# Eurus-Holmes/VAG-NMT

Hardware: AMD Instinct MI355X
Metric: training sentence-pairs/sec (Multi30K en->de, B=64) (higher is better)
Workload: dtype f32; 1 GPU; configs[1]: multimodal en->de train step, B=64/GPU, Ts=Tt=40, E=256, H=512, S=512, I=2048, Vs=8507, V=9391, dropout 0.3/0.5/0.5, tied emb, teacher_force_ratio=1; global_batch=64, parallelism=dp1, hip_graph=True

## Files before the change

include/vag_nmt.h:

```cpp
#ifndef VAG_NMT_H
#define VAG_NMT_H
#include <stddef.h>
#include <stdint.h>

#ifdef __cplusplus
extern "C" {
#endif

typedef void* vag_stream_t;

typedef struct { const float *w_ih, *w_hh, *b_ih, *b_hh; } vag_gru_w;
typedef struct { float *w_ih, *w_hh, *b_ih, *b_hh; } vag_gru_g;

typedef struct {
    const float* emb;
    vag_gru_w gru1;
    const float *attn_h, *attn_v, *c2h;
    vag_gru_w gru2;
} vag_dec_w;
typedef struct {
    float* emb;
    vag_gru_g gru1;
    float *attn_h, *attn_v, *c2h;
    vag_gru_g gru2;
// ... 367 lines not shown
int vag_mrt_pack(const int64_t* cand, int64_t G, int64_t Nc, int64_t L, const int64_t* gold, int64_t Tg, int include_gold, int64_t* tgt,
                 int64_t Tt, float* valid, vag_stream_t stream);

#define VAG_ADAM_SCRATCH_BYTES 2048
#define VAG_ADAM_SCRATCH_SKIPPED_OFFSET 28
#define VAG_ADAM_SCRATCH_GUARD_OFFSET 32
int vag_clip_adam_flat(float* p, float* g, float* m, float* v, int64_t n, int nseg, const int64_t* seg_off,
                       const float* seg_lr, const float* seg_wd, float clip, float grad_scale, float beta1,
                       float beta2, float eps, int zero_grad, int32_t* step, float* norm_out, void* scratch,
                       const float* lr_dev, vag_stream_t stream);

int vag_clip_adam_flat_ema(float* p, float* g, float* m, float* v, int64_t n, int nseg, const int64_t* seg_off,
                           const float* seg_lr, const float* seg_wd, float clip, float grad_scale, float beta1,
                           float beta2, float eps, int zero_grad, int32_t* step, float* norm_out, void* scratch,
                           const float* lr_dev, float* ema, float ema_decay, int ema_warmup, vag_stream_t stream);

int vag_swap_flat(float* a, float* b, int64_t n, vag_stream_t stream);

int vag_clip_adam_shard(float* p, float* g, float* m, float* v, int64_t n, int nseg, const int64_t* seg_off,
                        const float* seg_lr, const float* seg_wd, float clip, float grad_scale, float beta1,
                        float beta2, float eps, int zero_grad, int32_t* step, float* norm_out, void* scratch,
                        const float* lr_dev, int64_t lo, int64_t hi, int phase, double* sumsq, vag_stream_t stream);

typedef struct {
    const float* enc_emb;
    vag_gru_w enc_fw, enc_bw;
    const float *im_w, *im_b, *txt_w, *txt_b, *ctx2ctx, *emb2ctx, *mlp_w;
    const float *ini_w, *ini_b;
    const float* attn_e;
    vag_dec_w dec;
    vag_head_w head;
} vag_model_w;
typedef struct {
    float* enc_emb;
    vag_gru_g enc_fw, enc_bw;
    float *im_w, *im_b, *txt_w, *txt_b, *ctx2ctx, *emb2ctx, *mlp_w;
    float *ini_w, *ini_b;
    float* attn_e;
    vag_dec_g dec;
    vag_head_g head;
} vag_model_g;
typedef struct {
    int64_t B, Ts, Tt, Es, Et, H, S, I, V, ldl;
    int32_t multimodal;
    int32_t attn_method;
    int32_t activation_vse;
    int32_t rank_kind;
    int32_t free_run;
    int32_t storage;
    float margin, loss_w, init_split, p_emb, p_ctx, p_out;
    int32_t loss_ring;
    void* guard;
    float label_smoothing;
    int32_t mrt_n;
    float mrt_alpha, mrt_scale;
    const float *mrt_cost, *mrt_valid;
} vag_step_cfg;
int64_t vag_step_ws_floats(const vag_step_cfg* cfg);
int64_t vag_step_ws_offset(const vag_step_cfg* cfg, int which);
int vag_train_step(const vag_step_cfg* cfg, const vag_model_w* w, const vag_model_g* g, const int64_t* src,
                   const int32_t* lengths, const int64_t* tgt, const float* im, const float* vocab_weight, uint64_t* rng,
                   const float* derived, float* ws, float* losses, int phases, vag_stream_t stream);
typedef struct {
    int32_t k;
    float lambda;
    const int32_t* idx;
    const float* q;
} vag_kd_cfg;
int vag_step_kd_check(const vag_step_cfg* cfg, const vag_kd_cfg* kd);
int vag_train_step_kd(const vag_step_cfg* cfg, const vag_kd_cfg* kd, const vag_model_w* w, const vag_model_g* g, const int64_t* src,
                      const int32_t* lengths, const int64_t* tgt, const float* im, const float* vocab_weight, uint64_t* rng,
                      const float* derived, float* ws, float* losses, int phases, vag_stream_t stream);
typedef struct {
    float alpha;
    float* kl;
} vag_rdrop_cfg;
int vag_step_rdrop_check(const vag_step_cfg* cfg, const vag_rdrop_cfg* rd);
int vag_train_step_rdrop(const vag_step_cfg* cfg, const vag_rdrop_cfg* rd, const vag_model_w* w, const vag_model_g* g,
                         const int64_t* src, const int32_t* lengths, const int64_t* tgt, const float* im, const float* vocab_weight,
                         uint64_t* rng, const float* derived, float* ws, float* losses, int phases, vag_stream_t stream);
int vag_set_operator_context(const float* derived, int storage);
int vag_set_option(const char* name, int64_t value);
int64_t vag_handoff_planes_floats(int64_t B, int64_t Ts, int64_t Tt, int64_t H);
int vag_set_handoff_planes(float* buf, int64_t floats);
int vag_copy4(const void* const* src, void* const* dst, const int64_t* bytes, int n, vag_stream_t stream);
int64_t vag_derived_floats(int64_t H);
int vag_derive_weights(vag_dec_w w, const float* enc_whh_fw, const float* enc_whh_bw, int64_t H, int with_fp16,
                       float* derived, vag_stream_t stream);

int vag_recurrence_supported(int kind, int64_t B, int64_t Ts, int64_t Tt, int64_t H);
int vag_persistent_timeouts(void);
int vag_set_operator_guard(void* guard);
int vag_recurrence_time(int kind, double* ms_total, int* launches);
int vag_gemm_group_plan(int n, const int64_t* M, const int64_t* N, const int64_t* K, const int* accumulate, int* split, int* order);
enum { VAG_GEMM_TILED64 = 0,
       VAG_GEMM_TILED128_F32 = 1,
       VAG_GEMM_SPLIT128 = 2,
       VAG_GEMM_BIG256 = 3 };
int vag_gemm_plan(int64_t M, int64_t N, int64_t K, int a_kc, int b_kc, int vec, float beta, int act, int c_half, int a_bf16,
                  int rowsum, int planes, int* plan);
int64_t vag_recurrence_sync_words(int kind, int64_t B, int64_t T);
int vag_cgru_recurrence_fwd(const float* pe, const float* mask, const float* h0, const float* xp1, vag_dec_w w, const float* wcat,
                            const float* bcat, const float* encwp, int64_t B, int64_t Ts, int64_t Tt, int64_t H, float* h1,
                            float* g1, float* qhp, float* alpha, float* h2_all, float* g2, float* psc, void* sync,
                            vag_stream_t stream);

#define VAG_COMM_ID_BYTES 128
typedef struct vag_comm_s* vag_comm_t;
int vag_comm_unique_id(void* id);
int vag_comm_init(vag_comm_t* comm, int nranks, int rank, const void* id);
int vag_comm_allreduce(vag_comm_t comm, float* buf, int64_t n, vag_stream_t stream);
int vag_comm_size(vag_comm_t comm);
int vag_comm_destroy(vag_comm_t comm);

int vag_dropout_mask(const uint64_t* rng, int which, int64_t n, float p, float* out, vag_stream_t stream);
int vag_rng_advance(uint64_t* rng, vag_stream_t stream);

#ifdef __cplusplus
}
#endif
#endif
```

vag-nmt_amd/csrc/api.hip:

```cpp
#include "../../include/vag_nmt.h"
#include "api_shared.h"
#include <cstring>

static thread_local VagCallCtx g_base_ctx;
static thread_local VagCallCtx* g_active_ctx = nullptr;
VagCallCtx& vag_ctx() { return g_active_ctx ? *g_active_ctx : g_base_ctx; }
VagCallScope::VagCallScope(VagCallCtx& c) : ctx(c), prev(g_active_ctx) { g_active_ctx = &c; }
VagCallScope::~VagCallScope() {
    (void)vag_loss_defer_flush();
    if (ctx.leaf_on) vag_leaf_drop();
    g_active_ctx = prev;
}
static inline const float* as_f(const vag_half* p) { return reinterpret_cast<const float*>(p); }

VagOptions& vag_opt() {
    static VagOptions o;
    return o;
}

extern "C" {

int vag_version(void) { return 330; }

int vag_set_option(const char* name, int64_t value) {
// ... 325 lines not shown
    hipStream_t s = S_(stream);
    VAG_CHECK_ARG(dec_w_ok(w) && prep && H > 0 && H % 4 == 0 && aligned16(prep));
    const int64_t C = 2 * H;
    CgruPrep p = cgru_prep(prep, H);
    VAG_TRY(copy_async(p.wcat, w.attn_h, C * H * sizeof(float), s));
    VAG_TRY(copy_async(p.wcat + C * H, w.gru2.w_hh, 3 * H * H * sizeof(float), s));
    VAG_TRY(zero_async(p.bcat, C * sizeof(float), s));
    VAG_TRY(copy_async(p.bcat + C, w.gru2.b_hh, 3 * H * sizeof(float), s));
    return gemm_nn(3 * H, C, H, w.gru2.w_ih, H, w.c2h, C, 0.f, p.wp, C, s);
}

int vag_derive_weights(vag_dec_w w, const float* enc_whh_fw, const float* enc_whh_bw, int64_t H, int with_fp16,
                       float* derived, vag_stream_t stream) {
    hipStream_t s = S_(stream);
    VAG_CHECK_ARG(dec_w_ok(w) && enc_whh_fw && enc_whh_bw && derived && H > 0 && H % 4 == 0 && aligned16(derived));
    const int64_t C = 2 * H, Q = C + 3 * H;
    DerivedW d = derived_layout(derived, H);
    CgruPrep p = cgru_prep(d.prep, H);
    const VagJob jobs[9] = {
        {w.attn_h, p.wcat, C, H, H, H, 1},
        {w.gru2.w_hh, p.wcat + C * H, 3 * H, H, H, H, 1},
        {nullptr, p.bcat, 1, C, C, C, 0},
        {w.gru2.b_hh, p.bcat + C, 1, 3 * H, 3 * H, 3 * H, 1},
        {w.attn_h, d.wcatT, C, H, H, Q, 2},
        {w.gru2.w_hh, d.wcatT + C, 3 * H, H, H, Q, 2},
        {w.gru1.w_hh, d.whh1T, 3 * H, H, H, 3 * H, 2},
        {enc_whh_fw, d.encT, 3 * H, H, H, 3 * H, 2},
        {enc_whh_bw, d.encT + 3 * H * H, 3 * H, H, H, 3 * H, 2},
    };
    VAG_TRY(vag_jobs_launch(jobs, 9, s));
    if (with_fp16) {
        VAG_CHECK_ARG(H % 8 == 0);
        auto h = [&](vag_half* q) { return reinterpret_cast<float*>(q); };
        const VagJob j16[10] = {
            {w.attn_h, h(d.wcat16), C, H, H, H, 3},
            {w.gru2.w_hh, h(d.wcat16 + C * H), 3 * H, H, H, H, 3},
            {w.attn_h, h(d.wcatT16), C, H, H, Q, 4},
            {w.gru2.w_hh, h(d.wcatT16 + C), 3 * H, H, H, Q, 4},
            {w.gru1.w_hh, h(d.whh1_16), 3 * H, H, H, H, 3},
            {w.gru1.w_hh, h(d.whh1T16), 3 * H, H, H, 3 * H, 4},
            {enc_whh_fw, h(d.enc16), 3 * H, H, H, H, 3},
            {enc_whh_bw, h(d.enc16 + 3 * H * H), 3 * H, H, H, H, 3},
            {enc_whh_fw, h(d.encT16), 3 * H, H, H, 3 * H, 4},
            {enc_whh_bw, h(d.encT16 + 3 * H * H), 3 * H, H, H, 3 * H, 4},
        };
        VAG_TRY(vag_jobs_launch(j16, 10, s));
    }
    return VAG_OK;
}

struct CgruWs {
    float *xp1, *h1, *g1, *g2, *qhp, *scores, *alpha, *tmp, *prep, *encwp;
    float* uk;
    float* psc;
    unsigned* sync;
    unsigned* sync_b;
    float* dal;
    int64_t total;
};
static CgruWs cgru_ws(float* ws, int64_t B, int64_t Ts, int64_t Tt, int64_t E, int64_t H) {
    CgruWs w;
    const int64_t C = 2 * H;
    WsCarver c(ws);
    w.xp1 = c.take(Tt * B * 3 * H);
    w.g1 = c.take(Tt * 4 * B * H);
    w.g2 = c.take(Tt * 4 * B * H);
    w.qhp = c.take(Tt * B * (C + 3 * H));
    w.scores = c.take(B * Ts);
    w.alpha = c.take(Tt * B * Ts);
    w.tmp = c.take(B * E);
    w.prep = c.take(cgru_prep(nullptr, H).total);
    w.encwp = c.take(B * Ts * 3 * H);
    w.uk = c.take(B * Ts * H);
    w.h1 = c.take(Tt * B * H);
    w.psc = c.take(Tt * B * Ts * 4);
    w.sync = c.take_as<unsigned>(vag_dec_persistent_sync_words(B, Tt));
    w.sync_b = c.take_as<unsigned>(vag_dec_persistent_sync_words(B, Tt));
    w.dal = c.take(Tt * B * Ts * 4);
    w.total = c.off;
    return w;
}
}
void vag_step_zero_ranges(float* ws_enc, float* ws_dec, int64_t B, int64_t Ts, int64_t Tt, int64_t Es, int64_t Et, int64_t H,
                          unsigned** p, int64_t* n) {
    BiGruWs e = bigru_ws(ws_enc, B, Ts, Es, H);
    p[0] = e.sync;
    n[0] = (reinterpret_cast<unsigned*>(ws_enc) + e.total) - e.sync;
    CgruWs d = cgru_ws(ws_dec, B, Ts, Tt, Et, H);
    p[2] = reinterpret_cast<unsigned*>(e.dx);
    n[2] = Ts * B * Es;
    p[1] = reinterpret_cast<unsigned*>(d.h1);
    n[1] = (reinterpret_cast<unsigned*>(ws_dec) + d.total) - p[1];
}
extern "C" {
int64_t vag_cgru_ws_floats(int64_t B, int64_t Ts, int64_t Tt, int64_t E, int64_t H) {
    return cgru_ws(nullptr, B, Ts, Tt, E, H).total;
}
int64_t vag_cgru_ws_offset(int64_t B, int64_t Ts, int64_t Tt, int64_t E, int64_t H, int which) {
    static float base[1];
    CgruWs k = cgru_ws(base, B, Ts, Tt, E, H);
    const float* p = which == 0 ? k.alpha : which == 1 ? k.h1 : which == 2 ? k.qhp : nullptr;
    return p ? (int64_t)(p - base) : -1;
}

struct StepBufs {
    const float* xp1;
    const float* hprev;
    float *h1, *g1, *g2, *qhp, *scores, *alpha, *c, *h2;
};

static int cgru_step(const float* enc, const float* pe, const float* mask, int64_t rps, const vag_dec_w& w,
                     const CgruPrep& p, int64_t N, int64_t Ts, int64_t H, const StepBufs& b, hipStream_t s) {
    const int64_t C = 2 * H, Q = C + 3 * H;
    GruStepArgs a = gru_cell_args(b.xp1, b.hprev, w.gru1.w_hh, w.gru1.b_hh, N, H, b.h1, b.g1);
    VAG_TRY(vag_gru_step_launch(a, 1, s));
    VAG_TRY(vag_skinny_launch(N, Q, H, b.h1, H, p.wcat, H, p.bcat, nullptr, 0, b.qhp, Q, 0, s));
    VAG_TRY(vag_attn_scores_launch(0, pe, b.qhp, Q, w.attn_v, mask, N, rps, Ts, C, b.scores, s));
    VAG_TRY(vag_attn_ctx_launch(1, b.scores, enc, N, rps, Ts, C, b.alpha, b.c, s));
    a.lda = C; a.ldw = C; a.ldother = Q; a.K = (int)C; a.comp_hidden = 0;
    a.s[0].A = b.c; a.s[0].W = p.wp; a.s[0].bias = w.gru2.b_ih; a.s[0].other = b.qhp + C;
    a.s[0].hprev = b.h1; a.s[0].hout = b.h2; a.s[0].save = b.g2;
    VAG_TRY(vag_gru_step_launch(a, 1, s));
    return VAG_OK;
}

int vag_cgru_attn_decode_seq_fwd(const float* enc, const float* pe, const float* mask, const float* h0, int64_t* tok,
                                 vag_dec_w w, int64_t B, int64_t Ts, int64_t Tt, int64_t E, int64_t H, int64_t V,
                                 float* h2_all, float* c_all, float* e_all, float* ws, int free_run,
                                 const vag_head_w* head, float p_out, const uint64_t* rng, float* tmid, float* logits,
                                 int64_t ldl, vag_stream_t stream) {
    hipStream_t s = S_(stream);
    VAG_CHECK_ARG(enc && pe && mask && h0 && tok && h2_all && c_all && e_all && ws && dec_w_ok(w));
    VAG_CHECK_ARG(B > 0 && Ts > 0 && Tt > 0 && E % 4 == 0 && H % 4 == 0 && E > 0 && H > 0 && aligned16(ws));
    VAG_CHECK_ARG(!free_run || (head && tmid && logits && ldl >= V && ldl % 4 == 0));
    const int64_t C = 2 * H, Q = C + 3 * H, BH = B * H;
    CgruWs k = cgru_ws(ws, B, Ts, Tt, E, H);
    CgruPrep p = cgru_prep(k.prep, H);
    if (vag_ctx().derived) p = cgru_prep(derived_layout(const_cast<float*>(vag_ctx().derived), H).prep, H);
    else VAG_TRY(vag_cgru_prepare(w, H, k.prep, stream));
    const bool hoist = !free_run;
    const bool s16 = vag_ctx().store16;
    VAG_CHECK_ARG(!s16 || (hoist && vag_ctx().derived && H % 8 == 0 && Ts * B < (1ll << 28)));
    DerivedW dw16 = {};
    if (s16) dw16 = derived_layout(const_cast<float*>(vag_ctx().derived), H);
    {
        VagGemmGroup grp;
        if (!free_run) {
            if (!vag_ctx().step_gathered) VAG_TRY(vag_embed_gather_launch(tok, B, 1, Tt, B, w.emb, E, e_all, nullptr, 0, 0.f, s));
            VAG_TRY(vag_gemm_launch(Tt * B, 3 * H, E, 1.f, e_all, E, 1, w.gru1.w_ih, 1, E, 0.f, k.xp1, 3 * H, w.gru1.b_ih, 0, s));
        }
        VAG_TRY(vag_gemm_launch(B * Ts, H, C, 1.f, enc, C, 1, w.c2h, 1, C, 0.f, k.uk, H, nullptr, 0, s));
        VAG_TRY(grp.end(s));
    }
    {
        VagGemmGroup grp2;
        VAG_TRY(vag_gemm_launch(B * Ts, 3 * H, H, 1.f, k.uk, H, 1, w.gru2.w_ih, 1, H, 0.f, k.encwp, 3 * H, nullptr, 0, s, s16 ? 1 : 0));
        VAG_TRY(grp2.end(s));
    }
    auto hoisted_step = [&](int64_t t) -> int {
        const float* hprev = t == 0 ? h0 : h2_all + (t - 1) * BH;
        float* h1 = k.h1 + t * BH;
        float* qhp = k.qhp + t * B * Q;
        const GruStepArgs a = gru_cell_args(k.xp1 + t * B * 3 * H, hprev, s16 ? as_f(dw16.whh1_16) : w.gru1.w_hh, w.gru1.b_hh, B, H,
                                            h1, k.g1 + t * 4 * BH);
        VAG_TRY(vag_gru_step_launch(a, 1, s, s16));
        if (s16) {
            VAG_TRY(vag_skinny_launch(B, C, H, h1, H, as_f(dw16.wcat16), H, nullptr, nullptr, 0, qhp, Q, 0, s, true));
            VAG_TRY(vag_attn_dot_side_launch(0, pe, qhp, Q, w.attn_v, mask, nullptr, B, Ts, C, k.scores, B, 3 * H, H, h1, H,
                                             as_f(dw16.wcat16 + C * H), H, p.bcat + C, nullptr, qhp + C, Q, s, true));
            VAG_TRY(vag_attn_ctx_gru_launch(k.scores, k.encwp, B, 1, Ts, H, w.gru2.b_ih, qhp + C, Q, h1, k.alpha + t * B * Ts,
                                            h2_all + t * BH, k.g2 + t * 4 * BH, s, true));
            return VAG_OK;
        }
        if (Ts * B < (1ll << 28)) {
// ... 827 lines not shown
int vag_sample_step_p_dev(const float* const* logp, const int64_t* ldl, int64_t M, int64_t* toks, float* token_logp,
                          int32_t* di_state, int64_t max_len, int64_t* tok_out, int64_t B, int64_t n, int64_t V, float temperature,
                          int64_t top_k, const uint64_t* rng, int32_t* n_alive, float top_p, int32_t* set_size,
                          vag_stream_t stream) {
    VAG_CHECK_ARG(di_state != nullptr);
    return vag_sample_step_p_launch(logp, ldl, M, toks, token_logp, 0, di_state, max_len, nullptr, nullptr, nullptr, tok_out, B, n,
                                    V, temperature, top_k, rng, n_alive, top_p, set_size, S_(stream));
}
int vag_sample_noise(const uint64_t* rng, int64_t di, int64_t N, int64_t V, float* out, vag_stream_t stream) {
    return vag_sample_noise_launch(rng, di, N, V, out, S_(stream));
}

int vag_mbr_supported(int64_t Nh, int64_t Lh, int64_t Nr, int64_t Lr) { return vag_mbr_supported_host(Nh, Lh, Nr, Lr); }
int vag_mbr_select(const int64_t* hyps, const int64_t* refs, const float* weights, int64_t B, int64_t Nh, int64_t Lh, int64_t Nr,
                   int64_t Lr, int utility, int32_t* matches, float* util, float* expected, int64_t* best, vag_stream_t stream) {
    return vag_mbr_select_launch(hyps, refs, weights, B, Nh, Lh, Nr, Lr, utility, matches, util, expected, best, S_(stream));
}

int vag_corpus_bleu_supported(int64_t Lh, int64_t R, int64_t Lr) { return vag_corpus_bleu_supported_host(Lh, R, Lr); }
int vag_corpus_bleu_stats(const int64_t* hyps, const int64_t* refs, const int32_t* n_refs, int64_t N, int64_t Lh, int64_t R,
                          int64_t Lr, int32_t* per_sentence, int64_t* totals, vag_stream_t stream) {
    return vag_corpus_bleu_stats_launch(hyps, refs, n_refs, N, Lh, R, Lr, per_sentence, totals, S_(stream));
}

int vag_surface_expand(const int64_t* rows, int64_t R, int64_t L, const int32_t* off, const int32_t* chars, int64_t V, int32_t* out,
                       int64_t C, int32_t* lens, vag_stream_t stream) {
    return vag_surface_expand_launch(rows, R, L, off, chars, V, out, C, lens, S_(stream));
}
int vag_chrf_supported(int64_t Nh, int64_t Ch, int64_t Nr, int64_t Cr) { return vag_chrf_supported_host(Nh, Ch, Nr, Cr); }
int vag_chrf_max_chars(void) { return vag_chrf_max_chars_host(); }
int vag_chrf_select(const int32_t* hchars, const int32_t* hlens, const int32_t* rchars, const int32_t* rlens, const float* weights,
                    int64_t B, int64_t Nh, int64_t Ch, int64_t Nr, int64_t Cr, int32_t* matches, float* util, float* expected,
                    int64_t* best, vag_stream_t stream) {
    return vag_chrf_select_launch(hchars, hlens, rchars, rlens, weights, B, Nh, Ch, Nr, Cr, matches, util, expected, best, S_(stream));
}

int vag_mrt_weights(const float* nll, const float* cost, const float* valid, int64_t B, int64_t Tt, int64_t N, float alpha, float scale,
                    float* inv_cnt, float* q, float* risk, vag_stream_t stream) {
    VAG_CHECK_ARG(risk != nullptr);
    return vag_mrt_weights_launch(nll, cost, valid, B, Tt, N, alpha, scale, inv_cnt, q, risk, nullptr, 0.f, 0, S_(stream));
}
int vag_mrt_pack(const int64_t* cand, int64_t G, int64_t Nc, int64_t L, const int64_t* gold, int64_t Tg, int include_gold, int64_t* tgt,
                 int64_t Tt, float* valid, vag_stream_t stream) {
    return vag_mrt_pack_launch(cand, G, Nc, L, gold, Tg, include_gold, tgt, Tt, valid, S_(stream));
}

int vag_clip_adam_flat(float* p, float* g, float* m, float* v, int64_t n, int nseg, const int64_t* seg_off,
                       const float* seg_lr, const float* seg_wd, float clip, float grad_scale, float beta1, float beta2,
                       float eps, int zero_grad, int32_t* step, float* norm_out, void* scratch, const float* lr_dev,
                       vag_stream_t stream) {
    return vag_clip_adam_launch(p, g, m, v, n, nseg, seg_off, seg_lr, seg_wd, clip, grad_scale, beta1, beta2, eps, zero_grad,
                                step, norm_out, scratch, lr_dev, S_(stream));
}

int vag_clip_adam_flat_ema(float* p, float* g, float* m, float* v, int64_t n, int nseg, const int64_t* seg_off,
                           const float* seg_lr, const float* seg_wd, float clip, float grad_scale, float beta1, float beta2,
                           float eps, int zero_grad, int32_t* step, float* norm_out, void* scratch, const float* lr_dev,
                           float* ema, float ema_decay, int ema_warmup, vag_stream_t stream) {
    return vag_clip_adam_ema_launch(p, g, m, v, n, nseg, seg_off, seg_lr, seg_wd, clip, grad_scale, beta1, beta2, eps, zero_grad,
                                    step, norm_out, scratch, lr_dev, ema, ema_decay, ema_warmup, S_(stream));
}

int vag_swap_flat(float* a, float* b, int64_t n, vag_stream_t stream) { return vag_swap_flat_launch(a, b, n, S_(stream)); }

int vag_clip_adam_shard(float* p, float* g, float* m, float* v, int64_t n, int nseg, const int64_t* seg_off, const float* seg_lr,
                        const float* seg_wd, float clip, float grad_scale, float beta1, float beta2, float eps, int zero_grad,
                        int32_t* step, float* norm_out, void* scratch, const float* lr_dev, int64_t lo, int64_t hi, int phase,
                        double* sumsq, vag_stream_t stream) {
    return vag_clip_adam_shard_launch(p, g, m, v, n, nseg, seg_off, seg_lr, seg_wd, clip, grad_scale, beta1, beta2, eps, zero_grad,
                                      step, norm_out, scratch, lr_dev, lo, hi, phase, sumsq, S_(stream));
}

int vag_copy4(const void* const* src, void* const* dst, const int64_t* bytes, int n, vag_stream_t stream) {
    return vag_copy4_launch(src, dst, bytes, n, S_(stream));
}

int vag_recurrence_supported(int kind, int64_t B, int64_t Ts, int64_t Tt, int64_t H) {
    if (kind == 0) return vag_enc_persistent_ok(B, Ts, H) ? 1 : 0;
    if (kind == 1) return vag_dec_persistent_ok(B, Ts, Tt, H) ? 1 : 0;
    return 0;
}
int vag_persistent_timeouts(void) { return vag_persistent_timeouts_read(); }
int64_t vag_handoff_planes_floats(int64_t B, int64_t Ts, int64_t Tt, int64_t H) {
    const int64_t e = vag_enc_bwd_planes_floats(B, Ts, H), d = vag_dec_bwd_planes_floats(B, Tt, H), f = vag_enc_fwd_planes_floats(B, Ts, H);
    return std::max(std::max(e, d), f);
}
int vag_set_handoff_planes(float* buf, int64_t floats) {
    VAG_CHECK_ARG((buf == nullptr || (floats > 0 && aligned16(buf))));
    g_base_ctx.handoff_planes = buf;
    g_base_ctx.handoff_floats = buf ? floats : 0;
    return VAG_OK;
}
int vag_set_operator_guard(void* guard) {
    VAG_CHECK_ARG((reinterpret_cast<uintptr_t>(guard) & 3) == 0);
    g_base_ctx.guard = reinterpret_cast<unsigned*>(guard);
    return VAG_OK;
}
int vag_gemm_group_plan(int n, const int64_t* M, const int64_t* N, const int64_t* K, const int* accumulate, int* split,
                        int* order) {
    return vag_gemm_group_plan_host(n, M, N, K, accumulate, split, order);
}
int vag_gemm_plan(int64_t M, int64_t N, int64_t K, int a_kc, int b_kc, int vec, float beta, int act, int c_half, int a_bf16,
                  int rowsum, int planes, int* plan) {
    return vag_gemm_plan_host(M, N, K, a_kc, b_kc, vec, beta, act, c_half, a_bf16, rowsum, planes, plan);
}
int vag_recurrence_time(int kind, double* ms_total, int* launches) { return vag_persistent_time_read(kind, ms_total, launches); }
int64_t vag_recurrence_sync_words(int kind, int64_t B, int64_t T) {
    return kind == 0 ? vag_enc_persistent_sync_words(B, T) : vag_dec_persistent_sync_words(B, T);
}
int vag_cgru_recurrence_fwd(const float* pe, const float* mask, const float* h0, const float* xp1, vag_dec_w w, const float* wcat,
                            const float* bcat, const float* encwp, int64_t B, int64_t Ts, int64_t Tt, int64_t H, float* h1,
                            float* g1, float* qhp, float* alpha, float* h2_all, float* g2, float* psc, void* sync,
                            vag_stream_t stream) {
    VAG_CHECK_ARG(dec_w_ok(w) && vag_dec_persistent_ok(B, Ts, Tt, H));
    return vag_dec_fwd_persistent_launch(pe, mask, h0, xp1, w.gru1.w_hh, w.gru1.b_hh, wcat, bcat, w.attn_v, encwp, w.gru2.b_ih, h1,
                                         g1, qhp, alpha, h2_all, g2, psc, reinterpret_cast<unsigned*>(sync), B, Ts, Tt, H,
                                         S_(stream));
}

int vag_dropout_mask(const uint64_t* rng, int which, int64_t n, float p, float* out, vag_stream_t stream) {
    VAG_CHECK_ARG(which >= 1 && which <= 3);
    return vag_dropout_mask_launch(rng, which, n, p, out, S_(stream));
}
int vag_rng_advance(uint64_t* rng, vag_stream_t stream) { return vag_rng_advance_launch(rng, S_(stream)); }

}
```

vag-nmt_amd/csrc/call_ctx.h:

```cpp
#pragma once
#include <hip/hip_runtime.h>
#include <stdint.h>
#include "../../include/vag_nmt.h"

struct LossTask {
    const float* nll = nullptr; const float* inv_cnt = nullptr; float* losses = nullptr;
    int B = 0, Tt = 0, has_vse = 0, ring = 0;
    float w_mt = 0.f, w_vse = 0.f;
};
struct RmwDefer {
    float* out = nullptr;
    const float *a1 = nullptr, *x1 = nullptr, *a2 = nullptr, *x2 = nullptr;
    const float *mask = nullptr, *dx = nullptr; float coef = 0.f;
    int64_t B = 0, Ts = 0, C = 0;
};

struct VagCallCtx {
    const float* derived = nullptr;
    bool store16 = false;
    int gemm_planes = 3;
    unsigned* guard = nullptr;
    float* handoff_planes = nullptr;
    int64_t handoff_floats = 0;

    bool step_zeroed = false;
    bool step_gathered = false;
    bool poison_inject = false;
    bool persist_prezeroed = false;
    struct GemmScratch { float* slab = nullptr; int64_t floats = 0; unsigned* tickets = nullptr; int64_t ntickets = 0; hipStream_t stream = nullptr; } gemm_scratch;
    const float* gemm_prezeroed[4] = {nullptr, nullptr, nullptr, nullptr};
    struct LeafStream { hipStream_t stream = nullptr; hipEvent_t event = nullptr; bool used = false; } leaf_stream;

    struct RowMix { float* xmix = nullptr; float split = 0.f; const float* done = nullptr; } row_mix;
    struct Dh0Tanh { bool req = false; const float* done = nullptr; } dh0_tanh;
    struct LossDefer { bool on = false; LossTask task; hipStream_t stream = nullptr; } loss_defer;
    RmwDefer rmw;
    bool leaf_on = false;
    const float* u_all_ready = nullptr;
};

VagCallCtx& vag_ctx();

struct VagCallScope {
    VagCallCtx& ctx;
    VagCallCtx* prev;
    explicit VagCallScope(VagCallCtx& c);
    ~VagCallScope();
    VagCallScope(const VagCallScope&) = delete;
    VagCallScope& operator=(const VagCallScope&) = delete;
};
```

vag-nmt_amd/csrc/common.h:

```cpp
#pragma once
#include <hip/hip_runtime.h>
#include <stdint.h>
#include <stddef.h>

#define VAG_OK 0
#define VAG_EINVAL (-22)
#define VAG_ENOSYS (-38)

#define VAG_CHECK_ARG(cond)                     \
    do {                                        \
        if (!(cond)) return VAG_EINVAL;         \
    } while (0)

#define VAG_LAUNCH_CHECK()                                  \
    do {                                                    \
        hipError_t e__ = hipGetLastError();                 \
        if (e__ != hipSuccess) return (int)e__;             \
    } while (0)

#define VAG_TRY(expr)                  \
    do {                               \
        int r__ = (expr);              \
        if (r__ != 0) return r__;      \
    } while (0)

typedef float f32x4 __attribute__((ext_vector_type(4)));
typedef float f32x16 __attribute__((ext_vector_type(16)));

static inline int64_t cdiv64(int64_t a, int64_t b) { return (a + b - 1) / b; }
static inline bool aligned16(const void* p) { return (((uintptr_t)p) & 15) == 0; }

template <bool MAX>
__device__ __forceinline__ float wave_allreduce(float v) {
#define VAG_DPP_ROR(N) __builtin_bit_cast(float, __builtin_amdgcn_update_dpp(0, __builtin_bit_cast(int, v), 0x120 + (N), 0xf, 0xf, false))
    { const float o = VAG_DPP_ROR(8); v = MAX ? fmaxf(v, o) : v + o; }
    { const float o = VAG_DPP_ROR(4); v = MAX ? fmaxf(v, o) : v + o; }
    { const float o = VAG_DPP_ROR(2); v = MAX ? fmaxf(v, o) : v + o; }
    { const float o = VAG_DPP_ROR(1); v = MAX ? fmaxf(v, o) : v + o; }
#undef VAG_DPP_ROR
    float a = v, b = v;
    asm volatile("s_nop 1\n\tv_permlane16_swap_b32 %0, %1\n\ts_nop 1" : "+v"(a), "+v"(b));
    v = MAX ? fmaxf(a, b) : a + b;
    a = v; b = v;
    asm volatile("s_nop 1\n\tv_permlane32_swap_b32 %0, %1\n\ts_nop 1" : "+v"(a), "+v"(b));
    return MAX ? fmaxf(a, b) : a + b;
}
__device__ __forceinline__ float quad_sum(float v) {
    v += __builtin_bit_cast(float, __builtin_amdgcn_update_dpp(0, __builtin_bit_cast(int, v), 0xB1, 0xf, 0xf, false));
    v += __builtin_bit_cast(float, __builtin_amdgcn_update_dpp(0, __builtin_bit_cast(int, v), 0x4E, 0xf, 0xf, false));
    return v;
}
__device__ __forceinline__ float wave_sum(float v) { return wave_allreduce<false>(v); }
__device__ __forceinline__ float wave_max(float v) { return wave_allreduce<true>(v); }
__device__ __forceinline__ float vag_tanh(float x) {
    float e = __expf(2.0f * x);
    return 1.0f - 2.0f * __builtin_amdgcn_rcpf(e + 1.0f);
}
__device__ __forceinline__ float vag_sigmoid(float x) { return __builtin_amdgcn_rcpf(1.0f + __expf(-x)); }

__device__ __host__ __forceinline__ uint64_t vag_mix64(uint64_t z) {
    z += 0x9E3779B97F4A7C15ull;
    z = (z ^ (z >> 30)) * 0xBF58476D1CE4E5B9ull;
    z = (z ^ (z >> 27)) * 0x94D049BB133111EBull;
    return z ^ (z >> 31);
}
__device__ __forceinline__ float vag_drop_mul(const uint64_t* rng, uint32_t stream_id, uint64_t idx, float p) {
    if (rng == nullptr || p <= 0.0f) return 1.0f;
    uint64_t key = vag_mix64(rng[0] ^ (rng[1] * 0xD1342543DE82EF95ull) ^ ((uint64_t)stream_id << 56));
    uint64_t r = vag_mix64(key + idx);
    float u = (float)(r >> 40) * (1.0f / 16777216.0f);
    return (u >= p) ? 1.0f / (1.0f - p) : 0.0f;
}

typedef _Float16 vag_half;
__device__ __forceinline__ float h16_lo(unsigned p) { return (float)__builtin_bit_cast(vag_half, (unsigned short)(p & 0xffffu)); }
__device__ __forceinline__ float h16_hi(unsigned p) { return (float)__builtin_bit_cast(vag_half, (unsigned short)(p >> 16)); }
template <bool XH> __device__ __forceinline__ float4 ld4_any(const float* base, int64_t elem) {
    if (XH) {
        const uint2 p = *reinterpret_cast<const uint2*>(reinterpret_cast<const vag_half*>(base) + elem);
        return make_float4(h16_lo(p.x), h16_hi(p.x), h16_lo(p.y), h16_hi(p.y));
    }
    return *reinterpret_cast<const float4*>(base + elem);
}
template <bool XH> __device__ __forceinline__ float ld1_any(const float* base, int64_t elem) {
    if (XH) return (float)reinterpret_cast<const vag_half*>(base)[elem];
    return base[elem];
}

struct VagOptions {
    int gemm_f32mfma = 0;
    int gemm_big = 1;
    int gemm_slabs = 1;
    int gemm_nogroup = 0;
    int gemm_force_tile = 0;
    int gemm_force_splitk = 0;
    int gemm_debug = 0;
    int64_t head_chunk = -1;
    int head_fuse = 1;
    int head_bf16_grads = 1;
    int persistent = 1;
    int persistent_dec_bwd = 1;
    int persistent_enc_bwd = 1;
    int attn_dot_reg = 1;
    int handoff_planes = 7;
    int free_persistent = 1;
    int s16_one_plane = 1;
    int head_bf16_dlogits = 1;
    int leaf_queue = 1;
    int attn_row = 1;
    int loss_ride = 1;
    int dec_xcd_map = 33;
    int step_fork = 0;
    int64_t persist_spin_limit = 0;
    int persist_timing = 0;
    int64_t dec_bwd_stamps = 0;
    int64_t dec_stamps = 0;
};
VagOptions& vag_opt();

enum { VAG_ACT_NONE = 0, VAG_ACT_TANH = 1 };
enum { VAG_DROP_ENC_EMB = 1, VAG_DROP_ENC_CTX = 2, VAG_DROP_DEC_OUT = 3 };

int vag_gemm_launch(int64_t M, int64_t N, int64_t K, float alpha, const float* A, int64_t sam, int64_t sak,
                    const float* B, int64_t sbk, int64_t sbn, float beta, float* C, int64_t ldc,
                    const float* bias, int act, hipStream_t stream, int c_half = 0,
                    float* rowsum = nullptr,
                    int a_bf16 = 0);
int vag_gemm_launch_planes(int planes, int64_t M, int64_t N, int64_t K, float alpha, const float* A, int64_t sam, int64_t sak,
                           const float* B, int64_t sbk, int64_t sbn, float beta, float* C, int64_t ldc, hipStream_t stream,
                           int a_bf16 = 0);
int64_t vag_logits_parts_count(int64_t M, int64_t N, int64_t K, const float* A, int64_t lda, const float* W, int64_t ldw);
int vag_logits_parts_launch(int64_t M, int64_t N, int64_t K, const float* A, int64_t lda, const float* W, int64_t ldw,
                            const float* bias, float* out, int64_t ldo, float* parts, hipStream_t stream);
int vag_skinny_launch(int64_t M, int64_t N, int64_t K, const float* A, int64_t lda, const float* W, int64_t ldw,
                      const float* bias, const float* addend, int64_t ldadd, float* out, int64_t ldo, int act,
                      hipStream_t stream, bool w16 = false);
int vag_attn_dot_side_launch(int mode, const float* x, const float* q, int64_t ldq, const float* v, const float* mask,
                             const float* addend, int64_t N, int64_t Ts, int64_t W, float* out, int64_t M, int64_t Np,
                             int64_t K, const float* A, int64_t lda, const float* Wt, int64_t ldw, const float* pbias,
                             const float* padd, float* P, int64_t ldp, hipStream_t stream, bool s16 = false);
int vag_skinny_gather_launch(int64_t M, int64_t N, int64_t K, const float* table, int64_t ldt, const int64_t* idx, const float* W,
                             int64_t ldw, const float* bias, float* out, int64_t ldo, float* gathered, int64_t ldg,
                             hipStream_t stream);
int vag_skinny3_launch(int64_t M, int64_t N, const float* const* A, const int64_t* lda, const float* const* W, const int64_t* ldw,
                       const int64_t* K, const float* const* bias, float* out, int64_t ldo, int act, const uint64_t* rng, int sid,
                       float p, int64_t drop_idx0, hipStream_t stream, const float* addend = nullptr, int64_t ldadd = 0,
                       const float* addend2 = nullptr, const int64_t* idx2 = nullptr, int64_t ldadd2 = 0);
int vag_skinny_batched_launch(int64_t nb, int64_t M, int64_t N, int64_t K, const float* A, int64_t lda, int64_t bsA,
                              const float* W, int64_t ldw, int64_t bsW, float* out, int64_t ldo, int64_t bsO,
                              hipStream_t stream);
int vag_skinny_nn_launch(int64_t M, int64_t N, int64_t K, const float* A, int64_t lda, const float* B, int64_t ldb,
                         float beta, float* C, int64_t ldc, hipStream_t stream,
                         float* out2 = nullptr, int64_t ldo2 = 0, float scale2 = 0.f, int acc2 = 0);
void vag_gemm_group_begin();
int vag_gemm_group_end(hipStream_t stream);
void vag_gemm_group_abort();
struct VagGemmGroup {
    bool open = true;
    explicit VagGemmGroup(bool enable = true) : open(enable) { if (enable) vag_gemm_group_begin(); }
    int end(hipStream_t s) { if (!open) return VAG_OK; open = false; return vag_gemm_group_end(s); }
    ~VagGemmGroup() { if (open) vag_gemm_group_abort(); }
    VagGemmGroup(const VagGemmGroup&) = delete;
    VagGemmGroup& operator=(const VagGemmGroup&) = delete;
};
int vag_leaf_flush(hipStream_t stream);
void vag_leaf_drop();
int vag_colsum_launch(const float* X, int64_t M, int64_t N, int64_t ld, float* out, hipStream_t stream);
int vag_colsum3_launch(const float* X, int64_t M, int64_t N, int64_t ld, float* out, float* out2, float* out3,
                       hipStream_t stream);
int vag_transpose_launch(const float* in, int64_t M, int64_t N, float* out, hipStream_t stream);

struct GruSide {
    const float* A;
    const float* W;
    const float* bias;
    const float* other;
    const int64_t* other_idx;
    const float* hprev;
    float* hout;
    float* out2;
    float* save;
    int t;
};
struct GruStepArgs {
    GruSide s[2];
    int64_t lda, ldw, ldother, ldh, ld2;
    int M, K, H;
// ... 29 lines not shown
```

vag-nmt_amd/csrc/kernels.h:

```cpp
#pragma once
#include "common.h"
#include "call_ctx.h"
#include "../../include/vag_nmt.h"

static inline int64_t round64(int64_t n) { return (n + 63) & ~63ll; }
struct WsCarver {
    float* base;
    int64_t off = 0;
    explicit WsCarver(float* b) : base(b) {}
    float* take(int64_t n) {
        float* q = base ? base + off : nullptr;
        off += round64(n);
        return q;
    }
    template <class T> T* take_as(int64_t n) {
        return reinterpret_cast<T*>(take((n * (int64_t)sizeof(T) + 3) / 4));
    }
};
struct DecTables {
    float *embp, *embw3, *encw2;
    unsigned long long* cand;
    int64_t total;
};
DecTables vag_dec_tables(float* base, int64_t B, int64_t Ts, int64_t Tt, int64_t E, int64_t H, int64_t V, bool token_only = false);
// ... 107 lines not shown
                          const float* vw, const float* inv_cnt, const float* d_loss, const int32_t* idx, const float* q, int64_t K,
                          float lambda, float* g_bias, hipStream_t s);

int vag_token_conf_launch(const float* const* logits, const int64_t* ldl, const float* const* lse, int64_t M, const int64_t* tgt,
                          int64_t B, int64_t Tt, int64_t V, float* token_logp, float* entropy, int32_t* rank, int32_t* top,
                          float* top_logp, float* sent, hipStream_t s);

inline bool vag_rdrop_ok(float alpha) { return alpha > 0.f && alpha < INFINITY; }
int vag_rdrop_pair_launch(const float* logits, int64_t ldl, int64_t rows, int64_t V, const int64_t* tgt, int64_t B, int64_t Tt,
                          const float* vw, const float* lse, float alpha, float* kl, float* nll, hipStream_t s);
int vag_rdrop_bwd_colsum_launch(float* logits, int64_t ldl, int64_t rows, int64_t V, const int64_t* tgt, int64_t B, int64_t Tt,
                                const float* vw, const float* lse, const float* kl, const float* inv_cnt, const float* d_loss,
                                float alpha, float* g_bias, hipStream_t s, float eps);

int vag_l2norm_fwd_launch(const float* y, int64_t B, int64_t S, float* nrm, float* out, hipStream_t s);
int vag_l2norm_bwd_launch(const float* y, const float* nrm, const float* out, const float* d_out, int64_t B, int64_t S,
                          int act, float* dy, hipStream_t s);
int vag_rank_loss_launch(const float* scores, int64_t B, float margin, int kind, float* G, float* loss, hipStream_t s,
                         const float* g_scale = nullptr, float scale = 1.f);
int vag_retrieval_rank_launch(const float* scores, int64_t N, int* ranks, hipStream_t s);
int vag_scale_by_dev_launch(float* x, int64_t n, const float* scalar, hipStream_t s);

int vag_clip_adam_shard_launch(float* p, float* g, float* m, float* v, int64_t n, int nseg, const int64_t* seg_off,
                               const float* seg_lr, const float* seg_wd, float clip, float grad_scale, float beta1, float beta2,
                               float eps, int zero_grad, int32_t* step, float* norm_out, void* scratch, const float* lr_dev,
                               int64_t lo, int64_t hi, int phase, double* sumsq, hipStream_t s);
int vag_clip_adam_launch(float* p, float* g, float* m, float* v, int64_t n, int nseg, const int64_t* seg_off,
                         const float* seg_lr, const float* seg_wd, float clip, float grad_scale, float beta1,
                         float beta2, float eps, int zero_grad, int32_t* step, float* norm_out, void* scratch, const float* lr_dev,
                         hipStream_t s);
int vag_clip_adam_ema_launch(float* p, float* g, float* m, float* v, int64_t n, int nseg, const int64_t* seg_off,
                             const float* seg_lr, const float* seg_wd, float clip, float grad_scale, float beta1,
                             float beta2, float eps, int zero_grad, int32_t* step, float* norm_out, void* scratch,
                             const float* lr_dev, float* ema, float ema_decay, int ema_warmup, hipStream_t s);
int vag_swap_flat_launch(float* a, float* b, int64_t n, hipStream_t s);

bool vag_enc_persistent_ok(int64_t B, int64_t Ts, int64_t H);
int64_t vag_enc_persistent_sync_words(int64_t B, int64_t Ts);
int vag_enc_fwd_persistent_launch(const float* xp, const float* w_fw, const float* w_bw, const float* b_fw, const float* b_bw,
                                  const int* lengths, float* hst, float* gates, float* enc, float* planes, int64_t planes_floats,
                                  unsigned* sync, const uint64_t* rng, float p_ctx, int64_t B, int64_t Ts, int64_t H, hipStream_t s);
int64_t vag_enc_fwd_planes_floats(int64_t B, int64_t Ts, int64_t H);
int vag_enc_bwd_persistent_launch(const float* whhT, const float* d_enc, const float* gates, const float* hst, const int* lengths,
                                  const uint64_t* rng, float p_ctx, float* d_xp, float* dgh, float* planes, unsigned* sync, int64_t B,
                                  int64_t Ts, int64_t H, hipStream_t s);
int64_t vag_enc_bwd_planes_floats(int64_t B, int64_t Ts, int64_t H);
int64_t vag_dec_bwd_planes_floats(int64_t B, int64_t Tt, int64_t H);
bool vag_enc_wide16_ok(int64_t B, int64_t Ts, int64_t H);
int vag_enc_fwd_wide16_launch(const float* xp, const vag_half* w16_fw, const vag_half* w16_bw, const float* b_fw, const float* b_bw,
                              const int* lengths, float* hst, float* gates, float* enc, vag_half* hx, unsigned* sync, const uint64_t* rng,
                              float p_ctx, int64_t B, int64_t Ts, int64_t H, hipStream_t s);
int vag_enc_bwd_wide16_launch(const vag_half* wt16, const float* d_enc, const float* gates, const float* hst, const int* lengths,
                              const uint64_t* rng, float p_ctx, float* d_xp, float* dgh, vag_half* gx, unsigned* sync, int64_t B,
                              int64_t Ts, int64_t H, hipStream_t s);
int vag_gemm_group_plan_host(int n, const int64_t* M, const int64_t* N, const int64_t* K, const int* accumulate, int* split,
                             int* order);
int vag_gemm_plan_host(int64_t M, int64_t N, int64_t K, int a_kc, int b_kc, int vec, float beta, int act, int c_half, int a_bf16,
                       int rowsum, int planes, int* plan);
int vag_persistent_timeouts_read(void);
unsigned* vag_persist_guard(void);
int vag_persistent_time_read(int kind, double* ms_total, int* launches);
bool vag_dec_bwd_persistent_ok(int64_t B, int64_t Ts, int64_t Tt, int64_t H);
int vag_dec_bwd_persistent_launch(const float* pe, const float* encwp, const float* v, const float* wcatT, const float* whh1T,
                                  const float* h0, const float* h2_all, const float* h1, const float* g1, const float* g2,
                                  const float* qhp, const float* alpha, const float* d_h2_all, const float* dah, float* dgi2,
                                  float* dqgh, float* ds, float* dgi1, float* dgh1, float* d_h0, float* dal, float* planes,
                                  int64_t planes_floats, unsigned* sync, int64_t B, int64_t Ts, int64_t Tt, int64_t H, hipStream_t s);
float* vag_cgru_bwd_scratch_de(float* scratch, int64_t B, int64_t Ts, int64_t Tt, int64_t E, int64_t H);
float* vag_cgru_bwd_scratch_du(float* scratch, int64_t B, int64_t Ts, int64_t Tt, int64_t E, int64_t H);
int vag_attn_dot_row_launch(bool bwd, const float* x, const float* q, int64_t ldq, const float* mask, const float* alpha, int64_t B,
                            int64_t Ts, int64_t C, float* wout, float* sum, hipStream_t s);
int vag_rank_bwd_launch(const float* G, const float* im, const float* sv, const float* d_loss, int64_t B, int64_t S, float* d_im,
                        float* d_s, hipStream_t s);
int vag_attn_wsum_pair_launch(const float* a, const float* y, int64_t Wy, float* out_src, const float* x, int64_t Wx, float* out_time,
                              int64_t B, int64_t Ts, int64_t T, hipStream_t s);
int vag_loss_defer_flush();
bool vag_attn_row_gru_ok(int64_t N, int64_t Ts, int64_t H, int64_t W2);
int vag_attn_row_gru_launch(const float* pe, const float* q, int64_t ldq, const float* v, const float* mask, const float* keys,
                            const float* x2, int64_t N, int64_t rps, int64_t Ts, int64_t H, int64_t W2, const float* b_ih,
                            const float* hp, int64_t ldhp, const float* hprev, float* alpha, float* hout, float* out2, hipStream_t s);
int vag_rmw_defer_flush(hipStream_t s);
bool vag_rmw_defer_meanpool(const float* mask, const float* dx, float coef, int64_t B, int64_t Ts, int64_t C, float* out, int accumulate);
void vag_step_zero_ranges(float* ws_enc, float* ws_dec, int64_t B, int64_t Ts, int64_t Tt, int64_t Es, int64_t Et, int64_t H,
                          unsigned** p, int64_t* n);
bool vag_dec_persistent_ok(int64_t B, int64_t Ts, int64_t Tt, int64_t H);
int64_t vag_dec_persistent_sync_words(int64_t B, int64_t Tt);
int vag_dec_fwd_persistent_launch(const float* pe, const float* mask, const float* h0, const float* xp1, const float* W1,
                                  const float* b1, const float* wcat, const float* bcat, const float* v, const float* encwp,
                                  const float* b_ih2, float* h1, float* g1, float* qhp, float* alpha, float* h2_all, float* g2,
                                  float* psc, unsigned* sync, int64_t B, int64_t Ts, int64_t Tt, int64_t H, hipStream_t s);
bool vag_dec_free_persistent_ok(int64_t B, int64_t Ts, int64_t Tt, int64_t E, int64_t H, int64_t V);
int vag_dec_free_persistent_launch(const float* pe, const float* mask, const float* h0, const float* W1, const float* b1,
                                   const float* wcat, const float* bcat, const float* v, const float* encwp, const float* b_ih2,
                                   float* h1, float* g1, float* qhp, float* alpha, float* h2_all, float* g2, float* psc,
                                   unsigned* sync, const DecTables& tab, const float* hw1, const float* hb1, const float* hb2,
                                   const float* hb3, const float* out_w, const float* out_b, float* tmid, float* logits, int64_t ldl,
                                   int64_t* tok, const uint64_t* rng, float p_out, int64_t B, int64_t Ts, int64_t Tt, int64_t E,
                                   int64_t H, int64_t V, hipStream_t s);

int64_t vag_beam_scratch_bytes_impl(int64_t B, int64_t k, int64_t V);
int vag_beam_step_launch(float* logp, int64_t ldl, float* nll, int64_t* beam, int64_t di, int32_t* di_state,
                         int64_t max_len, const float* h_in, float* h_out, int64_t* tok_out, int64_t B, int64_t k,
                         int64_t V, int64_t H, int32_t* n_alive, void* scratch, hipStream_t s, const float* parts = nullptr,
                         int64_t nparts = 0, int flags = 0);
int vag_beam_finish_launch(const float* nll, const int64_t* beam, int64_t max_len, int64_t steps, int64_t B, int64_t k,
                           int64_t* out, float* best, hipStream_t s);
int vag_beam_ens_step_launch(const float* const* logp, const int64_t* ldl, int64_t M, float* nll, int64_t* beam, int64_t di,
                             int32_t* di_state, int64_t max_len, const float* const* h_in, float* const* h_out, const int64_t* H,
                             int64_t* tok_out, int64_t B, int64_t k, int64_t V, int32_t* n_alive, void* scratch, hipStream_t s,
                             int flags = 0);
int vag_beam_finish_nbest_launch(const float* nll, const int64_t* beam, int64_t max_len, int64_t steps, int64_t B, int64_t k,
                                 int64_t n, int64_t* out, float* scores, hipStream_t s);
int vag_beam_finish_nbest_slots_launch(const float* nll, const int64_t* beam, int64_t max_len, int64_t steps, int64_t B, int64_t k,
                                       int64_t n, int64_t* out, float* scores, int64_t* slots, hipStream_t s);
int64_t vag_beam_div_scratch_bytes_impl(int64_t B, int64_t k, int64_t V);
int vag_beam_div_step_launch(const float* const* logp, const int64_t* ldl, int64_t M, float* nll, int64_t* beam, int64_t di,
                             int32_t* di_state, int64_t max_len, const float* const* h_in, float* const* h_out, const int64_t* H,
                             int64_t* tok_out, int64_t B, int64_t k, int64_t V, int32_t* n_alive, void* scratch, int flags,
                             int64_t groups, float strength, hipStream_t s);
int64_t vag_beam_req_scratch_bytes_impl(int64_t B, int64_t k, int64_t V);
int vag_beam_req_step_launch(const float* const* logp, const int64_t* ldl, int64_t M, float* nll, int64_t* beam, int64_t di,
                             int32_t* di_state, int64_t max_len, const float* const* h_in, float* const* h_out, const int64_t* H,
                             int64_t* tok_out, int64_t B, int64_t k, int64_t V, int32_t* n_alive, void* scratch, int flags,
                             const int64_t* required, int32_t* state, hipStream_t s);
int64_t vag_beam_sbs_scratch_bytes_impl(int64_t B, int64_t k, int64_t V);
int vag_beam_sbs_step_launch(const float* const* logp, const int64_t* ldl, int64_t M, float* nll, int64_t* beam, int64_t di,
                             int32_t* di_state, int64_t max_len, const float* const* h_in, float* const* h_out, const int64_t* H,
                             int64_t* tok_out, int64_t B, int64_t k, int64_t V, int32_t* n_alive, void* scratch, int flags,
                             const uint64_t* rng, float* gum, hipStream_t s);
int64_t vag_beam_pen_scratch_bytes_impl(int64_t B, int64_t k, int64_t V);
int vag_beam_cover_launch(const float* const* alpha, int64_t M, const float* mask, const float* cov, const int64_t* beam, int64_t di,
                          const int32_t* di_state, int64_t max_len, int64_t B, int64_t k, int64_t Tp, float beta, float* cov_row,
                          float* cp_row, hipStream_t s);
int vag_beam_pen_step_launch(const float* const* logp, const int64_t* ldl, int64_t M, float* nll, int64_t* beam, int64_t di,
                             int32_t* di_state, int64_t max_len, const float* const* h_in, float* const* h_out, const int64_t* H,
                             int64_t* tok_out, int64_t B, int64_t k, int64_t V, int32_t* n_alive, void* scratch, int flags,
                             int32_t* lens, const float* cp_row, float* cpen, const float* cov_row, float* cov, int64_t Tp,
                             const float* lp, const float* bonus, int stepwise, hipStream_t s);
int vag_beam_finish_pen_launch(const float* nll, const int64_t* beam, const int32_t* lens, const float* cpen, const float* lp,
                               const float* bonus, int64_t max_len, int64_t steps, int64_t B, int64_t k, int64_t n, int64_t* out,
                               float* scores, int64_t* slots, float* logp, int32_t* length, float* cp, hipStream_t s);
int vag_beam_constrain_launch(float* const* logp, const int64_t* ldl, int64_t M, const int64_t* beam, int64_t di,
                              const int32_t* di_state, bool dev_form, int64_t max_len, int64_t B, int64_t k, int64_t V,
                              const int64_t* prefix, int64_t Lp, const int64_t* phrases, const int32_t* phrase_sent, int64_t P,
                              int64_t ngram, hipStream_t s);
int vag_forced_score_launch(const float* const* logits, const int64_t* ldl, const float* const* lse, int64_t M,
                            const int64_t* tgt, int64_t B, int64_t Tt, int64_t V, float* token_logp, float* logp, float* score,
                            hipStream_t s);
int vag_beam_attn_record_launch(const float* const* alpha, int64_t M, float* attn_hist, int64_t di, const int32_t* di_state,
                                int64_t max_len, int64_t B, int64_t k, int64_t Tp, hipStream_t s);
int vag_beam_finish_align_launch(const float* nll, const int64_t* beam, const float* attn_hist, int64_t max_len, int64_t steps,
                                 int64_t B, int64_t k, int64_t n, int64_t Tp, int64_t Ts, int64_t* out, float* scores,
                                 float* attention, int64_t* src_pos, hipStream_t s);
int vag_forced_align_launch(const float* const* alpha, int64_t M, const int64_t* tgt, int64_t B, int64_t Tt, int64_t Ts,
                            float* attention, int64_t* src_pos, hipStream_t s);
int vag_ens_argmax_launch(const float* const* logp, const int64_t* ldl, int64_t M, int64_t N, int64_t V, int64_t* out,
                          hipStream_t s);

int vag_sample_step_launch(const float* const* logp, const int64_t* ldl, int64_t M, int64_t* toks, float* token_logp, int64_t di,
                           int32_t* di_state, int64_t max_len, const float* const* h_in, float* const* h_out, const int64_t* H,
                           int64_t* tok_out, int64_t B, int64_t n, int64_t V, float temperature, int64_t top_k, const uint64_t* rng,
                           int32_t* n_alive, hipStream_t s);
int vag_sample_step_p_launch(const float* const* logp, const int64_t* ldl, int64_t M, int64_t* toks, float* token_logp, int64_t di,
                             int32_t* di_state, int64_t max_len, const float* const* h_in, float* const* h_out, const int64_t* H,
                             int64_t* tok_out, int64_t B, int64_t n, int64_t V, float temperature, int64_t top_k, const uint64_t* rng,
                             int32_t* n_alive, float top_p, int32_t* set_size, hipStream_t s);
int vag_sample_noise_launch(const uint64_t* rng, int64_t di, int64_t N, int64_t V, float* out, hipStream_t s);
// ... 67 lines not shown
```

vag-nmt_amd/csrc/persist.hip:

```cpp
#include "kernels.h"
#include "gemm_shared.h"
#include <algorithm>
#include <atomic>
#include <mutex>

namespace {

typedef unsigned __attribute__((address_space(1))) gu32;
#define RLX_AGENT __ATOMIC_RELAXED, __HIP_MEMORY_SCOPE_AGENT

constexpr unsigned SPIN_LIMIT = 1u << 19;
__device__ unsigned g_persist_timeouts;
__device__ unsigned g_persist_guard[2];
__device__ __forceinline__ void note_timeout(unsigned* err, unsigned* guard) {
    __hip_atomic_store((gu32*)err, 1u, RLX_AGENT);
    __hip_atomic_store((gu32*)guard, 1u, RLX_AGENT);
    atomicAdd(guard + 1, 1u);
    atomicAdd(&g_persist_timeouts, 1u);
}

struct EncPArgs {
    const float* xp;
    const float* W[2];
    const float* bias[2];
// ... 106 lines not shown
#pragma unroll
    for (int i = 0; i < 3; ++i) {
        const u32x4 t = {q[i][0], q[i][1], q[i][2], q[i][3]};
        p[i] = __builtin_bit_cast(bf16x8, t);
    }
}
__device__ __forceinline__ f32x4 mma6(const bf16x8 (&a)[3], const bf16x8 (&b)[3], f32x4 acc) {
    acc = __builtin_amdgcn_mfma_f32_16x16x32_bf16(a[0], b[2], acc, 0, 0, 0);
    acc = __builtin_amdgcn_mfma_f32_16x16x32_bf16(a[1], b[1], acc, 0, 0, 0);
    acc = __builtin_amdgcn_mfma_f32_16x16x32_bf16(a[2], b[0], acc, 0, 0, 0);
    acc = __builtin_amdgcn_mfma_f32_16x16x32_bf16(a[0], b[1], acc, 0, 0, 0);
    acc = __builtin_amdgcn_mfma_f32_16x16x32_bf16(a[1], b[0], acc, 0, 0, 0);
    acc = __builtin_amdgcn_mfma_f32_16x16x32_bf16(a[0], b[0], acc, 0, 0, 0);
    return acc;
}

constexpr int PL_PLANE_BYTES = 64 * 16, PL_KSTEP_BYTES = 3 * PL_PLANE_BYTES;
__host__ __device__ constexpr int64_t pl_block_bytes(int64_t K) { return (K / 32) * PL_KSTEP_BYTES; }
constexpr int PL_W2_PLANE_BYTES = 32 * 16, PL_W2_KSTEP_BYTES = 3 * PL_W2_PLANE_BYTES;
__host__ __device__ constexpr int64_t pl_w2_bytes(int64_t H) { return (3 * H / 32) * PL_W2_KSTEP_BYTES; }
typedef unsigned u32x2 __attribute__((ext_vector_type(2)));
__device__ __forceinline__ unsigned pl_slot_off(int r, int k0) { return (unsigned)((r + 16 * ((k0 & 31) >> 3)) * 16 + 8 * ((k0 >> 2) & 1)); }
__device__ __forceinline__ void st_planes4(const char* kblk, unsigned voff, float4 v) {
    unsigned q[3][2];
    split3(v.x, v.y, q[0][0], q[1][0], q[2][0]);
    split3(v.z, v.w, q[0][1], q[1][1], q[2][1]);
    const u32x2 x0 = {q[0][0], q[0][1]}, x1 = {q[1][0], q[1][1]}, x2 = {q[2][0], q[2][1]};
    asm volatile("global_store_dwordx2 %0, %1, %4 sc1\n\tglobal_store_dwordx2 %0, %2, %4 offset:1024 sc1\n\t"
                 "global_store_dwordx2 %0, %3, %4 offset:2048 sc1\n\ts_nop 1"
                 :: "v"(voff), "v"(x0), "v"(x1), "v"(x2), "s"(kblk) : "memory");
}
#define VAG_PLD(o, v, a, off) "global_load_dwordx4 %" #o ", %" #v ", %" #a " offset:" #off " sc1\n\t"
template <int N> __device__ __forceinline__ void ld_planes_sc1(const char* p, unsigned voff, u32x4 (&f)[3 * N]);
template <> __device__ __forceinline__ void ld_planes_sc1<1>(const char* p, unsigned voff, u32x4 (&f)[3]) {
    asm volatile(VAG_PLD(0, 3, 4, 0) VAG_PLD(1, 3, 4, 1024) VAG_PLD(2, 3, 4, 2048)
                 "s_waitcnt vmcnt(0)"
                 : "=&v"(f[0]), "=&v"(f[1]), "=&v"(f[2]) : "v"(voff), "s"(p) : "memory");
}
template <> __device__ __forceinline__ void ld_planes_sc1<2>(const char* p, unsigned voff, u32x4 (&f)[6]) {
    const char* p1 = p + 8192;
    asm volatile(VAG_PLD(0, 6, 7, 0) VAG_PLD(1, 6, 7, 1024) VAG_PLD(2, 6, 7, 2048) VAG_PLD(3, 6, 7, 3072) VAG_PLD(4, 6, 8, -4096) VAG_PLD(5, 6, 8, -3072)
                 "s_waitcnt vmcnt(0)"
                 : "=&v"(f[0]), "=&v"(f[1]), "=&v"(f[2]), "=&v"(f[3]), "=&v"(f[4]), "=&v"(f[5]) : "v"(voff), "s"(p), "s"(p1) : "memory");
}
template <> __device__ __forceinline__ void ld_planes_sc1<3>(const char* p, unsigned voff, u32x4 (&f)[9]) {
    const char* p1 = p + 8192;
    asm volatile(VAG_PLD(0, 9, 10, 0) VAG_PLD(1, 9, 10, 1024) VAG_PLD(2, 9, 10, 2048) VAG_PLD(3, 9, 10, 3072) VAG_PLD(4, 9, 11, -4096)
                 VAG_PLD(5, 9, 11, -3072) VAG_PLD(6, 9, 11, -2048) VAG_PLD(7, 9, 11, -1024) VAG_PLD(8, 9, 11, 0)
                 "s_waitcnt vmcnt(0)"
                 : "=&v"(f[0]), "=&v"(f[1]), "=&v"(f[2]), "=&v"(f[3]), "=&v"(f[4]), "=&v"(f[5]), "=&v"(f[6]), "=&v"(f[7]), "=&v"(f[8])
                 : "v"(voff), "s"(p), "s"(p1) : "memory");
}
template <> __device__ __forceinline__ void ld_planes_sc1<4>(const char* p, unsigned voff, u32x4 (&f)[12]) {
    const char* p1 = p + 8192;
    asm volatile(VAG_PLD(0, 12, 13, 0) VAG_PLD(1, 12, 13, 1024) VAG_PLD(2, 12, 13, 2048) VAG_PLD(3, 12, 13, 3072) VAG_PLD(4, 12, 14, -4096)
                 VAG_PLD(5, 12, 14, -3072) VAG_PLD(6, 12, 14, -2048) VAG_PLD(7, 12, 14, -1024) VAG_PLD(8, 12, 14, 0) VAG_PLD(9, 12, 14, 1024)
                 VAG_PLD(10, 12, 14, 2048) VAG_PLD(11, 12, 14, 3072)
                 "s_waitcnt vmcnt(0)"
                 : "=&v"(f[0]), "=&v"(f[1]), "=&v"(f[2]), "=&v"(f[3]), "=&v"(f[4]), "=&v"(f[5]), "=&v"(f[6]), "=&v"(f[7]), "=&v"(f[8]),
                   "=&v"(f[9]), "=&v"(f[10]), "=&v"(f[11])
                 : "v"(voff), "s"(p), "s"(p1) : "memory");
}
template <> __device__ __forceinline__ void ld_planes_sc1<6>(const char* p, unsigned voff, u32x4 (&f)[18]) {
    const char *p1 = p + 8192, *p2 = p + 16384;
    asm volatile(VAG_PLD(0, 18, 19, 0) VAG_PLD(1, 18, 19, 1024) VAG_PLD(2, 18, 19, 2048) VAG_PLD(3, 18, 19, 3072) VAG_PLD(4, 18, 20, -4096)
                 VAG_PLD(5, 18, 20, -3072) VAG_PLD(6, 18, 20, -2048) VAG_PLD(7, 18, 20, -1024) VAG_PLD(8, 18, 20, 0) VAG_PLD(9, 18, 20, 1024)
                 VAG_PLD(10, 18, 20, 2048) VAG_PLD(11, 18, 20, 3072) VAG_PLD(12, 18, 21, -4096) VAG_PLD(13, 18, 21, -3072)
                 VAG_PLD(14, 18, 21, -2048) VAG_PLD(15, 18, 21, -1024) VAG_PLD(16, 18, 21, 0) VAG_PLD(17, 18, 21, 1024)
                 "s_waitcnt vmcnt(0)"
                 : "=&v"(f[0]), "=&v"(f[1]), "=&v"(f[2]), "=&v"(f[3]), "=&v"(f[4]), "=&v"(f[5]), "=&v"(f[6]), "=&v"(f[7]), "=&v"(f[8]),
                   "=&v"(f[9]), "=&v"(f[10]), "=&v"(f[11]), "=&v"(f[12]), "=&v"(f[13]), "=&v"(f[14]), "=&v"(f[15]), "=&v"(f[16]), "=&v"(f[17])
                 : "v"(voff), "s"(p), "s"(p1), "s"(p2) : "memory");
}
#undef VAG_PLD
template <int N>
__device__ __forceinline__ f32x4 mma6_planes(const bf16x8 (&w)[N][3], const u32x4 (&f)[3 * N], f32x4 acc) {
#pragma unroll
    for (int s = 0; s < N; ++s) {
        const bf16x8 hf[3] = {__builtin_bit_cast(bf16x8, f[3 * s]), __builtin_bit_cast(bf16x8, f[3 * s + 1]),
                              __builtin_bit_cast(bf16x8, f[3 * s + 2])};
        acc = mma6(w[s], hf, acc);
    }
    return acc;
}

template <int KS, bool PL>
__global__ __launch_bounds__(512, 1) void enc_fwd_persistent_kernel(EncPArgs a) {
    __shared__ __attribute__((aligned(16))) float lds[21504];
    const int wg = blockIdx.x;
    const int cs = wg % a.CS, rt = a.rt0 + (wg / a.CS) % a.RTP, d = wg / (a.CS * a.RTP);
    const int lane = threadIdx.x & 63, wave = threadIdx.x >> 6;
    const int H = a.H, B = a.B, Ts = a.Ts;
    const int m0 = rt * 16, u0 = cs * 16;
    const int fr = lane & 15, fg = lane >> 4;
    const int kbase = wave * (H >> 3);
    const int64_t BH = (int64_t)B * H;

    bf16x8 wf[KS][3][3];
    {
        const float* W = a.W[d];
#pragma unroll
        for (int s = 0; s < KS; ++s)
#pragma unroll
            for (int j = 0; j < 3; ++j) {
                const float* p = W + (int64_t)(j * H + u0 + fr) * H + kbase + 32 * s + 8 * fg;
                split8(*reinterpret_cast<const float4*>(p), *reinterpret_cast<const float4*>(p + 4), wf[s][j]);
            }
    }
    const int erow = lane >> 2, equad = lane & 3, eslot = erow + 16 * equad;
    const int em = m0 + erow, eu = u0 + 4 * equad;
    const bool eok = wave == 0 && em < B;
    float4 bb[3] = {make_float4(0, 0, 0, 0), make_float4(0, 0, 0, 0), make_float4(0, 0, 0, 0)};
    int len = 0;
    if (eok) {
#pragma unroll
        for (int j = 0; j < 3; ++j) bb[j] = *reinterpret_cast<const float4*>(a.bias[d] + j * H + eu);
        len = a.lengths[em];
    }
    float4 hp = make_float4(0.f, 0.f, 0.f, 0.f);

    float* hs = a.hst + (int64_t)d * (Ts + 1) * BH;
    if (eok) *reinterpret_cast<float4*>(hs + (int64_t)em * H + eu) = hp;
    const __amdgpu_buffer_rsrc_t rs = __builtin_amdgcn_make_buffer_rsrc(hs, 0, (unsigned)((int64_t)(Ts + 1) * BH * 4), 0x00020000);
    gu32* cnt = (gu32*)(a.cnt + ((int64_t)d * a.RT + rt) * Ts);
    const int lrow = min(m0 + ld_row(lane), B - 1);
    const int src4 = ld_src4(lane);
    float4* red = reinterpret_cast<float4*>(lds);
    bool dead = false;
    const char* pld = PL ? a.pl + ((int64_t)d * Ts * a.RT + rt) * pl_block_bytes(H) : nullptr;
    const int64_t pl_step = (int64_t)a.RT * pl_block_bytes(H);
    const int pl_ld = __builtin_amdgcn_readfirstlane(wave) * (KS * PL_KSTEP_BYTES), pl_st = (u0 >> 5) * PL_KSTEP_BYTES;
    const unsigned pl_so = pl_slot_off(erow, eu);

    for (int k = 0; k < Ts; ++k) {
        const int t = d == 0 ? k : Ts - 1 - k;
        float4 xo[3];
        if (eok) {
            const float* xp = a.xp + ((int64_t)t * B + em) * 6 * H + d * 3 * H + eu;
#pragma unroll
            for (int j = 0; j < 3; ++j) xo[j] = *reinterpret_cast<const float4*>(xp + j * H);
        }
        if (k > 0) {
            if (threadIdx.x == 0 && !dead) {
                unsigned spins = 0;
                while (__hip_atomic_load(cnt + (k - 1), RLX_AGENT) < (unsigned)a.CS) {
                    if (++spins > a.spin) { note_timeout(a.err, a.guard); dead = true; break; }
                }
            }
            __syncthreads();
        }
        f32x4 acc[3] = {{0.f, 0.f, 0.f, 0.f}, {0.f, 0.f, 0.f, 0.f}, {0.f, 0.f, 0.f, 0.f}};
        if constexpr (PL) {
            u32x4 gf[3 * KS];
            if (k > 0) {
                ld_planes_sc1<KS>(pld + (k - 1) * pl_step + pl_ld, 16u * lane, gf);
            } else {
#pragma unroll
                for (int s = 0; s < 3 * KS; ++s) gf[s] = u32x4{0u, 0u, 0u, 0u};
            }
#pragma unroll
            for (int s = 0; s < KS; ++s) {
                const bf16x8 hf[3] = {__builtin_bit_cast(bf16x8, gf[3 * s]), __builtin_bit_cast(bf16x8, gf[3 * s + 1]),
                                      __builtin_bit_cast(bf16x8, gf[3 * s + 2])};
#pragma unroll
                for (int j = 0; j < 3; ++j) acc[j] = mma6(wf[s][j], hf, acc[j]);
            }
// ... 506 lines not shown
                        q[0] = (unsigned)__builtin_amdgcn_ds_bpermute(wsrc4, (int)q[0]);
                        q[1] = (unsigned)__builtin_amdgcn_ds_bpermute(wsrc4, (int)q[1]);
                        q[2] = (unsigned)__builtin_amdgcn_ds_bpermute(wsrc4, (int)q[2]);
                        q[3] = (unsigned)__builtin_amdgcn_ds_bpermute(wsrc4, (int)q[3]);
                        acc = __builtin_amdgcn_mfma_f32_16x16x32_f16(wf[hf_ * HK + s], __builtin_bit_cast(h16x8, q), acc, 0, 0, 0);
                    }
                }
                red[(((r * 4 + kq) * 2 + ch)) * 64 + lane] =
                    make_float4(acc[0] * (1.f / GSCALE), acc[1] * (1.f / GSCALE), acc[2] * (1.f / GSCALE), acc[3] * (1.f / GSCALE));
            }
            __syncthreads();
#pragma unroll
            for (int q = 0; q < 4; ++q) {
                const float4 o = red[(((er * 4 + q) * 2 + ech)) * 64 + lane];
                dh.x += o.x; dh.y += o.y; dh.z += o.z; dh.w += o.w;
            }
        }
        if (eok) {
            const bool active = t < len;
            float dhv[4] = {dh.x, dh.y, dh.z, dh.w};
            float gi[3][4], gh[3][4], cy[4];
            if (!active) {
#pragma unroll
                for (int q = 0; q < 4; ++q) { gi[0][q] = gi[1][q] = gi[2][q] = gh[0][q] = gh[1][q] = gh[2][q] = 0.f; cy[q] = dhv[q]; }
            } else {
                const float ev[4] = {e4.x, e4.y, e4.z, e4.w};
                const float r_[4] = {sv[0].x, sv[0].y, sv[0].z, sv[0].w}, z_[4] = {sv[1].x, sv[1].y, sv[1].z, sv[1].w};
                const float n_[4] = {sv[2].x, sv[2].y, sv[2].z, sv[2].w}, hn[4] = {sv[3].x, sv[3].y, sv[3].z, sv[3].w};
                const float hpv[4] = {hp.x, hp.y, hp.z, hp.w};
#pragma unroll
                for (int q = 0; q < 4; ++q) {
                    float e = ev[q];
                    if (a.rng && a.p_ctx > 0.f)
                        e *= vag_drop_mul(a.rng, VAG_DROP_ENC_CTX, (uint64_t)em * ld_add + (uint64_t)t * 2 * H + d * H + eu + q, a.p_ctx);
                    const float x = dhv[q] + e;
                    const float dn_pre = x * (1.f - z_[q]) * (1.f - n_[q] * n_[q]);
                    const float dz_pre = x * (hpv[q] - n_[q]) * z_[q] * (1.f - z_[q]);
                    const float dr_pre = dn_pre * hn[q] * r_[q] * (1.f - r_[q]);
                    gi[0][q] = dr_pre; gi[1][q] = dz_pre; gi[2][q] = dn_pre;
                    gh[0][q] = dr_pre; gh[1][q] = dz_pre; gh[2][q] = dn_pre * r_[q];
                    cy[q] = x * z_[q];
                }
            }
            carry = make_float4(cy[0], cy[1], cy[2], cy[3]);
            const int64_t go = ((int64_t)k * B + em) * K + eu;
#pragma unroll
            for (int g = 0; g < 3; ++g)
                st_sc1_h4(gxd + go + g * H, gh[g][0] * GSCALE, gh[g][1] * GSCALE, gh[g][2] * GSCALE, gh[g][3] * GSCALE);
            asm volatile("s_waitcnt vmcnt(0)" ::: "memory");
            if (lane == 0) __hip_atomic_fetch_add(cnt + k, 1u, RLX_AGENT);
#pragma unroll
            for (int g = 0; g < 3; ++g) *reinterpret_cast<float4*>(dghd + go + g * H) = make_float4(gh[g][0], gh[g][1], gh[g][2], gh[g][3]);
            float* gio = a.d_xp + ((int64_t)t * B + em) * 6 * H + d * 3 * H + eu;
#pragma unroll
            for (int g = 0; g < 3; ++g) *reinterpret_cast<float4*>(gio + g * H) = make_float4(gi[g][0], gi[g][1], gi[g][2], gi[g][3]);
        } else if (lane == 0) {
            __hip_atomic_fetch_add(cnt + k, 1u, RLX_AGENT);
        }
    }
}

struct DecPArgs {
    const float *pe, *mask, *h0, *xp1, *W1, *b1, *wcat, *bcat, *v, *encwp, *b_ih2;
    float *h1, *g1, *qhp, *alpha, *h2_all, *g2, *psc;
    unsigned* cnt;
    unsigned* err;
    unsigned* guard;
    unsigned spin;
    unsigned long long* dbg;
    int B, Ts, Tt, H, RT;
    int rt0;
    const float *embp;
    const float *embw3;
    const float *encw2;
    const float *hw1, *hb1, *hb2, *hb3, *out_w, *out_b;
    float *tmid;
    float *logits;
    unsigned long long* cand;
    int64_t* tok;
    const uint64_t* rng;
    float p_out;
    int V, ldl;
    int xcd_map;
};

constexpr int SHARDS = 4, SHARD_STRIDE = 16, CNT_WORDS = SHARDS * SHARD_STRIDE;
__device__ __forceinline__ void arrive(gu32* c, int i) { __hip_atomic_fetch_add(c + (i & (SHARDS - 1)) * SHARD_STRIDE, 1u, RLX_AGENT); }
__device__ __forceinline__ void wait_count(gu32* c, unsigned want_per_shard, unsigned* err, unsigned* guard, unsigned spin, bool& dead) {
    if (threadIdx.x < 64 && !dead) {
        const int lane = threadIdx.x;
        unsigned spins = 0;
        for (;;) {
            const bool ok = lane >= SHARDS || __hip_atomic_load(c + lane * SHARD_STRIDE, RLX_AGENT) >= want_per_shard;
            if (__all(ok)) break;
            if (++spins > spin) { if (lane == 0) note_timeout(err, guard); dead = true; break; }
        }
    }
    __syncthreads();
}

__device__ __forceinline__ void ld_acc_shards(const float* p0, const float* p1, int64_t stride, float& v0, float& v1) {
    float a0, a1, a2, a3, b0, b1, b2, b3;
    const float *p02 = p0 + 2 * stride, *p12 = p1 + 2 * stride;
    const float *p01 = p0 + stride, *p03 = p02 + stride, *p11 = p1 + stride, *p13 = p12 + stride;
    asm volatile("global_load_dword %0, %8, off sc1\n\tglobal_load_dword %1, %9, off sc1\n\t"
                 "global_load_dword %2, %10, off sc1\n\tglobal_load_dword %3, %11, off sc1\n\t"
                 "global_load_dword %4, %12, off sc1\n\tglobal_load_dword %5, %13, off sc1\n\t"
                 "global_load_dword %6, %14, off sc1\n\tglobal_load_dword %7, %15, off sc1\n\ts_waitcnt vmcnt(0)"
                 : "=&v"(a0), "=&v"(a1), "=&v"(a2), "=&v"(a3), "=&v"(b0), "=&v"(b1), "=&v"(b2), "=&v"(b3)
                 : "v"(p0), "v"(p01), "v"(p02), "v"(p03), "v"(p1), "v"(p11), "v"(p12), "v"(p13) : "memory");
    v0 = (a0 + a1) + (a2 + a3);
    v1 = (b0 + b1) + (b2 + b3);
}

__device__ __forceinline__ void ld_acc_shards_and_rows6(const float* p0, const float* p1, int64_t stride, float& v0, float& v1,
                                                        const float* rows, float4 (&a)[6], float4 (&b)[6]) {
    float a0, a1, a2, a3, b0, b1, b2, b3;
    const float *p02 = p0 + 2 * stride, *p12 = p1 + 2 * stride;
    const float *p01 = p0 + stride, *p03 = p02 + stride, *p11 = p1 + stride, *p13 = p12 + stride;
    asm volatile("global_load_dword %0, %20, off sc1\n\tglobal_load_dword %1, %21, off sc1\n\t"
                 "global_load_dword %2, %22, off sc1\n\tglobal_load_dword %3, %23, off sc1\n\t"
                 "global_load_dword %4, %24, off sc1\n\tglobal_load_dword %5, %25, off sc1\n\t"
                 "global_load_dword %6, %26, off sc1\n\tglobal_load_dword %7, %27, off sc1\n\t"
                 "global_load_dwordx4 %8, %28, off sc1\n\tglobal_load_dwordx4 %9, %28, off offset:16 sc1\n\t"
                 "global_load_dwordx4 %10, %28, off offset:128 sc1\n\tglobal_load_dwordx4 %11, %28, off offset:144 sc1\n\t"
                 "global_load_dwordx4 %12, %28, off offset:256 sc1\n\tglobal_load_dwordx4 %13, %28, off offset:272 sc1\n\t"
                 "global_load_dwordx4 %14, %28, off offset:384 sc1\n\tglobal_load_dwordx4 %15, %28, off offset:400 sc1\n\t"
                 "global_load_dwordx4 %16, %28, off offset:512 sc1\n\tglobal_load_dwordx4 %17, %28, off offset:528 sc1\n\t"
                 "global_load_dwordx4 %18, %28, off offset:640 sc1\n\tglobal_load_dwordx4 %19, %28, off offset:656 sc1\n\t"
                 "s_waitcnt vmcnt(0)"
                 : "=&v"(a0), "=&v"(a1), "=&v"(a2), "=&v"(a3), "=&v"(b0), "=&v"(b1), "=&v"(b2), "=&v"(b3),
                   "=&v"(a[0]), "=&v"(b[0]), "=&v"(a[1]), "=&v"(b[1]), "=&v"(a[2]), "=&v"(b[2]), "=&v"(a[3]), "=&v"(b[3]),
                   "=&v"(a[4]), "=&v"(b[4]), "=&v"(a[5]), "=&v"(b[5])
                 : "v"(p0), "v"(p01), "v"(p02), "v"(p03), "v"(p1), "v"(p11), "v"(p12), "v"(p13), "v"(rows) : "memory");
    v0 = (a0 + a1) + (a2 + a3);
    v1 = (b0 + b1) + (b2 + b3);
}

__device__ __forceinline__ void ld_acc_shards_and_rows3(const float* p0, const float* p1, int64_t stride, float& v0, float& v1,
                                                        const float* rows, float4 (&a)[3], float4 (&b)[3]) {
    float a0, a1, a2, a3, b0, b1, b2, b3;
    const float *p02 = p0 + 2 * stride, *p12 = p1 + 2 * stride;
    const float *p01 = p0 + stride, *p03 = p02 + stride, *p11 = p1 + stride, *p13 = p12 + stride;
    asm volatile("global_load_dword %0, %14, off sc1\n\tglobal_load_dword %1, %15, off sc1\n\t"
                 "global_load_dword %2, %16, off sc1\n\tglobal_load_dword %3, %17, off sc1\n\t"
                 "global_load_dword %4, %18, off sc1\n\tglobal_load_dword %5, %19, off sc1\n\t"
                 "global_load_dword %6, %20, off sc1\n\tglobal_load_dword %7, %21, off sc1\n\t"
                 "global_load_dwordx4 %8, %22, off sc1\n\tglobal_load_dwordx4 %9, %22, off offset:16 sc1\n\t"
                 "global_load_dwordx4 %10, %22, off offset:128 sc1\n\tglobal_load_dwordx4 %11, %22, off offset:144 sc1\n\t"
                 "global_load_dwordx4 %12, %22, off offset:256 sc1\n\tglobal_load_dwordx4 %13, %22, off offset:272 sc1\n\t"
                 "s_waitcnt vmcnt(0)"
                 : "=&v"(a0), "=&v"(a1), "=&v"(a2), "=&v"(a3), "=&v"(b0), "=&v"(b1), "=&v"(b2), "=&v"(b3),
                   "=&v"(a[0]), "=&v"(b[0]), "=&v"(a[1]), "=&v"(b[1]), "=&v"(a[2]), "=&v"(b[2])
                 : "v"(p0), "v"(p01), "v"(p02), "v"(p03), "v"(p1), "v"(p11), "v"(p12), "v"(p13), "v"(rows) : "memory");
    v0 = (a0 + a1) + (a2 + a3);
    v1 = (b0 + b1) + (b2 + b3);
}
__device__ __forceinline__ void ld_acc_shards_and_rows(const float* p0, const float* p1, int64_t stride, float& v0, float& v1,
                                                       const float* rows, float4 (&a)[6], float4 (&b)[6]) {
    ld_acc_shards_and_rows6(p0, p1, stride, v0, v1, rows, a, b);
}
__device__ __forceinline__ void ld_acc_shards_and_rows(const float* p0, const float* p1, int64_t stride, float& v0, float& v1,
                                                       const float* rows, float4 (&a)[3], float4 (&b)[3]) {
    ld_acc_shards_and_rows3(p0, p1, stride, v0, v1, rows, a, b);
}

constexpr int DEC_WGS = 64;
template <int WGS>
__device__ __forceinline__ void dec_slice_map(int mode, int rt0, int& i, int& rt) {
    const int bx = blockIdx.x % WGS;
    rt = rt0 + blockIdx.x / WGS;
    int g = mode == 1 ? 8 : (mode == 2 ? 2 : (mode == 3 ? 4 : 1));
    if (g > WGS / 8) g = WGS / 8;
    i = (bx & 7) * g + ((bx >> 3) % g) + 8 * g * (bx / (8 * g));
}
constexpr int ACC_SHARDS = 4;
constexpr int DEC_U = 8;

constexpr int DEC_E = 4 * DEC_WGS;
__device__ __forceinline__ unsigned long long cand_key(float v, int idx) {
    const unsigned u = __builtin_bit_cast(unsigned, v);
    return ((unsigned long long)(u ^ ((u >> 31) ? 0xffffffffu : 0x80000000u)) << 32) | (unsigned long long)(0xffffffffu - (unsigned)idx);
}

template <bool FREE, int WGS = DEC_WGS>
__global__ __launch_bounds__(512, 1) void dec_fwd_persistent_kernel(DecPArgs a) {
    extern __shared__ __attribute__((aligned(16))) float dlds[];
    static_assert(WGS == 64 || (WGS == 32 && !FREE), "H = 512 (both forms) or H = 256 (teacher-forced form)");
    constexpr int H = WGS * DEC_U, C = 2 * H, Q = C + 3 * H, KS = H / 256;
    constexpr int E = DEC_E;
    int i, rt;
    dec_slice_map<WGS>(a.xcd_map, a.rt0, i, rt);
    const int lane = threadIdx.x & 63, wave = threadIdx.x >> 6;
    const int B = a.B, Ts = a.Ts, Tt = a.Tt;
    const int m0 = rt * 16, u0 = i * DEC_U;
    const int fr = lane & 15, fg = lane >> 4;
    const int kbase = wave * (H >> 3);
    const int64_t BH = (int64_t)B * H;
    float4* red = reinterpret_cast<float4*>(dlds);
    float* pe_s = dlds + 6144;
    float* ew_s = pe_s + 16 * Ts * 16;
    float* sc_s = ew_s + 16 * Ts * 24;
    float* gi_s = sc_s + 16 * Ts;
    float* hp_s = gi_s + 16 * 24;
    float* bs_s = hp_s + 16 * 24;
    float* hs_s = bs_s + 80;
    float* v_s = hs_s + 256;
    float* mk_s = v_s + C;
    float* q_s = mk_s + 16 * Ts;
    float* cw_s = q_s + 256;
    float* hb_s = cw_s + 64;
    int* tok_s = reinterpret_cast<int*>(hb_s + 16);
    float* ew2_s = reinterpret_cast<float*>(tok_s + 16);
    unsigned long long* cb_s = reinterpret_cast<unsigned long long*>(q_s);
    bf16x8* tm_s = reinterpret_cast<bf16x8*>(red);

#ifdef VAG_LAB
#define VAG_PSTAMP(k) do { if (!FREE && a.dbg && blockIdx.x == 0 && threadIdx.x == 0) a.dbg[Tt * 8 + (k)] = __builtin_amdgcn_s_memrealtime(); } while (0)
#else
#define VAG_PSTAMP(k) do { } while (0)
#endif
    VAG_PSTAMP(0);
#ifdef VAG_LAB
    if (!FREE && a.dbg && threadIdx.x == 0 && rt < 8) {
        if (i == 0) a.dbg[(Tt + 1) * 8 + rt] = __builtin_amdgcn_s_memrealtime();
        if (i == WGS - 1) a.dbg[(Tt + 3) * 8 + rt] = __builtin_amdgcn_s_memrealtime();
    }
#endif
    bf16x8 w1[KS][2][3], w2[KS][3][3];
    {
        const int ur = fr & 7, g01 = fr >> 3;
#pragma unroll
        for (int s = 0; s < KS; ++s) {
            const int ko = kbase + 32 * s + 8 * fg;
            const float* p0 = a.W1 + (int64_t)(g01 * H + u0 + ur) * H + ko;
            const float* p1 = a.W1 + (int64_t)(2 * H + u0 + ur) * H + ko;
            if (FREE && fr >= 8 && fr < 12) p1 = a.hw1 + (int64_t)(4 * i + fr - 8) * H + ko;
            split8(*reinterpret_cast<const float4*>(p0), *reinterpret_cast<const float4*>(p0 + 4), w1[s][0]);
            split8(*reinterpret_cast<const float4*>(p1), *reinterpret_cast<const float4*>(p1 + 4), w1[s][1]);
            const float* q0 = a.wcat + (int64_t)(16 * i + fr) * H + ko;
            const float* q1 = a.wcat + (int64_t)(C + g01 * H + u0 + ur) * H + ko;
            const float* q2 = a.wcat + (int64_t)(C + 2 * H + u0 + ur) * H + ko;
            split8(*reinterpret_cast<const float4*>(q0), *reinterpret_cast<const float4*>(q0 + 4), w2[s][0]);
            split8(*reinterpret_cast<const float4*>(q1), *reinterpret_cast<const float4*>(q1 + 4), w2[s][1]);
            split8(*reinterpret_cast<const float4*>(q2), *reinterpret_cast<const float4*>(q2 + 4), w2[s][2]);
        }
    }
    VAG_PSTAMP(1);
    for (int x = threadIdx.x; x < 16 * Ts * 4; x += 512) {
        const int P = x >> 2, c4 = x & 3;
        const int r = P / Ts, sp = P - r * Ts, b = min(m0 + r, B - 1);
        reinterpret_cast<float4*>(pe_s)[x] = *reinterpret_cast<const float4*>(a.pe + ((int64_t)b * Ts + sp) * C + 16 * i + 4 * c4);
    }
    for (int x = threadIdx.x; x < 16 * Ts * 6; x += 512) {
        const int hf = x & 1, g = (x >> 1) % 3, rs_ = x / 6;
        const int r = rs_ / Ts, sp = rs_ - r * Ts, b = min(m0 + r, B - 1);
        reinterpret_cast<float4*>(ew_s)[rs_ * 6 + g * 2 + hf] =
            *reinterpret_cast<const float4*>(a.encwp + ((int64_t)b * Ts + sp) * 3 * H + g * H + u0 + 4 * hf);
    }
    const int hq = (threadIdx.x >> 4) & 1;
    const int em = m0 + fr, eu = u0 + 4 * hq;
    const bool ep = threadIdx.x < 32, eok = ep && em < B;
    if (threadIdx.x < 72) {
        const int kind = threadIdx.x / 24, g = (threadIdx.x / 8) % 3, u = threadIdx.x & 7;
        const float* src = kind == 0 ? a.b1 : (kind == 1 ? a.bcat + C : a.b_ih2);
        bs_s[threadIdx.x] = src[g * H + u0 + u];
    }
    for (int x = threadIdx.x; x < C / 4; x += 512) reinterpret_cast<float4*>(v_s)[x] = reinterpret_cast<const float4*>(a.v)[x];
    for (int x = threadIdx.x; x < 16 * Ts; x += 512) {
        const int r = x / Ts, sp = x - r * Ts;
        mk_s[x] = a.mask[(int64_t)min(m0 + r, B - 1) * Ts + sp];
    }
    if (ep) *reinterpret_cast<float4*>(hs_s + 128 + fr * 8 + 4 * hq) = eok ? *reinterpret_cast<const float4*>(a.h0 + (int64_t)em * H + eu)
                                                                             : make_float4(0.f, 0.f, 0.f, 0.f);
    float4 e3 = make_float4(0.f, 0.f, 0.f, 0.f);
    if (FREE) {
        for (int x = threadIdx.x; x < 16 * Ts; x += 512) {
            const int r = x / Ts, sp = x - r * Ts, b = min(m0 + r, B - 1);
            reinterpret_cast<float4*>(ew2_s)[x] = *reinterpret_cast<const float4*>(a.encw2 + ((int64_t)b * Ts + sp) * E + 4 * i);
        }
        if (threadIdx.x < 4) hb_s[threadIdx.x] = a.hb1[4 * i + threadIdx.x] + a.hb2[4 * i + threadIdx.x] + a.hb3[4 * i + threadIdx.x];
        if (threadIdx.x < 16) {
            const int tk = min(max((int)a.tok[min(m0 + (int)threadIdx.x, B - 1)], 0), a.V - 1);
            tok_s[threadIdx.x] = tk;
            e3 = *reinterpret_cast<const float4*>(a.embw3 + (int64_t)tk * E + 4 * i);
        }
    }
    gu32* c1 = (gu32*)(a.cnt + ((int64_t)0 * a.RT + rt) * Tt * CNT_WORDS);
    gu32* c2 = (gu32*)(a.cnt + ((int64_t)1 * a.RT + rt) * Tt * CNT_WORDS);
    gu32* c4 = (gu32*)(a.cnt + ((int64_t)3 * a.RT + rt) * Tt * CNT_WORDS);
    gu32* c5 = (gu32*)(a.cnt + ((int64_t)2 * a.RT + rt) * Tt * CNT_WORDS);
    gu32* c6 = (gu32*)(a.cnt + ((int64_t)4 * a.RT + rt) * Tt * CNT_WORDS);
    constexpr unsigned PER_SHARD = WGS / SHARDS;
    bool dead = false;
    __syncthreads();
    VAG_PSTAMP(2);
#ifdef VAG_LAB
    const bool stamp = a.dbg != nullptr && blockIdx.x == 0 && threadIdx.x == 0;
#define VAG_STAMP(k) do { if (stamp) a.dbg[t * (FREE ? 16 : 8) + (k)] = __builtin_amdgcn_s_memrealtime(); } while (0)
#else
#define VAG_STAMP(k) do { } while (0)
#endif

    for (int t = 0; t < Tt + (FREE ? 1 : 0); ++t) {
        int tx = threadIdx.x;
        if (FREE) asm volatile("" : "+v"(tx));
        const int lane = tx & 63, wave = FREE ? __builtin_amdgcn_readfirstlane(tx >> 6) : tx >> 6, fr = lane & 15, fg = lane >> 4;
        const int kbase = wave * (H >> 3), hq = (tx >> 4) & 1, em = m0 + fr, eu = u0 + 4 * hq;
        const bool ep = tx < 32, eok = ep && em < B;
        const int arow = min(m0 + fr, B - 1);
        const int lrow = min(m0 + ld_row(lane), B - 1);
        const int src4 = ld_src4(lane);
        VAG_STAMP(0);
        float4 ha[KS], hb[KS];
        if (t == 0) {
            const float* hp = a.h0 + (int64_t)arow * H + kbase + 8 * fg;
#pragma unroll
            for (int s = 0; s < KS; ++s) { ha[s] = *reinterpret_cast<const float4*>(hp + 32 * s); hb[s] = *reinterpret_cast<const float4*>(hp + 32 * s + 4); }
        } else {
            wait_count(c1 + (t - 1) * CNT_WORDS, PER_SHARD, a.err, a.guard, a.spin, dead);
            VAG_STAMP(1);
            ld_rows_tagged<KS>(a.h2_all + ((int64_t)(t - 1) * B + lrow) * H + kbase + 8 * (lane & 3), ha, hb, a.spin, dead, a.err, a.guard);
#pragma unroll
            for (int s = 0; s < KS; ++s) { ha[s] = perm4(ha[s], src4); hb[s] = perm4(hb[s], src4); }
        }
        {
            f32x4 acc[2] = {{0.f, 0.f, 0.f, 0.f}, {0.f, 0.f, 0.f, 0.f}};
#pragma unroll
            for (int s = 0; s < KS; ++s) {
                bf16x8 hf[3];
                split8(ha[s], hb[s], hf);
                acc[0] = mma6(w1[s][0], hf, acc[0]);
                acc[1] = mma6(w1[s][1], hf, acc[1]);
            }
            red[(wave * 3 + 0) * 64 + lane] = make_float4(acc[0][0], acc[0][1], acc[0][2], acc[0][3]);
            red[(wave * 3 + 1) * 64 + lane] = make_float4(acc[1][0], acc[1][1], acc[1][2], acc[1][3]);
        }
        float4 xo[3];
        if (!FREE && eok) {
            const float* xp = a.xp1 + ((int64_t)t * B + em) * 3 * H + eu;
#pragma unroll
            for (int g = 0; g < 3; ++g) xo[g] = *reinterpret_cast<const float4*>(xp + g * H);
        }
        __syncthreads();
        float4 cr = make_float4(0, 0, 0, 0), cz = cr, cn = cr, hw = cr;
        if (ep) {
#pragma unroll
            for (int w = 0; w < 8; ++w) {
                const float4 x0 = red[(w * 3 + 0) * 64 + hq * 16 + fr], x1 = red[(w * 3 + 0) * 64 + (2 + hq) * 16 + fr];
                const float4 x2 = red[(w * 3 + 1) * 64 + hq * 16 + fr];
                cr.x += x0.x; cr.y += x0.y; cr.z += x0.z; cr.w += x0.w;
                cz.x += x1.x; cz.y += x1.y; cz.z += x1.z; cz.w += x1.w;
                cn.x += x2.x; cn.y += x2.y; cn.z += x2.z; cn.w += x2.w;
                if (FREE) {
                    const float4 x3 = red[(w * 3 + 1) * 64 + 2 * 16 + fr];
                    hw.x += x3.x; hw.y += x3.y; hw.z += x3.z; hw.w += x3.w;
                }
            }
        }
        if (FREE) {
            VAG_STAMP(8);
            if (t >= 1) {
                const int ts = t - 1;
                const int V = a.V, NVT = (V + 15) >> 4, NJ = i < NVT ? (NVT - i + 63) >> 6 : 0;
                const int nfull = NJ >> 3, rext = NJ & 7;
                const bool splitx = rext >= 1 && rext <= 3;
                const int xj = splitx ? (wave < 2 * rext ? 8 * nfull + (wave >> 1) : -1) : (wave < rext ? 8 * nfull + wave : -1);
                const int npass = 2 * nfull + (xj < 0 ? 0 : (splitx ? 1 : 2));
                auto pass_ptr = [&](int g, int u) -> const float* {
                    const int j = g < 2 * nfull ? wave + 8 * (g >> 1) : xj;
                    const int k0 = g < 2 * nfull ? 4 * (g & 1) : (splitx ? 4 * (wave & 1) : 4 * (g - 2 * nfull));
                    return a.out_w + (int64_t)min(16 * (i + 64 * j) + fr, V - 1) * E + 32 * (k0 + u) + 8 * fg;
                };
                float4 wr[4][2];
                if (npass > 0) {
#pragma unroll
                    for (int u = 0; u < 4; ++u) { const float* wp = pass_ptr(0, u); wr[u][0] = *reinterpret_cast<const float4*>(wp); wr[u][1] = *reinterpret_cast<const float4*>(wp + 4); }
                }
                if (tx < 16) {
                    const float4 cw = *reinterpret_cast<const float4*>(cw_s + 4 * fr);
                    const float4 bb = *reinterpret_cast<const float4*>(hb_s);
                    const uint64_t di = ((uint64_t)ts * B + (uint64_t)min(m0 + fr, B - 1)) * E + 4 * i;
                    float4 tv;
                    tv.x = vag_tanh(hw.x + cw.x + e3.x + bb.x) * vag_drop_mul(a.rng, VAG_DROP_DEC_OUT, di + 0, a.p_out);
                    tv.y = vag_tanh(hw.y + cw.y + e3.y + bb.y) * vag_drop_mul(a.rng, VAG_DROP_DEC_OUT, di + 1, a.p_out);
                    tv.z = vag_tanh(hw.z + cw.z + e3.z + bb.z) * vag_drop_mul(a.rng, VAG_DROP_DEC_OUT, di + 2, a.p_out);
                    tv.w = vag_tanh(hw.w + cw.w + e3.w + bb.w) * vag_drop_mul(a.rng, VAG_DROP_DEC_OUT, di + 3, a.p_out);
                    if (m0 + fr < B) st_sc1_f4(a.tmid + ((int64_t)ts * B + m0 + fr) * E + 4 * i, tv);
                    asm volatile("s_waitcnt vmcnt(0)" ::: "memory");
                }
                if (tx == 0) arrive(c5 + ts * CNT_WORDS, i);
                wait_count(c5 + ts * CNT_WORDS, PER_SHARD, a.err, a.guard, a.spin, dead);
                VAG_STAMP(9);
                {
                    float4 ta[1], tb[1];
                    bf16x8 tf[3];
                    ld_rows_sc1<1>(a.tmid + ((int64_t)ts * B + lrow) * E + 32 * wave + 8 * (lane & 3), ta, tb);
                    split8(perm4(ta[0], src4), perm4(tb[0], src4), tf);
#pragma unroll
                    for (int pl = 0; pl < 3; ++pl) tm_s[(pl * 8 + wave) * 64 + lane] = tf[pl];
                }
                __syncthreads();
                unsigned long long best = 0ull;
                f32x4 acc = {0.f, 0.f, 0.f, 0.f};
                float* part_s = gi_s;
                auto finish_tile = [&](int j, const f32x4& t4) {
                    const int v0 = 16 * (i + 64 * j) + 4 * fg;
                    float lv[4] = {t4[0], t4[1], t4[2], t4[3]};
#pragma unroll
                    for (int q = 0; q < 4; ++q)
                        if (v0 + q < V) {
                            lv[q] += a.out_b[v0 + q];
                            const unsigned long long key = cand_key(lv[q], v0 + q);
                            best = key > best ? key : best;
                        }
                    if (a.logits && m0 + fr < B) {
                        float* lp = a.logits + ((int64_t)ts * B + m0 + fr) * a.ldl + v0;
                        if (v0 + 3 < V) *reinterpret_cast<float4*>(lp) = make_float4(lv[0], lv[1], lv[2], lv[3]);
                        else
                            for (int q = 0; q < 4; ++q) if (v0 + q < V) lp[q] = lv[q];
                    }
                };
                for (int g = 0; g < npass; ++g) {
                    const int k0 = g < 2 * nfull ? 4 * (g & 1) : (splitx ? 4 * (wave & 1) : 4 * (g - 2 * nfull));
#pragma unroll
                    for (int u = 0; u < 4; ++u) {
                        const float4 ca = wr[u][0], cb = wr[u][1];
                        if (g + 1 < npass) {
                            const float* wp = pass_ptr(g + 1, u);
                            wr[u][0] = *reinterpret_cast<const float4*>(wp); wr[u][1] = *reinterpret_cast<const float4*>(wp + 4);
                        }
                        bf16x8 aw[3], bw[3];
                        split8(ca, cb, aw);
#pragma unroll
                        for (int pl = 0; pl < 3; ++pl) bw[pl] = tm_s[(pl * 8 + k0 + u) * 64 + lane];
                        acc = mma6(aw, bw, acc);
                    }
                    if (g < 2 * nfull ? (g & 1) : (!splitx && g == npass - 1)) {
                        finish_tile(g < 2 * nfull ? wave + 8 * (g >> 1) : xj, acc);
                        acc = f32x4{0.f, 0.f, 0.f, 0.f};
                    }
                }
                if (splitx) {
                    if (xj >= 0 && (wave & 1)) *reinterpret_cast<f32x4*>(part_s + ((wave >> 1) * 64 + lane) * 4) = acc;
                    __syncthreads();
                    if (xj >= 0 && !(wave & 1)) finish_tile(xj, acc + *reinterpret_cast<const f32x4*>(part_s + ((wave >> 1) * 64 + lane) * 4));
                }
                VAG_STAMP(10);
                {
                    unsigned lo = (unsigned)best, hi = (unsigned)(best >> 32);
#pragma unroll
                    for (int o = 16; o <= 32; o <<= 1) {
                        const unsigned olo = __shfl_xor(lo, o, 64), ohi = __shfl_xor(hi, o, 64);
                        const unsigned long long ob = ((unsigned long long)ohi << 32) | olo;
                        if (ob > best) { best = ob; lo = olo; hi = ohi; }
                    }
                    if (lane < 16) cb_s[wave * 16 + lane] = best;
                }
                __syncthreads();
                if (tx < 16) {
                    unsigned long long b = 0ull;
#pragma unroll
                    for (int x = 0; x < 8; ++x) { const unsigned long long c = cb_s[16 * x + fr]; b = c > b ? c : b; }
                    if (m0 + fr < B)
                        __hip_atomic_store(a.cand + ((int64_t)ts * B + m0 + fr) * DEC_WGS + i, b, RLX_AGENT);
                    asm volatile("s_waitcnt vmcnt(0)" ::: "memory");
                }
                if (tx == 0) arrive(c6 + ts * CNT_WORDS, i);
                wait_count(c6 + ts * CNT_WORDS, PER_SHARD, a.err, a.guard, a.spin, dead);
                VAG_STAMP(11);
                if (tx < 128) {
                    const int r = tx >> 3, c0 = tx & 7;
                    const unsigned long long* cp = a.cand + ((int64_t)ts * B + min(m0 + r, B - 1)) * DEC_WGS + c0;
                    unsigned long long k[8];
#pragma unroll
                    for (int x = 0; x < 8; ++x) k[x] = __hip_atomic_load(cp + 8 * x, RLX_AGENT);
                    unsigned long long b = k[0];
#pragma unroll
                    for (int x = 1; x < 8; ++x) b = k[x] > b ? k[x] : b;
                    cb_s[tx] = b;
                }
                __syncthreads();
                if (tx < 16) {
                    unsigned long long b = 0ull;
#pragma unroll
                    for (int x = 0; x < 8; ++x) { const unsigned long long c = cb_s[fr * 8 + x]; b = c > b ? c : b; }
                    const int tk = min(max((int)(0xffffffffu - (unsigned)(b & 0xffffffffull)), 0), V - 1);
                    tok_s[fr] = tk;
                    if (i == 0 && m0 + fr < B) a.tok[(int64_t)t * B + m0 + fr] = tk;
                    e3 = *reinterpret_cast<const float4*>(a.embw3 + (int64_t)tk * E + 4 * i);
                }
                __syncthreads();
            }
            VAG_STAMP(12);
            if (t == Tt) break;

            if (eok) {
                const float* xp = a.embp + (int64_t)tok_s[fr] * 3 * H + eu;
#pragma unroll
                for (int g = 0; g < 3; ++g) xo[g] = *reinterpret_cast<const float4*>(xp + g * H);
            }
        }
        if (ep) {
            if (eok) {
                const float4 b0 = *reinterpret_cast<const float4*>(bs_s + 0 * 8 + 4 * hq), b1_ = *reinterpret_cast<const float4*>(bs_s + 1 * 8 + 4 * hq);
                const float4 b2_ = *reinterpret_cast<const float4*>(bs_s + 2 * 8 + 4 * hq);
                const float r_[4] = {cr.x + b0.x + xo[0].x, cr.y + b0.y + xo[0].y, cr.z + b0.z + xo[0].z, cr.w + b0.w + xo[0].w};
                const float z_[4] = {cz.x + b1_.x + xo[1].x, cz.y + b1_.y + xo[1].y, cz.z + b1_.z + xo[1].z, cz.w + b1_.w + xo[1].w};
                const float gh[4] = {cn.x + b2_.x, cn.y + b2_.y, cn.z + b2_.z, cn.w + b2_.w};
                const float xn[4] = {xo[2].x, xo[2].y, xo[2].z, xo[2].w};
                const float4 hprev = *reinterpret_cast<const float4*>(hs_s + 128 + fr * 8 + 4 * hq);
                const float hpv[4] = {hprev.x, hprev.y, hprev.z, hprev.w};
                float rr[4], zz[4], nn[4], ho[4];
#pragma unroll
                for (int q = 0; q < 4; ++q) {
                    rr[q] = vag_sigmoid(r_[q]);
                    zz[q] = vag_sigmoid(z_[q]);
                    nn[q] = vag_tanh(xn[q] + rr[q] * gh[q]);
                    ho[q] = (1.f - zz[q]) * nn[q] + zz[q] * hpv[q];
                }
                const float4 h1v = tag4(make_float4(ho[0], ho[1], ho[2], ho[3]));
                *reinterpret_cast<float4*>(hs_s + fr * 8 + 4 * hq) = h1v;
                const int64_t o = (int64_t)em * H + eu;
                st_sc1_f4(a.h1 + (int64_t)t * BH + o, h1v);
                if (!VAG_TAGGED) asm volatile("s_waitcnt vmcnt(0)" ::: "memory");
                if (VAG_TAGGED && tx == 0) arrive(c2 + t * CNT_WORDS, i);
                float* sv = a.g1 + (int64_t)t * 4 * BH + o;
                *reinterpret_cast<float4*>(sv) = make_float4(rr[0], rr[1], rr[2], rr[3]);
                *reinterpret_cast<float4*>(sv + BH) = make_float4(zz[0], zz[1], zz[2], zz[3]);
                *reinterpret_cast<float4*>(sv + 2 * BH) = make_float4(nn[0], nn[1], nn[2], nn[3]);
                *reinterpret_cast<float4*>(sv + 3 * BH) = make_float4(gh[0], gh[1], gh[2], gh[3]);
            }
            if (tx == 0 && (!VAG_TAGGED || !eok)) arrive(c2 + t * CNT_WORDS, i);
        }
        VAG_STAMP(2);
        wait_count(c2 + t * CNT_WORDS, PER_SHARD, a.err, a.guard, a.spin, dead);
        VAG_STAMP(3);
        ld_rows_tagged<KS>(a.h1 + ((int64_t)t * B + lrow) * H + kbase + 8 * (lane & 3), ha, hb, a.spin, dead, a.err, a.guard);
#pragma unroll
        for (int s = 0; s < KS; ++s) { ha[s] = perm4(ha[s], src4); hb[s] = perm4(hb[s], src4); }
        bf16x8 hf2[KS][3];
        {
            f32x4 acc = {0.f, 0.f, 0.f, 0.f};
#pragma unroll
            for (int s = 0; s < KS; ++s) {
                split8(ha[s], hb[s], hf2[s]);
                acc = mma6(w2[s][0], hf2[s], acc);
            }
            red[(wave * 3 + 0) * 64 + lane] = make_float4(acc[0], acc[1], acc[2], acc[3]);
        }
        __syncthreads();
        if (wave == 0) {
            float4 qv = make_float4(0, 0, 0, 0);
#pragma unroll
            for (int w = 0; w < 8; ++w) {
                const float4 x0 = red[(w * 3 + 0) * 64 + lane];
                qv.x += x0.x; qv.y += x0.y; qv.z += x0.z; qv.w += x0.w;
            }
            if (m0 + fr < B) *reinterpret_cast<float4*>(a.qhp + ((int64_t)t * B + m0 + fr) * Q + 16 * i + 4 * fg) = qv;
            *reinterpret_cast<float4*>(q_s + fr * 16 + 4 * fg) = qv;
        }
        __syncthreads();
        {
            const int cq = tx & 3;
            const float4 vq = *reinterpret_cast<const float4*>(v_s + 16 * i + 4 * cq);
            for (int P = tx >> 2; P < 16 * Ts; P += 128) {
                const int r = P / Ts;
                const float4 pv = reinterpret_cast<const float4*>(pe_s)[P * 4 + cq];
                const float4 qq = *reinterpret_cast<const float4*>(q_s + r * 16 + 4 * cq);
                float acc = vq.x * vag_tanh(pv.x + qq.x) + vq.y * vag_tanh(pv.y + qq.y) + vq.z * vag_tanh(pv.z + qq.z) +
                            vq.w * vag_tanh(pv.w + qq.w);
                acc = quad_sum(acc);
                if (cq == 0 && m0 + r < B)
                    atomicAdd(a.psc + (((int64_t)t * ACC_SHARDS + (i & (ACC_SHARDS - 1))) * B + m0 + r) * Ts + (P - r * Ts), acc);
            }
        }
        {
            f32x4 acc[2] = {{0.f, 0.f, 0.f, 0.f}, {0.f, 0.f, 0.f, 0.f}};
#pragma unroll
            for (int s = 0; s < KS; ++s) {
                acc[0] = mma6(w2[s][1], hf2[s], acc[0]);
                acc[1] = mma6(w2[s][2], hf2[s], acc[1]);
            }
            red[(wave * 3 + 1) * 64 + lane] = make_float4(acc[0][0], acc[0][1], acc[0][2], acc[0][3]);
            red[(wave * 3 + 2) * 64 + lane] = make_float4(acc[1][0], acc[1][1], acc[1][2], acc[1][3]);
        }
        VAG_STAMP(4);
        asm volatile("s_waitcnt vmcnt(0)" ::: "memory");
        __syncthreads();
        if (tx == 0) arrive(c4 + t * CNT_WORDS, i);
        VAG_STAMP(5);
        if (ep) {
            float4 hp2[3] = {make_float4(0, 0, 0, 0), make_float4(0, 0, 0, 0), make_float4(0, 0, 0, 0)};
#pragma unroll
            for (int w = 0; w < 8; ++w) {
                const float4 x0 = red[(w * 3 + 1) * 64 + hq * 16 + fr], x1 = red[(w * 3 + 1) * 64 + (2 + hq) * 16 + fr];
                const float4 x2 = red[(w * 3 + 2) * 64 + hq * 16 + fr];
                hp2[0].x += x0.x; hp2[0].y += x0.y; hp2[0].z += x0.z; hp2[0].w += x0.w;
                hp2[1].x += x1.x; hp2[1].y += x1.y; hp2[1].z += x1.z; hp2[1].w += x1.w;
                hp2[2].x += x2.x; hp2[2].y += x2.y; hp2[2].z += x2.z; hp2[2].w += x2.w;
            }
#pragma unroll
            for (int g = 0; g < 3; ++g) {
                const float4 bb = *reinterpret_cast<const float4*>(bs_s + 24 + g * 8 + 4 * hq);
                hp2[g].x += bb.x; hp2[g].y += bb.y; hp2[g].z += bb.z; hp2[g].w += bb.w;
                *reinterpret_cast<float4*>(hp_s + fr * 24 + g * 8 + 4 * hq) = hp2[g];
                if (eok) *reinterpret_cast<float4*>(a.qhp + ((int64_t)t * B + em) * Q + C + g * H + eu) = hp2[g];
            }
        }
        VAG_STAMP(6);
        wait_count(c4 + t * CNT_WORDS, PER_SHARD, a.err, a.guard, a.spin, dead);
        VAG_STAMP(7);
        for (int x0 = tx; x0 < 16 * Ts; x0 += 1024) {
            const int x1 = x0 + 512;
            const int r0 = x0 / Ts, r1 = min(x1, 16 * Ts - 1) / Ts;
            const float* p0 = a.psc + ((int64_t)t * ACC_SHARDS * B + min(m0 + r0, B - 1)) * Ts + (x0 - r0 * Ts);
            const float* p1 = a.psc + ((int64_t)t * ACC_SHARDS * B + min(m0 + r1, B - 1)) * Ts + (min(x1, 16 * Ts - 1) - r1 * Ts);
            float v0, v1;
            ld_acc_shards(p0, p1, (int64_t)B * Ts, v0, v1);
            sc_s[x0] = mk_s[x0] == 0.f ? -INFINITY : v0;
            if (x1 < 16 * Ts) sc_s[x1] = mk_s[x1] == 0.f ? -INFINITY : v1;
        }
        __syncthreads();
        for (int r = wave; r < 16; r += 8) {
            float mx = -INFINITY;
            for (int sp = lane; sp < Ts; sp += 64) mx = fmaxf(mx, sc_s[r * Ts + sp]);
            mx = wave_max(mx);
            float sum = 0.f;
            for (int sp = lane; sp < Ts; sp += 64) sum += __expf(sc_s[r * Ts + sp] - mx);
            sum = wave_sum(sum);
            const float inv = 1.f / sum;
            for (int sp = lane; sp < Ts; sp += 64) {
                const float al = __expf(sc_s[r * Ts + sp] - mx) * inv;
                sc_s[r * Ts + sp] = al;
                if (((r * Ts + sp) & (WGS - 1)) == i && m0 + r < B) a.alpha[((int64_t)t * B + m0 + r) * Ts + sp] = al;
            }
        }
        __syncthreads();
        if (tx < 16 * 24) {
            const int r = tx / 24, col = tx - r * 24;
            const float* al = sc_s + r * Ts;
            const float* ew = ew_s + (int64_t)r * Ts * 24 + col;
            float s0 = 0.f, s1 = 0.f;
            int sp = 0;
            for (; sp + 1 < Ts; sp += 2) { s0 += al[sp] * ew[sp * 24]; s1 += al[sp + 1] * ew[(sp + 1) * 24]; }
            if (sp < Ts) s0 += al[sp] * ew[sp * 24];
            gi_s[tx] = s0 + s1;
        } else if (FREE && tx < 16 * 24 + 64) {
            const int x = tx - 16 * 24, r = x >> 2, col = x & 3;
            const float* al = sc_s + r * Ts;
            const float* ew = ew2_s + (int64_t)r * Ts * 4 + col;
            float s0 = 0.f, s1 = 0.f;
            int sp = 0;
            for (; sp + 1 < Ts; sp += 2) { s0 += al[sp] * ew[sp * 4]; s1 += al[sp + 1] * ew[(sp + 1) * 4]; }
            if (sp < Ts) s0 += al[sp] * ew[sp * 4];
            cw_s[x] = s0 + s1;
        }
        __syncthreads();
        if (eok) {
            float gi[3][4];
#pragma unroll
            for (int g = 0; g < 3; ++g) {
                const float4 x = *reinterpret_cast<const float4*>(gi_s + fr * 24 + g * 8 + 4 * hq);
                gi[g][0] = x.x; gi[g][1] = x.y; gi[g][2] = x.z; gi[g][3] = x.w;
            }
            float bi[3][4], hh[3][4];
#pragma unroll
            for (int g = 0; g < 3; ++g) {
                const float4 x = *reinterpret_cast<const float4*>(bs_s + 48 + g * 8 + 4 * hq);
                const float4 y = *reinterpret_cast<const float4*>(hp_s + fr * 24 + g * 8 + 4 * hq);
                bi[g][0] = x.x; bi[g][1] = x.y; bi[g][2] = x.z; bi[g][3] = x.w;
                hh[g][0] = y.x; hh[g][1] = y.y; hh[g][2] = y.z; hh[g][3] = y.w;
            }
            const float* hr = hh[0];
            const float* hz = hh[1];
            const float* hn = hh[2];
            const float4 h1v = *reinterpret_cast<const float4*>(hs_s + fr * 8 + 4 * hq);
            const float h1a[4] = {h1v.x, h1v.y, h1v.z, h1v.w};
            float rr[4], zz[4], nn[4], ho[4];
#pragma unroll
            for (int q = 0; q < 4; ++q) {
                rr[q] = vag_sigmoid(gi[0][q] + bi[0][q] + hr[q]);
                zz[q] = vag_sigmoid(gi[1][q] + bi[1][q] + hz[q]);
                nn[q] = vag_tanh(gi[2][q] + bi[2][q] + rr[q] * hn[q]);
                ho[q] = (1.f - zz[q]) * nn[q] + zz[q] * h1a[q];
            }
            const float4 h2v = tag4(make_float4(ho[0], ho[1], ho[2], ho[3]));
            *reinterpret_cast<float4*>(hs_s + 128 + fr * 8 + 4 * hq) = h2v;
            const int64_t o = (int64_t)em * H + eu;
            st_sc1_f4(a.h2_all + (int64_t)t * BH + o, h2v);
            if (!VAG_TAGGED) asm volatile("s_waitcnt vmcnt(0)" ::: "memory");
            if (VAG_TAGGED && tx == 0) arrive(c1 + t * CNT_WORDS, i);
            float* sv = a.g2 + (int64_t)t * 4 * BH + o;
            *reinterpret_cast<float4*>(sv) = make_float4(rr[0], rr[1], rr[2], rr[3]);
            *reinterpret_cast<float4*>(sv + BH) = make_float4(zz[0], zz[1], zz[2], zz[3]);
            *reinterpret_cast<float4*>(sv + 2 * BH) = make_float4(nn[0], nn[1], nn[2], nn[3]);
            *reinterpret_cast<float4*>(sv + 3 * BH) = make_float4(hn[0], hn[1], hn[2], hn[3]);
        }
        if (tx == 0 && (!VAG_TAGGED || !eok)) arrive(c1 + t * CNT_WORDS, i);
    }
#ifdef VAG_LAB
    if (!FREE && a.dbg && threadIdx.x == 0 && i == 0 && rt < 8) a.dbg[(Tt + 2) * 8 + rt] = __builtin_amdgcn_s_memrealtime();
#endif
#undef VAG_STAMP
}

struct DecBArgs {
    const float *pe, *encwp, *v, *wcatT, *whh1T;
    const float *h0, *h2_all, *h1, *g1, *g2, *qhp, *alpha;
    const float *d_h2_all, *dah;
    float *dgi2, *dqgh, *ds, *dgi1, *dgh1, *d_h0;
    float* dal;
    unsigned* cnt;
    unsigned* err;
    unsigned* guard;
    unsigned spin;
    unsigned long long* dbg;
    int B, Ts, Tt, H, RT;
    int rt0;
    int xcd_map;
    int h0_tanh;
    char *pl_dq, *pl_dgh1;
    char *pl_dgh2, *pl_w2;
};

__device__ __forceinline__ void cell_bwd4(const float (&dh)[4], const float4 (&sv)[4], const float4 hp, float (&gi)[3][4],
                                          float (&gh)[3][4], float (&direct)[4]) {
    const float r_[4] = {sv[0].x, sv[0].y, sv[0].z, sv[0].w}, z_[4] = {sv[1].x, sv[1].y, sv[1].z, sv[1].w};
    const float n_[4] = {sv[2].x, sv[2].y, sv[2].z, sv[2].w}, hn[4] = {sv[3].x, sv[3].y, sv[3].z, sv[3].w};
    const float hpv[4] = {hp.x, hp.y, hp.z, hp.w};
#pragma unroll
    for (int q = 0; q < 4; ++q) {
        const float dn_pre = dh[q] * (1.f - z_[q]) * (1.f - n_[q] * n_[q]);
        const float dz_pre = dh[q] * (hpv[q] - n_[q]) * z_[q] * (1.f - z_[q]);
        const float dr_pre = dn_pre * hn[q] * r_[q] * (1.f - r_[q]);
        gi[0][q] = dr_pre; gi[1][q] = dz_pre; gi[2][q] = dn_pre;
        gh[0][q] = dr_pre; gh[1][q] = dz_pre; gh[2][q] = dn_pre * r_[q];
        direct[q] = dh[q] * z_[q];
    }
}

template <int WGS, int PLM>
__global__ __launch_bounds__(512, 1) void dec_bwd_persistent_kernel(DecBArgs a) {
    extern __shared__ __attribute__((aligned(16))) float dlds[];
    constexpr bool PL = (PLM & 1) != 0, PL2 = (PLM & 2) != 0;
    static_assert(PL || !PL2, "the hidden side's planes come with the hand-off planes");
    constexpr int H = WGS * DEC_U, C = 2 * H, Q = C + 3 * H;
    constexpr unsigned PER_SHARD = WGS / SHARDS;
    int i, rt;
    dec_slice_map<WGS>(a.xcd_map, a.rt0, i, rt);
    const int lane = threadIdx.x & 63, wave = threadIdx.x >> 6;
    const int B = a.B, Ts = a.Ts, Tt = a.Tt;
#ifdef VAG_LAB
#define VAG_BPSTAMP(k) do { if (a.dbg && blockIdx.x == 0 && threadIdx.x == 0) a.dbg[Tt * 8 + (k)] = __builtin_amdgcn_s_memrealtime(); } while (0)
#else
#define VAG_BPSTAMP(k) do { } while (0)
#endif
    VAG_BPSTAMP(0);
    const int m0 = rt * 16, u0 = i * DEC_U;
    const int fr = lane & 15, fg = lane >> 4;
    const int64_t BH = (int64_t)B * H;
    const int NP = 16 * Ts;
    float4* red = reinterpret_cast<float4*>(dlds);
    float* pe_s = dlds + 2048;
    float* ew_t = pe_s + NP * 16;
    float* da_s = ew_t + 24 * NP;
    float* al_s = da_s + NP;
    float* gi_s = al_s + NP;
    float* d1_s = gi_s + 384;
    float* pb_s = d1_s + 128;
    float* c1_s = pb_s + 128;
    float* dq_s = c1_s + 128;
    float* wb_s = dq_s + 256;
    constexpr int WBLD = C + 4;

    constexpr int KB = C / 8 / 32, KC = 3 * H / 8 / 32;
    bf16x8 wc[KC][3];
    {
        const float* pc = a.whh1T + (int64_t)(u0 + (fr & 7)) * (3 * H) + wave * (3 * H >> 3) + 8 * fg;
#pragma unroll
        for (int s = 0; s < KC; ++s) split8(*reinterpret_cast<const float4*>(pc + 32 * s), *reinterpret_cast<const float4*>(pc + 32 * s + 4), wc[s]);
    }
// ... 482 lines not shown
    for (int rt0 = 0; rt0 < RT; rt0 += tpp) launch(rt0, std::min(tpp, RT - rt0));
}
static int enc_tiles_per_pass(int64_t H) {
    const int cus = persist_cu_count();
    return (H == 256 || H == 512 || H == 1024) ? (int)(cus / (2 * (H / 16))) : 0;
}
static bool passes_ok(int64_t rt, int tpp, int max_passes) {
    if (tpp <= 0 || rt > (int64_t)tpp * max_passes) return false;
    return rt <= tpp || 4 * (rt - tpp * ((rt - 1) / tpp)) >= 3 * tpp;
}
bool vag_enc_persistent_ok(int64_t B, int64_t Ts, int64_t H) {
    if (!(H == 256 || H == 512 || H == 1024) || B <= 0 || Ts <= 0) return false;
    return passes_ok(cdiv64(B, 16), enc_tiles_per_pass(H), 2) && persist_lds_ok(84 * 1024) && (int64_t)(Ts + 1) * B * H * 4 < (1ll << 31);
}
int64_t vag_enc_persistent_sync_words(int64_t B, int64_t Ts) { return 2 * cdiv64(B, 16) * Ts + 64; }

int vag_enc_fwd_persistent_launch(const float* xp, const float* w_fw, const float* w_bw, const float* b_fw, const float* b_bw,
                                  const int* lengths, float* hst, float* gates, float* enc, float* planes, int64_t planes_floats,
                                  unsigned* sync, const uint64_t* rng, float p_ctx, int64_t B, int64_t Ts, int64_t H, hipStream_t s) {
    VAG_CHECK_ARG(xp && w_fw && w_bw && b_fw && b_bw && lengths && hst && gates && enc && sync && vag_enc_persistent_ok(B, Ts, H));
    VAG_CHECK_ARG(aligned16(xp) && aligned16(w_fw) && aligned16(w_bw) && aligned16(b_fw) && aligned16(b_bw) && aligned16(hst) &&
                  aligned16(gates) && aligned16(enc) && aligned16(planes));
    const int64_t pl_need = vag_enc_fwd_planes_floats(B, Ts, H);
    const bool pl = planes && (vag_opt().handoff_planes & 4) && pl_need > 0 && planes_floats >= pl_need;
    EncPArgs a;
    a.pl = pl ? reinterpret_cast<char*>(planes) : nullptr;
    a.xp = xp; a.W[0] = w_fw; a.W[1] = w_bw; a.bias[0] = b_fw; a.bias[1] = b_bw; a.lengths = lengths;
    a.hst = hst; a.gates = gates; a.enc = enc; a.rng = rng; a.p_ctx = p_ctx;
    a.B = (int)B; a.Ts = (int)Ts; a.H = (int)H; a.RT = (int)cdiv64(B, 16); a.CS = (int)(H / 16);
    VAG_TRY(sync_begin(a, sync, vag_enc_persistent_sync_words(B, Ts), s));
    {
        PTimerScope timed(0, s);
        row_tile_passes(a.RT, enc_tiles_per_pass(H), [&](int rt0, int tiles) {
            a.rt0 = rt0; a.RTP = tiles;
            const dim3 grid((unsigned)(2 * a.RTP * a.CS));
            if (H == 256 && pl) hipLaunchKernelGGL((enc_fwd_persistent_kernel<1, true>), grid, dim3(512), 0, s, a);
            else if (H == 256) hipLaunchKernelGGL((enc_fwd_persistent_kernel<1, false>), grid, dim3(512), 0, s, a);
            else if (H == 512 && pl) hipLaunchKernelGGL((enc_fwd_persistent_kernel<2, true>), grid, dim3(512), 0, s, a);
            else if (H == 512) hipLaunchKernelGGL((enc_fwd_persistent_kernel<2, false>), grid, dim3(512), 0, s, a);
            else if (pl) hipLaunchKernelGGL((enc_fwd_persistent_kernel<4, true>), grid, dim3(512), 0, s, a);
            else hipLaunchKernelGGL((enc_fwd_persistent_kernel<4, false>), grid, dim3(512), 0, s, a);
        });
    }
    VAG_LAUNCH_CHECK();
    return VAG_OK;
}

constexpr int DEC_MAX_PASSES = 2;
static int64_t dec_persistent_lds_bytes(int64_t Ts, bool free_run = false) {
    return 4 * (6144 + 16 * Ts * 16 + 16 * Ts * 24 + 16 * Ts + 16 * 24 + 16 * 24 + 80 + 256 + 1024 + 16 * Ts + 256 +
                (free_run ? 64 + 16 + 16 + 16 * Ts * 4 : 0));
}
static int dec_wgs(int64_t H) { return (int)(H / DEC_U); }
static int dec_tiles_per_pass(int64_t H) {
    const int cus = persist_cu_count();
    return (H == 256 || H == 512) ? cus / dec_wgs(H) : 0;
}
bool vag_dec_persistent_ok(int64_t B, int64_t Ts, int64_t Tt, int64_t H) {
    if ((H != 512 && H != 256) || B <= 0 || Ts <= 0 || Tt <= 0 || Ts > 512) return false;
    const int tpp = dec_tiles_per_pass(H);
    if (!passes_ok(cdiv64(B, 16), tpp, DEC_MAX_PASSES)) return false;
    return dec_persistent_lds_bytes(Ts) <= 160 * 1024 && persist_lds_ok(160 * 1024);
}
int64_t vag_dec_persistent_sync_words(int64_t B, int64_t Tt) { return 5 * cdiv64(B, 16) * Tt * CNT_WORDS + 64; }

static DecPArgs dec_fwd_args(const float* pe, const float* mask, const float* h0, const float* xp1, const float* W1, const float* b1,
                             const float* wcat, const float* bcat, const float* v, const float* encwp, const float* b_ih2, float* h1,
                             float* g1, float* qhp, float* alpha, float* h2_all, float* g2, float* psc, int64_t B, int64_t Ts,
                             int64_t Tt, int64_t H) {
    DecPArgs a = {};
    a.pe = pe; a.mask = mask; a.h0 = h0; a.xp1 = xp1; a.W1 = W1; a.b1 = b1; a.wcat = wcat; a.bcat = bcat; a.v = v; a.encwp = encwp;
    a.b_ih2 = b_ih2; a.h1 = h1; a.g1 = g1; a.qhp = qhp; a.alpha = alpha; a.h2_all = h2_all; a.g2 = g2; a.psc = psc;
    a.B = (int)B; a.Ts = (int)Ts; a.Tt = (int)Tt; a.H = (int)H; a.RT = (int)cdiv64(B, 16);
    a.xcd_map = vag_opt().dec_xcd_map & 15;
#ifdef VAG_LAB
    a.dbg = reinterpret_cast<unsigned long long*>(vag_opt().dec_stamps);
#else
    a.dbg = nullptr;
#endif
    return a;
}
static int dec_fwd_zero(DecPArgs& a, unsigned* sync, hipStream_t s) {
    VAG_TRY(sync_begin(a, sync, vag_dec_persistent_sync_words(a.B, a.Tt), s, a.psc, a.Tt * a.B * a.Ts * ACC_SHARDS));
    if (VAG_TAGGED && !vag_ctx().persist_prezeroed) {
        const int nh = a.Tt * a.B * a.H;
        hipLaunchKernelGGL(zero2_u32_kernel, dim3((unsigned)cdiv64(2 * (int64_t)nh, 256)), dim3(256), 0, s,
                           reinterpret_cast<unsigned*>(a.h1), nh, reinterpret_cast<unsigned*>(a.h2_all), nh);
        VAG_LAUNCH_CHECK();
    }
    return VAG_OK;
}

int vag_dec_fwd_persistent_launch(const float* pe, const float* mask, const float* h0, const float* xp1, const float* W1,
                                  const float* b1, const float* wcat, const float* bcat, const float* v, const float* encwp,
                                  const float* b_ih2, float* h1, float* g1, float* qhp, float* alpha, float* h2_all, float* g2,
                                  float* psc, unsigned* sync, int64_t B, int64_t Ts, int64_t Tt, int64_t H, hipStream_t s) {
    VAG_CHECK_ARG(pe && mask && h0 && xp1 && W1 && b1 && wcat && bcat && v && encwp && b_ih2 && h1 && g1 && qhp && alpha && h2_all &&
                  g2 && psc && sync && vag_dec_persistent_ok(B, Ts, Tt, H));
    VAG_CHECK_ARG(aligned16(pe) && aligned16(h0) && aligned16(xp1) && aligned16(W1) && aligned16(b1) && aligned16(wcat) &&
                  aligned16(bcat) && aligned16(v) && aligned16(encwp) && aligned16(b_ih2) && aligned16(h1) && aligned16(g1) &&
                  aligned16(qhp) && aligned16(h2_all) && aligned16(g2));
    DecPArgs a = dec_fwd_args(pe, mask, h0, xp1, W1, b1, wcat, bcat, v, encwp, b_ih2, h1, g1, qhp, alpha, h2_all, g2, psc, B, Ts, Tt, H);
    VAG_TRY(dec_fwd_zero(a, sync, s));
    int64_t lds = dec_persistent_lds_bytes(Ts);
    if (lds < 84 * 1024) lds = 84 * 1024;
    if (!max_lds_once<dec_fwd_persistent_kernel<false, 64>>()) return VAG_EINVAL;
    if (H == 256 && !max_lds_once<dec_fwd_persistent_kernel<false, 32>>()) return VAG_EINVAL;
    {
        PTimerScope timed(1, s);
        row_tile_passes(a.RT, dec_tiles_per_pass(H), [&](int rt0, int tiles) {
            a.rt0 = rt0;
            if (H == 512) hipLaunchKernelGGL((dec_fwd_persistent_kernel<false, 64>), dim3(tiles * 64u), dim3(512), (size_t)lds, s, a);
            else hipLaunchKernelGGL((dec_fwd_persistent_kernel<false, 32>), dim3(tiles * 32u), dim3(512), (size_t)lds, s, a);
        });
    }
    VAG_LAUNCH_CHECK();
    return VAG_OK;
}

bool vag_dec_free_persistent_ok(int64_t B, int64_t Ts, int64_t Tt, int64_t E, int64_t H, int64_t V) {
    if (H != 512 || E != DEC_E || B <= 0 || B > 64 || Ts <= 0 || Tt <= 0 || Ts > 512 || V < 16 || V >= (1ll << 30)) return false;
    const int cus = persist_cu_count();
    return cdiv64(B, 16) * DEC_WGS <= cus && dec_persistent_lds_bytes(Ts, true) <= 160 * 1024 && persist_lds_ok(160 * 1024);
}
DecTables vag_dec_tables(float* base, int64_t B, int64_t Ts, int64_t Tt, int64_t E, int64_t H, int64_t V, bool token_only) {
    WsCarver c(base);
    DecTables t = {};
    t.embp = c.take(V * 3 * H); t.embw3 = c.take(V * E);
    if (!token_only) { t.encw2 = c.take(B * Ts * E); t.cand = c.take_as<unsigned long long>(Tt * B * DEC_WGS); }
    t.total = c.off;
    return t;
}
int vag_dec_free_persistent_launch(const float* pe, const float* mask, const float* h0, const float* W1, const float* b1,
                                   const float* wcat, const float* bcat, const float* v, const float* encwp, const float* b_ih2,
                                   float* h1, float* g1, float* qhp, float* alpha, float* h2_all, float* g2, float* psc,
                                   unsigned* sync, const DecTables& tab, const float* hw1, const float* hb1, const float* hb2,
                                   const float* hb3, const float* out_w, const float* out_b, float* tmid, float* logits, int64_t ldl,
                                   int64_t* tok, const uint64_t* rng, float p_out, int64_t B, int64_t Ts, int64_t Tt, int64_t E,
                                   int64_t H, int64_t V, hipStream_t s) {
    const float* tables = tab.embp;
    VAG_CHECK_ARG(pe && mask && h0 && W1 && b1 && wcat && bcat && v && encwp && b_ih2 && h1 && g1 && qhp && alpha && h2_all && g2 &&
                  psc && sync && tables && hw1 && hb1 && hb2 && hb3 && out_w && out_b && tmid && tok &&
                  vag_dec_free_persistent_ok(B, Ts, Tt, E, H, V));
    VAG_CHECK_ARG(aligned16(pe) && aligned16(h0) && aligned16(W1) && aligned16(b1) && aligned16(wcat) && aligned16(bcat) &&
                  aligned16(v) && aligned16(encwp) && aligned16(b_ih2) && aligned16(h1) && aligned16(g1) && aligned16(qhp) &&
                  aligned16(h2_all) && aligned16(g2) && aligned16(tables) && aligned16(hw1) && aligned16(out_w) && aligned16(tmid));
    VAG_CHECK_ARG(!logits || (aligned16(logits) && ldl >= V && ldl % 4 == 0));
    DecPArgs a = dec_fwd_args(pe, mask, h0, nullptr, W1, b1, wcat, bcat, v, encwp, b_ih2, h1, g1, qhp, alpha, h2_all, g2, psc, B, Ts, Tt, H);
    a.embp = tab.embp; a.embw3 = tab.embw3; a.encw2 = tab.encw2; a.cand = tab.cand;
    a.hw1 = hw1; a.hb1 = hb1; a.hb2 = hb2; a.hb3 = hb3; a.out_w = out_w; a.out_b = out_b; a.tmid = tmid; a.logits = logits;
    a.tok = tok; a.rng = rng; a.p_out = p_out; a.V = (int)V; a.ldl = (int)ldl;
    VAG_TRY(dec_fwd_zero(a, sync, s));
    int64_t lds = dec_persistent_lds_bytes(Ts, true);
    if (lds < 84 * 1024) lds = 84 * 1024;
    if (!max_lds_once<dec_fwd_persistent_kernel<true>>()) return VAG_EINVAL;
    {
        PTimerScope timed(1, s);
        hipLaunchKernelGGL(dec_fwd_persistent_kernel<true>, dim3((unsigned)(a.RT * DEC_WGS)), dim3(512), (size_t)lds, s, a);
    }
    VAG_LAUNCH_CHECK();
    return VAG_OK;
}

bool vag_enc_wide16_ok(int64_t B, int64_t Ts, int64_t H) {
    if (!(H == 512 || H == 1024) || B < 1 || Ts < 1) return false;
    const int64_t wgs = 2 * cdiv64(B, 64) * (H / 32);
    if (wgs > persist_cu_count() || !persist_lds_ok(160 * 1024)) return false;
    return 2 * cdiv64(B, 64) * Ts + 64 <= vag_enc_persistent_sync_words(B, Ts);
}
int vag_enc_fwd_wide16_launch(const float* xp, const vag_half* w16_fw, const vag_half* w16_bw, const float* b_fw, const float* b_bw,
                              const int* lengths, float* hst, float* gates, float* enc, vag_half* hx, unsigned* sync, const uint64_t* rng,
                              float p_ctx, int64_t B, int64_t Ts, int64_t H, hipStream_t s) {
    VAG_CHECK_ARG(xp && w16_fw && w16_bw && b_fw && b_bw && lengths && hst && gates && enc && hx && sync &&
                  vag_enc_wide16_ok(B, Ts, H));
    VAG_CHECK_ARG(aligned16(xp) && aligned16(w16_fw) && aligned16(w16_bw) && aligned16(b_fw) && aligned16(b_bw) && aligned16(hst) &&
                  aligned16(gates) && aligned16(enc) && aligned16(hx));
    EncWArgs a;
    a.xp = xp; a.W16[0] = w16_fw; a.W16[1] = w16_bw; a.bias[0] = b_fw; a.bias[1] = b_bw; a.lengths = lengths;
    a.hst = hst; a.gates = gates; a.enc = enc; a.hx = hx; a.rng = rng; a.p_ctx = p_ctx;
    a.B = (int)B; a.Ts = (int)Ts; a.H = (int)H; a.RG = (int)cdiv64(B, 64); a.CS = (int)(H / 32);
    VAG_TRY(sync_begin(a, sync, vag_enc_persistent_sync_words(B, Ts), s));
    const size_t lds = 96 * 1024;
    if (!max_lds_once<enc_fwd_wide16_kernel<4>>() || !max_lds_once<enc_fwd_wide16_kernel<8>>()) return VAG_EINVAL;
    const dim3 grid((unsigned)(2 * a.RG * a.CS));
    {
        PTimerScope timed(0, s);
        if (H == 512) hipLaunchKernelGGL(enc_fwd_wide16_kernel<4>, grid, dim3(512), lds, s, a);
        else hipLaunchKernelGGL(enc_fwd_wide16_kernel<8>, grid, dim3(512), lds, s, a);
    }
    VAG_LAUNCH_CHECK();
    return VAG_OK;
}

int vag_enc_bwd_wide16_launch(const vag_half* wt16, const float* d_enc, const float* gates, const float* hst, const int* lengths,
                              const uint64_t* rng, float p_ctx, float* d_xp, float* dgh, vag_half* gx, unsigned* sync, int64_t B,
                              int64_t Ts, int64_t H, hipStream_t s) {
    VAG_CHECK_ARG(wt16 && d_enc && gates && hst && lengths && d_xp && dgh && gx && sync && vag_enc_wide16_ok(B, Ts, H));
    VAG_CHECK_ARG(aligned16(wt16) && aligned16(d_enc) && aligned16(gates) && aligned16(hst) && aligned16(d_xp) && aligned16(dgh) &&
                  aligned16(gx));
    EncWBArgs a;
    a.WT16[0] = wt16; a.WT16[1] = wt16 + 3 * H * H; a.d_enc = d_enc; a.gates = gates; a.hst = hst; a.lengths = lengths;
    a.rng = rng; a.p_ctx = p_ctx; a.d_xp = d_xp; a.dgh = dgh; a.gx = gx;
    a.B = (int)B; a.Ts = (int)Ts; a.H = (int)H; a.RG = (int)cdiv64(B, 64); a.CS = (int)(H / 32);
    VAG_TRY(sync_begin(a, sync, vag_enc_persistent_sync_words(B, Ts), s));
    const size_t lds = 84 * 1024;
    if (!max_lds_once<enc_bwd_wide16_kernel<6>>() || !max_lds_once<enc_bwd_wide16_kernel<12>>()) return VAG_EINVAL;
    const dim3 grid((unsigned)(2 * a.RG * a.CS));
    {
        PTimerScope timed(2, s);
        if (H == 512) hipLaunchKernelGGL(enc_bwd_wide16_kernel<6>, grid, dim3(512), lds, s, a);
        else hipLaunchKernelGGL(enc_bwd_wide16_kernel<12>, grid, dim3(512), lds, s, a);
    }
    VAG_LAUNCH_CHECK();
    return VAG_OK;
}

int vag_enc_bwd_persistent_launch(const float* whhT, const float* d_enc, const float* gates, const float* hst, const int* lengths,
                                  const uint64_t* rng, float p_ctx, float* d_xp, float* dgh, float* planes, unsigned* sync, int64_t B,
                                  int64_t Ts, int64_t H, hipStream_t s) {
    VAG_CHECK_ARG(whhT && d_enc && gates && hst && lengths && d_xp && dgh && sync && (H == 512 || H == 256) && vag_enc_persistent_ok(B, Ts, H));
    VAG_CHECK_ARG(aligned16(whhT) && aligned16(d_enc) && aligned16(gates) && aligned16(hst) && aligned16(d_xp) && aligned16(dgh) && aligned16(planes));
    const bool pl = planes && (vag_opt().handoff_planes & 1) && vag_enc_bwd_planes_floats(B, Ts, H) > 0;
    EncBArgs a;
    a.WT[0] = whhT; a.WT[1] = whhT + 3 * H * H; a.d_enc = d_enc; a.gates = gates; a.hst = hst; a.lengths = lengths;
    a.rng = rng; a.p_ctx = p_ctx; a.d_xp = d_xp; a.dgh = dgh; a.pl = reinterpret_cast<char*>(planes);
    a.B = (int)B; a.Ts = (int)Ts; a.H = (int)H; a.RT = (int)cdiv64(B, 16); a.CS = (int)(H / 16);
    VAG_TRY(sync_begin(a, sync, vag_enc_persistent_sync_words(B, Ts), s));
    {
        PTimerScope timed(2, s);
        row_tile_passes(a.RT, enc_tiles_per_pass(H), [&](int rt0, int tiles) {
            a.rt0 = rt0; a.RTP = tiles;
            const dim3 grid((unsigned)(2 * a.RTP * a.CS));
            if (H == 512 && pl) hipLaunchKernelGGL((enc_bwd_persistent_kernel<6, true>), grid, dim3(512), 0, s, a);
            else if (H == 512) hipLaunchKernelGGL((enc_bwd_persistent_kernel<6, false>), grid, dim3(512), 0, s, a);
            else if (pl) hipLaunchKernelGGL((enc_bwd_persistent_kernel<3, true>), grid, dim3(512), 0, s, a);
            else hipLaunchKernelGGL((enc_bwd_persistent_kernel<3, false>), grid, dim3(512), 0, s, a);
        });
    }
    VAG_LAUNCH_CHECK();
    return VAG_OK;
}

unsigned* vag_persist_guard(void) {
    if (vag_ctx().guard) return vag_ctx().guard;
    void* p = nullptr;
    if (hipGetSymbolAddress(&p, HIP_SYMBOL(g_persist_guard)) != hipSuccess) { (void)hipGetLastError(); return nullptr; }
    return reinterpret_cast<unsigned*>(p);
}
int vag_persistent_timeouts_read(void) {
    unsigned v = 0, z = 0;
    const unsigned zz[2] = {0u, 0u};
    if (hipMemcpyFromSymbol(&v, HIP_SYMBOL(g_persist_timeouts), sizeof(v)) != hipSuccess) return -1;
    if (v != 0 && (hipMemcpyToSymbol(HIP_SYMBOL(g_persist_timeouts), &z, sizeof(z)) != hipSuccess ||
                   hipMemcpyToSymbol(HIP_SYMBOL(g_persist_guard), zz, sizeof(zz)) != hipSuccess)) return -1;
    return (int)v;
}

static int64_t dec_bwd_persistent_lds_bytes(int64_t Ts, int64_t H = 512) {
    const int64_t NP = 16 * Ts;
    return 4 * (2048 + NP * 16 + 24 * NP + 2 * NP + 384 + 3 * 128 + 256 + 8 * (2 * H + 4) + 64);
}
static bool pl_any_device_takes(int64_t rt, int tpp_max) {
    for (int tpp = 1; tpp <= tpp_max; ++tpp)
        if (passes_ok(rt, tpp, DEC_MAX_PASSES)) return true;
    return false;
}
constexpr int PL_MAX_CUS = 256;
int64_t vag_enc_bwd_planes_floats(int64_t B, int64_t Ts, int64_t H) {
    if ((H != 512 && H != 256) || B <= 0 || Ts <= 0 || !pl_any_device_takes(cdiv64(B, 16), (int)(PL_MAX_CUS / (2 * (H / 16))))) return 0;
    return 2 * Ts * cdiv64(B, 16) * pl_block_bytes(3 * H) / 4;
}
int64_t vag_enc_fwd_planes_floats(int64_t B, int64_t Ts, int64_t H) {
    if ((H != 1024 && H != 512 && H != 256) || B <= 0 || Ts <= 0 || !pl_any_device_takes(cdiv64(B, 16), (int)(PL_MAX_CUS / (2 * (H / 16))))) return 0;
    return 2 * Ts * cdiv64(B, 16) * pl_block_bytes(H) / 4;
}
static int64_t dec_bwd_handoff_floats(int64_t B, int64_t Tt, int64_t H) {
    if ((H != 512 && H != 256) || B <= 0 || Tt <= 0 || !pl_any_device_takes(cdiv64(B, 16), PL_MAX_CUS / dec_wgs(H))) return 0;
    return Tt * cdiv64(B, 16) * (pl_block_bytes(2 * H) + pl_block_bytes(3 * H)) / 4;
}
static int64_t dec_bwd_hidden_floats(int64_t B, int64_t Tt, int64_t H, int64_t tiles_per_pass) {
    const int64_t RT = cdiv64(B, 16);
    return (Tt * RT * pl_block_bytes(3 * H) + std::min(RT, tiles_per_pass) * dec_wgs(H) * pl_w2_bytes(H)) / 4;
}
int64_t vag_dec_bwd_planes_floats(int64_t B, int64_t Tt, int64_t H) {
    const int64_t base = dec_bwd_handoff_floats(B, Tt, H);
    return base > 0 ? base + dec_bwd_hidden_floats(B, Tt, H, PL_MAX_CUS / dec_wgs(H)) : 0;
}
bool vag_dec_bwd_persistent_ok(int64_t B, int64_t Ts, int64_t Tt, int64_t H) {
    return vag_dec_persistent_ok(B, Ts, Tt, H) && dec_bwd_persistent_lds_bytes(Ts, H) <= 160 * 1024;
}
int vag_dec_bwd_persistent_launch(const float* pe, const float* encwp, const float* v, const float* wcatT, const float* whh1T,
                                  const float* h0, const float* h2_all, const float* h1, const float* g1, const float* g2,
                                  const float* qhp, const float* alpha, const float* d_h2_all, const float* dah, float* dgi2,
                                  float* dqgh, float* ds, float* dgi1, float* dgh1, float* d_h0, float* dal, float* planes,
                                  int64_t planes_floats, unsigned* sync, int64_t B, int64_t Ts, int64_t Tt, int64_t H, hipStream_t s) {
    VAG_CHECK_ARG(pe && encwp && v && wcatT && whh1T && h0 && h2_all && h1 && g1 && g2 && qhp && alpha && d_h2_all && dah && dgi2 &&
                  dqgh && ds && dgi1 && dgh1 && d_h0 && dal && sync && vag_dec_bwd_persistent_ok(B, Ts, Tt, H));
    VAG_CHECK_ARG(aligned16(pe) && aligned16(encwp) && aligned16(wcatT) && aligned16(whh1T) && aligned16(h0) && aligned16(h2_all) &&
                  aligned16(h1) && aligned16(g1) && aligned16(g2) && aligned16(qhp) && aligned16(d_h2_all) && aligned16(dgi2) &&
                  aligned16(dqgh) && aligned16(dgi1) && aligned16(dgh1) && aligned16(d_h0) && aligned16(planes));
    const int64_t pl_base = dec_bwd_handoff_floats(B, Tt, H);
    const int64_t pl_hid = dec_bwd_hidden_floats(B, Tt, H, dec_tiles_per_pass(H));
    const int plopt = vag_opt().handoff_planes;
    const bool pl = planes && (plopt & 1) && pl_base > 0 && planes_floats >= pl_base;
    const bool pl2 = pl && (plopt & 2) && planes_floats >= vag_dec_bwd_planes_floats(B, Tt, H) && planes_floats >= pl_base + pl_hid;
    DecBArgs a;
    a.pe = pe; a.encwp = encwp; a.v = v; a.wcatT = wcatT; a.whh1T = whh1T; a.h0 = h0; a.h2_all = h2_all; a.h1 = h1; a.g1 = g1;
    a.g2 = g2; a.qhp = qhp; a.alpha = alpha; a.d_h2_all = d_h2_all; a.dah = dah; a.dgi2 = dgi2; a.dqgh = dqgh; a.ds = ds;
    a.dgi1 = dgi1; a.dgh1 = dgh1; a.d_h0 = d_h0; a.dal = dal;
    VagCallCtx::Dh0Tanh& dh0 = vag_ctx().dh0_tanh;
    a.h0_tanh = dh0.req ? 1 : 0;
    if (dh0.req) dh0.done = d_h0;
    dh0.req = false;
#ifdef VAG_LAB
    a.dbg = reinterpret_cast<unsigned long long*>(vag_opt().dec_bwd_stamps);
#else
    a.dbg = nullptr;
#endif
    a.B = (int)B; a.Ts = (int)Ts; a.Tt = (int)Tt; a.H = (int)H; a.RT = (int)cdiv64(B, 16);
    a.pl_dq = reinterpret_cast<char*>(planes);
    a.pl_dgh1 = a.pl_dq ? a.pl_dq + Tt * a.RT * pl_block_bytes(2 * H) : nullptr;
    a.pl_dgh2 = pl2 ? a.pl_dq + pl_base * 4 : nullptr;
    a.pl_w2 = pl2 ? a.pl_dgh2 + Tt * a.RT * pl_block_bytes(3 * H) : nullptr;
    a.xcd_map = vag_opt().dec_xcd_map >> 4;
    VAG_TRY(sync_begin(a, sync, vag_dec_persistent_sync_words(B, Tt), s, dal, (int)(Tt * B * Ts) * ACC_SHARDS));
    int64_t lds = dec_bwd_persistent_lds_bytes(Ts, H);
    if (lds < 84 * 1024) lds = 84 * 1024;
    const int form = pl2 ? 3 : pl ? 1 : 0;
    bool lds_ok = false;
    void (*kern)(DecBArgs) = nullptr;
#define VAG_DEC_BWD_FORM(W, F) do { lds_ok = max_lds_once<dec_bwd_persistent_kernel<W, F>>(); kern = dec_bwd_persistent_kernel<W, F>; } while (0)
    if (H == 512) { if (form == 3) VAG_DEC_BWD_FORM(64, 3); else if (form == 1) VAG_DEC_BWD_FORM(64, 1); else VAG_DEC_BWD_FORM(64, 0); }
    else { if (form == 3) VAG_DEC_BWD_FORM(32, 3); else if (form == 1) VAG_DEC_BWD_FORM(32, 1); else VAG_DEC_BWD_FORM(32, 0); }
#undef VAG_DEC_BWD_FORM
    if (!lds_ok) return VAG_EINVAL;
    {
        PTimerScope timed(3, s);
        row_tile_passes(a.RT, dec_tiles_per_pass(H), [&](int rt0, int tiles) {
            a.rt0 = rt0;
            hipLaunchKernelGGL(kern, dim3(tiles * (unsigned)dec_wgs(H)), dim3(512), (size_t)lds, s, a);
        });
    }
    VAG_LAUNCH_CHECK();
    return VAG_OK;
}
```

vag-nmt_amd/csrc/step.hip:

```cpp
#include "../../include/vag_nmt.h"
#include <vector>
#include "kernels.h"

#define S_(x) reinterpret_cast<hipStream_t>(x)

namespace {

struct StepWs {
    float *enc, *mask, *ws_enc, *pe;
    float *y_im, *nrm_im, *im_emb, *ws_img, *alpha_v, *ctx, *y_txt, *nrm_txt, *txt_emb, *rscores, *G;
    float *xmix, *hseq, *c_all, *e_all, *ws_dec, *tmid, *logits, *lse, *nll, *inv_cnt, *consts;
    int64_t* tok;
    float *d_enc, *d_pe, *d_h2, *d_c, *d_e, *d_h0, *d_ctx, *d_im, *d_txt, *scr_dec, *scr_head, *scr_ini;
    float* free_tab;
    float* gemm_slab;
    unsigned* gemm_ticket;
    int64_t gemm_slab_floats, gemm_tickets;
    int64_t total;
};

StepWs step_ws(float* p, const vag_step_cfg& c) {
    StepWs w;
    const int64_t B = c.B, Ts = c.Ts, Tt = c.Tt, H = c.H, C = 2 * c.H, S = c.S, R = c.Tt * c.B;
    WsCarver cv(p);
// ... 145 lines not shown
        f = fork_state();
        if (!f) return main;
        if (hipEventRecord(f->ev[slot], main) != hipSuccess || hipStreamWaitEvent(f->side, f->ev[slot], 0) != hipSuccess) {
            (void)hipGetLastError();
            return main;
        }
        open = true;
        return f->side;
    }
    int join(hipStream_t main, int slot) {
        if (!open) return VAG_OK;
        open = false;
        if (hipEventRecord(f->ev[slot], f->side) != hipSuccess || hipStreamWaitEvent(main, f->ev[slot], 0) != hipSuccess)
            return (int)hipGetLastError();
        return VAG_OK;
    }
};
}

static int train_step(const vag_step_cfg* cfg, const vag_kd_cfg* kd, const vag_rdrop_cfg* rd, const vag_model_w* wp,
                      const vag_model_g* gp, const int64_t* src, const int32_t* lengths, const int64_t* tgt, const float* im, const float* vocab_weight, uint64_t* rng,
                      const float* derived, float* ws, float* losses, int phases, vag_stream_t stream) {
    hipStream_t s = S_(stream);
    VAG_CHECK_ARG(cfg_ok(cfg) && wp && gp && src && lengths && tgt && vocab_weight && ws && losses && aligned16(ws));
    const vag_step_cfg& c = *cfg;
    const vag_model_w& w = *wp;
    const vag_model_g& g = *gp;
    const bool mm = c.multimodal != 0;
    VAG_CHECK_ARG(!mm || (im && w.im_w && w.im_b && w.txt_w && w.txt_b && w.ctx2ctx && w.emb2ctx &&
                          (c.attn_method == 0 || w.mlp_w)));
    VAG_CHECK_ARG(w.enc_emb && w.ini_w && w.ini_b && w.attn_e && (phases & 55) != 0 && (phases & ~55) == 0);
    const int64_t B = c.B, Ts = c.Ts, Tt = c.Tt, H = c.H, C = 2 * H, S = c.S, V = c.V, Et = c.Et;
    StepWs k = step_ws(ws, c);
    VAG_CHECK_ARG(c.storage == 0 || (c.storage == 1 && derived && !c.free_run && H % 8 == 0));
    int64_t chunk = 0;
    if (!c.free_run && (double)c.Tt * (double)c.B * (double)c.ldl * 4.0 > 1073741824.0) {
        chunk = (int64_t)(671088640.0 / ((double)c.ldl * 4.0)) / c.B * c.B;
        if (chunk < c.B) chunk = c.B;
    }
    if (vag_opt().head_chunk >= 0)
        chunk = c.free_run ? 0 : vag_opt().head_chunk;
    VagCallCtx ctx = vag_ctx();
    ctx.derived = derived;
    ctx.store16 = c.storage == 1;
    ctx.gemm_planes = ctx.store16 ? 2 : 3;
    const bool mrt = c.mrt_n > 0;
    if (c.guard) ctx.guard = reinterpret_cast<unsigned*>(c.guard);
    ctx.persist_prezeroed = true;
    ctx.step_zeroed = true;
    VagCallScope scope(ctx);
    const VagCallCtx::GemmScratch slabs = {k.gemm_slab, k.gemm_slab_floats, k.gemm_ticket, k.gemm_tickets, s};
    if (!(phases & 1)) ctx.gemm_scratch = slabs;
    const bool head_finish_in_fwd = chunk > 0 && (phases & 1) && (phases & (2 | 16)) && vag_opt().head_fuse != 0 && !mrt;
    const bool has_vse = mm && c.rank_kind >= 0;
    const float w_mt = mm ? c.loss_w : 1.f, w_vse = mm ? 1.f - c.loss_w : 0.f;
    float* h0 = k.hseq;
    float* h2_all = k.hseq + B * H;
    const uint64_t* crng = rng;
    float* d_e = vag_cgru_bwd_scratch_de(k.scr_dec, B, Ts, Tt, Et, H);
    HeadSeq head;
    head.B = B; head.Tt = Tt; head.E = Et; head.H = H; head.V = V; head.ldl = c.ldl;
    head.p_out = c.p_out; head.rng = crng; head.eps = c.label_smoothing;
    head.h2 = h2_all; head.c = k.c_all; head.e = k.e_all; head.w = w.head;
    head.tgt = tgt; head.vocab_weight = vocab_weight; head.logits_ready = c.free_run ? 1 : 0;
    head.tmid = k.tmid; head.logits = k.logits; head.lse = k.lse; head.nll = k.nll; head.inv_cnt = k.inv_cnt;
    head.losses = losses; head.w_mt = w_mt; head.w_vse = w_vse; head.has_vse = has_vse ? 1 : 0; head.ring = c.loss_ring;
    head.d_loss = k.consts + 0; head.d_h2 = k.d_h2; head.d_c = k.d_c; head.d_e = d_e; head.g = g.head; head.dt = k.scr_head;
    head.inv_cnt_ready = true; head.chunk = chunk; head.finish_in_fwd = head_finish_in_fwd;
    if (mrt) head.mrt = {c.mrt_n, c.mrt_alpha, c.mrt_scale, c.mrt_cost, c.mrt_valid};
    if (kd) head.kd = {kd->k, kd->lambda, kd->idx, kd->q};
    if (rd) head.rd = {rd->alpha, rd->kl};
    head.s = s;
    const bool one_plane = c.storage == 1 && !c.free_run && vag_opt().s16_one_plane != 0;
    StepBranch br_im, br_leaf, br_dw;
    if (phases & 1) {
        if (one_plane) ctx.gemm_planes = 11;
        if (mm) {
            hipStream_t si = br_im.fork(s, 0, 1);
            VAG_TRY(vag_img_proj_l2_fwd(im, w.im_w, w.im_b, B, c.I, S, c.activation_vse, k.y_im, k.nrm_im, k.im_emb, si));
        }
        {
            unsigned* zp[3];
            int64_t zn[3];
            vag_step_zero_ranges(k.ws_enc, k.ws_dec, B, Ts, Tt, c.Es, Et, H, zp, zn);
            int64_t nb = cdiv64((Tt + 1) * B, 256);
            if (nb < cdiv64(zn[1], 1024)) nb = cdiv64(zn[1], 1024);
            if (nb > 1024) nb = 1024;
            ZeroRanges zr;
            zr.p[0] = reinterpret_cast<uint4*>(h2_all); zr.n[0] = Tt * B * H / 4;
            zr.p[1] = reinterpret_cast<uint4*>(k.tmid); zr.n[1] = Tt * B * Et / 4;
            zr.p[2] = reinterpret_cast<uint4*>(zp[2]); zr.n[2] = zn[2] / 4;
            zr.p[3] = reinterpret_cast<uint4*>(k.scr_head); zr.n[3] = chunk > 0 ? 0 : Tt * B * Et / 4;
            zr.p[4] = reinterpret_cast<uint4*>(vag_cgru_bwd_scratch_du(k.scr_dec, B, Ts, Tt, Et, H)); zr.n[4] = Tt * B * H / 4;
            zr.p[5] = reinterpret_cast<uint4*>(k.gemm_ticket); zr.n[5] = k.gemm_tickets / 4;
            GatherTask ga = {nullptr, nullptr, 0};
            if (!c.free_run) { ga.emb = w.dec.emb; ga.out = k.e_all; ga.E4 = (int)(Et / 4); }
            hipLaunchKernelGGL(step_prologue_kernel, dim3((unsigned)nb), dim3(256), 0, s, rng, tgt, (int)B, (int)Tt, k.tok,
                               k.consts, k.inv_cnt, w_mt, w_vse, zp[0], zn[0], zp[1], zn[1], zr, ga);
            VAG_LAUNCH_CHECK();
            if (ga.out) ctx.step_gathered = true;
        }
        ctx.gemm_scratch = slabs;
        VAG_TRY(vag_bigru_seq_fwd(src, lengths, w.enc_emb, w.enc_fw, w.enc_bw, c.p_emb, c.p_ctx, crng, B, Ts, c.Es, H, k.enc,
                                  k.mask, k.ws_enc, stream));
        if (mm) {
            VAG_TRY(br_im.join(s, 1));
            ctx.row_mix = {k.xmix, c.init_split, nullptr};
            const int rc_att = vag_imagine_attn_ctx_fwd(k.im_emb, k.enc, k.mask, w.ctx2ctx, w.emb2ctx, w.mlp_w, c.attn_method, B, Ts, C, S,
                                                        k.alpha_v, k.ctx, k.ws_img, stream);
            ctx.row_mix.xmix = nullptr;
            VAG_TRY(rc_att);
            VAG_TRY(vag_img_proj_l2_fwd(k.ctx, w.txt_w, w.txt_b, B, C, S, c.activation_vse, k.y_txt, k.nrm_txt, k.txt_emb,
                                        stream));
            if (has_vse)
                VAG_TRY(vag_rank_loss_fwd_impl(k.im_emb, k.txt_emb, B, S, c.margin, c.rank_kind | (rd ? 2 : 0), k.rscores, k.G,
                                               losses + 2, k.consts + 1, s, rd ? 0.25f : 1.f));
        }
        VAG_TRY(vag_dec_init_fwd(k.enc, k.mask, mm ? k.ctx : nullptr, mm ? c.init_split : 0.f, w.ini_w, w.ini_b, B, Ts, C, H,
                                 k.xmix, h0, stream));
        {
            VagGemmGroup outer(derived != nullptr);
            VAG_TRY(vag_attn_keys_proj(k.enc, w.attn_e, B * Ts, C, k.pe, stream));
            if (c.free_run && vag_cgru_free_supported(B, Ts, Tt, Et, H, V))
                VAG_TRY(vag_cgru_attn_decode_free_fwd(k.enc, k.pe, k.mask, h0, k.tok, w.dec, B, Ts, Tt, Et, H, V, h2_all, k.c_all,
                                                      k.e_all, k.ws_dec, &w.head, c.p_out, crng, k.tmid, k.logits, c.ldl,
                                                      k.free_tab, stream));
            else
            VAG_TRY(vag_cgru_attn_decode_seq_fwd(k.enc, k.pe, k.mask, h0, k.tok, w.dec, B, Ts, Tt, Et, H, V, h2_all, k.c_all,
                                                 k.e_all, k.ws_dec, c.free_run, &w.head, c.p_out, crng, k.tmid, k.logits,
                                                 c.ldl, stream));
            VAG_TRY(outer.end(s));
        }
        if ((phases & (2 | 16)) && chunk == 0 && vag_opt().loss_ride != 0 && !mrt && !rd) ctx.loss_defer.on = true;
        VAG_TRY(vag_head_seq_fwd(head));
    }
    if (one_plane && (phases & 54)) ctx.gemm_planes = 1;
    if (phases & (2 | 16)) {
        if (chunk == 0) ctx.gemm_prezeroed[0] = k.scr_head;
        ctx.gemm_prezeroed[1] = vag_cgru_bwd_scratch_du(k.scr_dec, B, Ts, Tt, Et, H);
        VAG_TRY(vag_head_seq_bwd(head));
        VAG_TRY(vag_loss_defer_flush());
        {
            VagGemmGroup outer(true);
            ForkState* dw_side = (phases & 4) && (phases & (2 | 32)) && (vag_opt().step_fork & 4) ? fork_state() : nullptr;
            if (dw_side) ctx.leaf_stream = {dw_side->side, dw_side->ev[4], false};
            ctx.dh0_tanh.req = (phases & 2) != 0;
            VAG_TRY(vag_cgru_attn_decode_seq_bwd_loop(k.enc, k.pe, k.mask, h0, k.tok, w.dec, B, Ts, Tt, Et, H, V, h2_all, k.c_all,
                                                      k.e_all, k.d_h2, k.d_c, d_e, k.ws_dec, k.d_enc, 0, k.d_pe, k.d_h0,
                                                      k.scr_dec, stream));
            VAG_TRY(vag_attn_keys_proj_bwd(k.enc, w.attn_e, k.d_pe, B * Ts, C, k.d_enc, 1, g.attn_e, stream));
            VAG_TRY(vag_cgru_attn_decode_seq_bwd_weights(h0, k.tok, w.dec, B, Ts, Tt, Et, H, h2_all, k.c_all, k.e_all, d_e,
                                                         k.ws_dec, g.dec, k.scr_dec, stream));
            VAG_TRY(outer.end(s));
            if (dw_side && ctx.leaf_stream.used) { br_dw.f = dw_side; br_dw.open = true; }
            ctx.leaf_stream.stream = nullptr; ctx.leaf_stream.event = nullptr;
            ctx.dh0_tanh.req = false;
        }
    }
    if (phases & (2 | 32)) {
        ctx.leaf_on = vag_opt().leaf_queue != 0;
        ctx.rmw = RmwDefer();
        ctx.rmw.out = k.d_enc;
        if (mm) {
            if (has_vse) {
                VAG_TRY(vag_rank_loss_bwd_impl(k.im_emb, k.txt_emb, k.G, nullptr, B, S, k.d_im, k.d_txt, s));
            } else {
                VAG_TRY(vag_axpy_launch(0.f, k.d_im, k.d_im, B * S, 2, s));
                VAG_TRY(vag_axpy_launch(0.f, k.d_txt, k.d_txt, B * S, 2, s));
            }
            VAG_TRY(vag_img_proj_l2_bwd(k.ctx, w.txt_w, k.y_txt, k.nrm_txt, k.txt_emb, k.d_txt, B, C, S, c.activation_vse,
                                        k.d_ctx, g.txt_w, g.txt_b, stream));
        }
// ... 54 lines not shown
```

vag-nmt_amd/vagnmt_hip/_lib.py:

```python
import ctypes as C
import os
import subprocess

import torch

_HERE = os.path.dirname(os.path.abspath(__file__))
PKG_ROOT = os.path.dirname(_HERE)
CSRC = os.path.join(PKG_ROOT, "csrc")
LIB_PATH = os.environ.get("VAG_LIB") or os.path.join(PKG_ROOT, "lib", "libvagnmt.so")

P = C.c_void_p
I64 = C.c_int64
I32 = C.c_int
F = C.c_float


class GruW(C.Structure):
    _fields_ = [("w_ih", P), ("w_hh", P), ("b_ih", P), ("b_hh", P)]


class DecW(C.Structure):
    _fields_ = [("emb", P), ("gru1", GruW), ("attn_h", P), ("attn_v", P), ("c2h", P), ("gru2", GruW)]


# ... 113 lines not shown
    "vag_imagine_attn_ctx_bwd": (I32, [P, P, P, P, P, P, I32, I64, I64, I64, I64, P, P, P, P, I32, P, P, P, P, P]),
    "vag_rank_loss_fwd": (I32, [P, P, I64, I64, F, I32, P, P, P, P]),
    "vag_rank_loss_bwd": (I32, [P, P, P, P, I64, I64, P, P, P]),
    "vag_gather_rows_i64": (I32, [P, I64, P, I64, I64, P, P]),
    "vag_retrieval_ranks": (I32, [P, P, I64, I64, P, P, P]),
    "vag_dec_init_fwd": (I32, [P, P, P, F, P, P, I64, I64, I64, I64, P, P, P]),
    "vag_dec_init_bwd": (I32, [P, P, P, F, P, P, I64, I64, I64, I64, P, I32, P, P, P, P, P]),
    "vag_beam_scratch_bytes": (I64, [I64, I64, I64, I64]),
    "vag_beam_step": (I32, [P, I64, P, P, I64, I64, P, P, I64, I64, I64, I64, P, P, P]),
    "vag_beam_step_dev": (I32, [P, I64, P, P, P, I64, P, P, P, I64, I64, I64, I64, P, P, P]),
    "vag_head_logits_parts_count": (I64, [HeadW, I64, I64, I64]),
    "vag_head_logits_step": (I32, [P, P, P, HeadW, I64, I64, I64, I64, P, I64, P, P, P]),
    "vag_beam_step_logits_dev": (I32, [P, I64, P, I64, P, P, P, I64, P, P, P, I64, I64, I64, I64, P, P, P]),
    "vag_beam_finish": (I32, [P, P, I64, I64, I64, I64, P, P, P]),
    "vag_ens_max_models": (I32, []),
    "vag_beam_ens_step": (I32, [P, P, I64, P, P, I64, I64, P, P, P, I64, I64, I64, P, P, P]),
    "vag_beam_ens_step_dev": (I32, [P, P, I64, P, P, P, I64, P, P, P, P, I64, I64, I64, P, P, P]),
    "vag_ens_argmax": (I32, [P, P, I64, I64, I64, P, P]),
    "vag_beam_step_opt": (I32, [P, I64, P, P, I64, I64, P, P, I64, I64, I64, I64, P, P, I32, P]),
    "vag_beam_step_dev_opt": (I32, [P, I64, P, P, P, I64, P, P, P, I64, I64, I64, I64, P, P, I32, P]),
    "vag_beam_step_logits_dev_opt": (I32, [P, I64, P, I64, P, P, P, I64, P, P, P, I64, I64, I64, I64, P, P, I32, P]),
    "vag_beam_ens_step_opt": (I32, [P, P, I64, P, P, I64, I64, P, P, P, I64, I64, I64, P, P, I32, P]),
    "vag_beam_ens_step_dev_opt": (I32, [P, P, I64, P, P, P, I64, P, P, P, P, I64, I64, I64, P, P, I32, P]),
    "vag_beam_finish_nbest": (I32, [P, P, I64, I64, I64, I64, I64, P, P, P]),
    "vag_beam_finish_nbest_slots": (I32, [P, P, I64, I64, I64, I64, I64, P, P, P, P]),
    "vag_beam_div_scratch_bytes": (I64, [I64, I64, I64, I64]),
    "vag_beam_div_step": (I32, [P, P, I64, P, P, I64, I64, P, P, P, I64, I64, I64, P, P, I32, I64, F, P]),
    "vag_beam_div_step_dev": (I32, [P, P, I64, P, P, P, I64, P, P, P, P, I64, I64, I64, P, P, I32, I64, F, P]),
    "vag_beam_req_scratch_bytes": (I64, [I64, I64, I64, I64]),
    "vag_beam_req_step": (I32, [P, P, I64, P, P, I64, I64, P, P, P, I64, I64, I64, P, P, I32, P, P, P]),
    "vag_beam_req_step_dev": (I32, [P, P, I64, P, P, P, I64, P, P, P, P, I64, I64, I64, P, P, I32, P, P, P]),
    "vag_beam_sbs_scratch_bytes": (I64, [I64, I64, I64, I64]),
    "vag_beam_sbs_step": (I32, [P, P, I64, P, P, I64, I64, P, P, P, I64, I64, I64, P, P, I32, P, P, P]),
    "vag_beam_sbs_step_dev": (I32, [P, P, I64, P, P, P, I64, P, P, P, P, I64, I64, I64, P, P, I32, P, P, P]),
    "vag_beam_pen_scratch_bytes": (I64, [I64, I64, I64, I64]),
    "vag_beam_cover": (I32, [P, I64, P, P, P, I64, I64, I64, I64, I64, F, P, P, P]),
    "vag_beam_cover_dev": (I32, [P, I64, P, P, P, P, I64, I64, I64, I64, F, P, P, P]),
    "vag_beam_pen_step": (I32, [P, P, I64, P, P, I64, I64, P, P, P, I64, I64, I64, P, P, I32, P, P, P, P, P, I64, P, P, I32, P]),
    "vag_beam_pen_step_dev": (I32, [P, P, I64, P, P, P, I64, P, P, P, P, I64, I64, I64, P, P, I32, P, P, P, P, P, I64, P, P, I32,
                                    P]),
    "vag_beam_finish_pen": (I32, [P, P, P, P, P, P, I64, I64, I64, I64, I64, P, P, P, P, P, P, P]),
    "vag_beam_constrain": (I32, [P, P, I64, P, I64, I64, I64, I64, I64, P, I64, P, P, I64, I64, P]),
    "vag_beam_constrain_dev": (I32, [P, P, I64, P, P, I64, I64, I64, I64, P, I64, P, P, I64, I64, P]),
    "vag_forced_score": (I32, [P, P, P, I64, P, I64, I64, I64, P, P, P, P]),
    "vag_token_conf": (I32, [P, P, P, I64, P, I64, I64, I64, P, P, P, P, P, P, P]),
    "vag_beam_attn_record": (I32, [P, I64, P, I64, I64, I64, I64, I64, P]),
    "vag_beam_attn_record_dev": (I32, [P, I64, P, P, I64, I64, I64, I64, P]),
    "vag_beam_finish_align": (I32, [P, P, P, I64, I64, I64, I64, I64, I64, I64, P, P, P, P, P]),
    "vag_forced_align": (I32, [P, I64, P, I64, I64, I64, P, P, P]),
    "vag_sample_step": (I32, [P, P, I64, P, P, I64, I64, P, P, P, P, I64, I64, I64, F, I64, P, P, P]),
    "vag_sample_step_dev": (I32, [P, P, I64, P, P, P, I64, P, I64, I64, I64, F, I64, P, P, P]),
    "vag_sample_step_p": (I32, [P, P, I64, P, P, I64, I64, P, P, P, P, I64, I64, I64, F, I64, P, P, F, P, P]),
    "vag_sample_step_p_dev": (I32, [P, P, I64, P, P, P, I64, P, I64, I64, I64, F, I64, P, P, F, P, P]),
    "vag_sample_noise": (I32, [P, I64, I64, I64, P, P]),
    "vag_mbr_supported": (I32, [I64, I64, I64, I64]),
    "vag_mbr_select": (I32, [P, P, P, I64, I64, I64, I64, I64, I32, P, P, P, P, P]),
    "vag_corpus_bleu_supported": (I32, [I64, I64, I64]),
    "vag_corpus_bleu_stats": (I32, [P, P, P, I64, I64, I64, I64, P, P, P]),
    "vag_surface_expand": (I32, [P, I64, I64, P, P, I64, P, I64, P, P]),
    "vag_chrf_supported": (I32, [I64, I64, I64, I64]),
    "vag_chrf_max_chars": (I32, []),
    "vag_chrf_select": (I32, [P, P, P, P, P, I64, I64, I64, I64, I64, P, P, P, P, P]),
    "vag_mrt_weights": (I32, [P, P, P, I64, I64, I64, F, F, P, P, P, P]),
    "vag_mrt_pack": (I32, [P, I64, I64, I64, P, I64, I32, P, I64, P, P]),
    "vag_clip_adam_flat": (I32, [P, P, P, P, I64, I32, C.POINTER(I64), C.POINTER(F), C.POINTER(F), F, F, F, F, F, I32, P,
                                 P, P, P, P]),
    "vag_clip_adam_flat_ema": (I32, [P, P, P, P, I64, I32, C.POINTER(I64), C.POINTER(F), C.POINTER(F), F, F, F, F, F, I32, P,
                                     P, P, P, P, F, I32, P]),
    "vag_swap_flat": (I32, [P, P, I64, P]),
    "vag_clip_adam_shard": (I32, [P, P, P, P, I64, I32, C.POINTER(I64), C.POINTER(F), C.POINTER(F), F, F, F, F, F, I32, P,
                                  P, P, P, I64, I64, I32, P, P]),
    "vag_step_ws_floats": (I64, [StepCfgArg]),
    "vag_step_ws_offset": (I64, [StepCfgArg, I32]),
    "vag_train_step": (I32, [StepCfgArg, C.POINTER(ModelW), C.POINTER(ModelW), P, P, P, P, P, P, P, P, P, I32, P]),
    "vag_step_kd_check": (I32, [StepCfgArg, C.POINTER(KdCfg)]),
    "vag_train_step_kd": (I32, [StepCfgArg, C.POINTER(KdCfg), C.POINTER(ModelW), C.POINTER(ModelW), P, P, P, P, P, P, P, P, P, I32, P]),
    "vag_step_rdrop_check": (I32, [StepCfgArg, C.POINTER(RdropCfg)]),
    "vag_train_step_rdrop": (I32, [StepCfgArg, C.POINTER(RdropCfg), C.POINTER(ModelW), C.POINTER(ModelW), P, P, P, P, P, P, P, P, P, I32,
                                   P]),
    "vag_copy4": (I32, [C.POINTER(P), C.POINTER(P), C.POINTER(I64), I32, P]),
    "vag_set_operator_context": (I32, [P, I32]),
    "vag_set_option": (I32, [C.c_char_p, I64]),
    "vag_handoff_planes_floats": (I64, [I64, I64, I64, I64]),
    "vag_set_handoff_planes": (I32, [P, I64]),
    "vag_recurrence_supported": (I32, [I32, I64, I64, I64, I64]),
    "vag_persistent_timeouts": (I32, []),
    "vag_set_operator_guard": (I32, [P]),
    "vag_recurrence_time": (I32, [I32, P, P]),
    "vag_gemm_group_plan": (I32, [I32, P, P, P, P, P, P]),
    "vag_gemm_plan": (I32, [I64, I64, I64, I32, I32, I32, F, I32, I32, I32, I32, I32, P]),
    "vag_comm_unique_id": (I32, [P]),
    "vag_comm_init": (I32, [P, I32, I32, P]),
    "vag_comm_allreduce": (I32, [P, P, I64, P]),
    "vag_comm_size": (I32, [P]),
    "vag_comm_destroy": (I32, [P]),
    "vag_recurrence_sync_words": (I64, [I32, I64, I64]),
    "vag_cgru_recurrence_fwd": (I32, [P, P, P, P, DecW, P, P, P, I64, I64, I64, I64, P, P, P, P, P, P, P, P, P]),
    "vag_derived_floats": (I64, [I64]),
    "vag_derive_weights": (I32, [DecW, P, P, I64, I32, P, P]),
    "vag_cgru_ws_offset": (I64, [I64, I64, I64, I64, I64, I32]),
    "vag_dropout_mask": (I32, [P, I32, I64, F, P, P]),
    "vag_rng_advance": (I32, [P, P]),
}

_lib = None


def use_lab_build():
    global LIB_PATH
    assert _lib is None, "use_lab_build() must come before the library is loaded"
    r = subprocess.run(["make", "-C", CSRC, "-j8", "LAB=1"], capture_output=True, text=True)
    if r.returncode != 0:
        raise RuntimeError("building libvagnmt_lab.so failed:\n" + r.stderr[-2000:])
    LIB_PATH = os.path.join(os.path.dirname(LIB_PATH), "libvagnmt_lab.so")
    return LIB_PATH


def build(verbose=False):
    r = subprocess.run(["make", "-C", CSRC, "-j8"], capture_output=True, text=True)
    if verbose or r.returncode != 0:
        print(r.stdout[-4000:])
        print(r.stderr[-4000:])
    if r.returncode != 0:
        raise RuntimeError("building libvagnmt.so failed")
    return LIB_PATH


def lib():
    global _lib
    if _lib is None:
        if not os.path.exists(LIB_PATH):
            raise RuntimeError(
                "libvagnmt.so not found at %s: build it with `make -C %s` (or __graft_entry__.build()). "
                "There is no CPU fallback for the VAG-NMT hot path." % (LIB_PATH, CSRC))
        L = C.CDLL(LIB_PATH)
        for name, (res, args) in PROTOS.items():
            fn = getattr(L, name)
            fn.restype = res
            fn.argtypes = args
        _lib = L
    return _lib


class VagError(RuntimeError):
    pass


def check(rc, what=""):
    if rc != 0:
        kind = "argument/shape error" if rc < 0 else "hipError_t"
        raise VagError("libvagnmt %s failed: %s %d" % (what, kind, rc))


def stream():
    return C.c_void_p(torch.cuda.current_stream().cuda_stream)


class capture:
    _streams = {}

    def __init__(self, graph, pool=None):
        self._graph = graph
        self._pool = pool
        self._gc = False
        self._ctx = None

# ... 65 lines not shown
```

Measured before the change: 23290 sentence-pairs/s.

## Hand off decoder forward hidden states via pre-split bf16 planes

Adds a plane-based hand-off form of the persistent teacher-forced decoder forward kernel. Each step's h1/h2 is written once as pre-split bf16x3 planes with nonzero markers, and consumers read these directly instead of loading tagged fp32 rows, permuting them and re-splitting before the MMAs. The goal is less per-step work on the serial recurrence critical path. In exchange the epilogue runs as float2 on half as many threads, the handoff buffer grows to hold both encoder and decoder planes, and zero-initialisation moves to the plane region. The option default is raised to 15 so this path is on by default.

```diff
diff --git a/include/vag_nmt.h b/include/vag_nmt.h
--- a/include/vag_nmt.h
+++ b/include/vag_nmt.h
@@ -473,6 +473,7 @@
 int vag_set_operator_context(const float* derived, int storage);
 int vag_set_option(const char* name, int64_t value);
 int64_t vag_handoff_planes_floats(int64_t B, int64_t Ts, int64_t Tt, int64_t H);
+int64_t vag_dec_fwd_planes_floats(int64_t B, int64_t Tt, int64_t H);
 int vag_set_handoff_planes(float* buf, int64_t floats);
 int vag_copy4(const void* const* src, void* const* dst, const int64_t* bytes, int n, vag_stream_t stream);
 int64_t vag_derived_floats(int64_t H);
diff --git a/vag-nmt_amd/csrc/api.hip b/vag-nmt_amd/csrc/api.hip
--- a/vag-nmt_amd/csrc/api.hip
+++ b/vag-nmt_amd/csrc/api.hip
@@ -431,14 +431,14 @@
 }
 }
 void vag_step_zero_ranges(float* ws_enc, float* ws_dec, int64_t B, int64_t Ts, int64_t Tt, int64_t Es, int64_t Et, int64_t H,
-                          unsigned** p, int64_t* n) {
+                          bool dec_fwd_planes, unsigned** p, int64_t* n) {
     BiGruWs e = bigru_ws(ws_enc, B, Ts, Es, H);
     p[0] = e.sync;
     n[0] = (reinterpret_cast<unsigned*>(ws_enc) + e.total) - e.sync;
     CgruWs d = cgru_ws(ws_dec, B, Ts, Tt, Et, H);
     p[2] = reinterpret_cast<unsigned*>(e.dx);
     n[2] = Ts * B * Es;
-    p[1] = reinterpret_cast<unsigned*>(d.h1);
+    p[1] = reinterpret_cast<unsigned*>(dec_fwd_planes ? d.psc : d.h1);
     n[1] = (reinterpret_cast<unsigned*>(ws_dec) + d.total) - p[1];
 }
 extern "C" {
@@ -1432,7 +1432,8 @@
 }
 int vag_persistent_timeouts(void) { return vag_persistent_timeouts_read(); }
 int64_t vag_handoff_planes_floats(int64_t B, int64_t Ts, int64_t Tt, int64_t H) {
-    const int64_t e = vag_enc_bwd_planes_floats(B, Ts, H), d = vag_dec_bwd_planes_floats(B, Tt, H), f = vag_enc_fwd_planes_floats(B, Ts, H);
+    const int64_t e = vag_enc_bwd_planes_floats(B, Ts, H), d = vag_dec_bwd_planes_floats(B, Tt, H);
+    const int64_t f = vag_enc_fwd_planes_floats(B, Ts, H) + vag_dec_fwd_planes_floats(B, Tt, H);
     return std::max(std::max(e, d), f);
 }
 int vag_set_handoff_planes(float* buf, int64_t floats) {
diff --git a/vag-nmt_amd/csrc/call_ctx.h b/vag-nmt_amd/csrc/call_ctx.h
--- a/vag-nmt_amd/csrc/call_ctx.h
+++ b/vag-nmt_amd/csrc/call_ctx.h
@@ -27,6 +27,7 @@
     bool step_gathered = false;
     bool poison_inject = false;
     bool persist_prezeroed = false;
+    float* dec_fwd_planes_zeroed = nullptr;
     struct GemmScratch { float* slab = nullptr; int64_t floats = 0; unsigned* tickets = nullptr; int64_t ntickets = 0; hipStream_t stream = nullptr; } gemm_scratch;
     const float* gemm_prezeroed[4] = {nullptr, nullptr, nullptr, nullptr};
     struct LeafStream { hipStream_t stream = nullptr; hipEvent_t event = nullptr; bool used = false; } leaf_stream;
diff --git a/vag-nmt_amd/csrc/common.h b/vag-nmt_amd/csrc/common.h
--- a/vag-nmt_amd/csrc/common.h
+++ b/vag-nmt_amd/csrc/common.h
@@ -102,7 +102,7 @@
     int persistent_dec_bwd = 1;
     int persistent_enc_bwd = 1;
     int attn_dot_reg = 1;
-    int handoff_planes = 7;
+    int handoff_planes = 15;
     int free_persistent = 1;
     int s16_one_plane = 1;
     int head_bf16_dlogits = 1;
diff --git a/vag-nmt_amd/csrc/kernels.h b/vag-nmt_amd/csrc/kernels.h
--- a/vag-nmt_amd/csrc/kernels.h
+++ b/vag-nmt_amd/csrc/kernels.h
@@ -213,7 +213,8 @@
 int vag_rmw_defer_flush(hipStream_t s);
 bool vag_rmw_defer_meanpool(const float* mask, const float* dx, float coef, int64_t B, int64_t Ts, int64_t C, float* out, int accumulate);
 void vag_step_zero_ranges(float* ws_enc, float* ws_dec, int64_t B, int64_t Ts, int64_t Tt, int64_t Es, int64_t Et, int64_t H,
-                          unsigned** p, int64_t* n);
+                          bool dec_fwd_planes, unsigned** p, int64_t* n);
+float* vag_dec_fwd_planes_region(int64_t B, int64_t Ts, int64_t Tt, int64_t H);
 bool vag_dec_persistent_ok(int64_t B, int64_t Ts, int64_t Tt, int64_t H);
 int64_t vag_dec_persistent_sync_words(int64_t B, int64_t Tt);
 int vag_dec_fwd_persistent_launch(const float* pe, const float* mask, const float* h0, const float* xp1, const float* W1,
diff --git a/vag-nmt_amd/csrc/persist.hip b/vag-nmt_amd/csrc/persist.hip
--- a/vag-nmt_amd/csrc/persist.hip
+++ b/vag-nmt_amd/csrc/persist.hip
@@ -212,6 +212,27 @@
         acc = mma6(w[s], hf, acc);
     }
     return acc;
+}
+
+__device__ __forceinline__ unsigned pl_mark(unsigned w) { return w ? w : 0x80008000u; }
+__device__ __forceinline__ void st_planes2_marked(const char* kblk, unsigned voff, float x, float y) {
+    unsigned q0, q1, q2;
+    split3(x, y, q0, q1, q2);
+    asm volatile("global_store_dword %0, %1, %4 sc1\n\tglobal_store_dword %0, %2, %4 offset:1024 sc1\n\t"
+                 "global_store_dword %0, %3, %4 offset:2048 sc1\n\ts_nop 1"
+                 :: "v"(voff), "v"(pl_mark(q0)), "v"(pl_mark(q1)), "v"(pl_mark(q2)), "s"(kblk) : "memory");
+}
+template <int N>
+__device__ __forceinline__ void ld_planes_marked(const char* p, unsigned voff, u32x4 (&f)[3 * N], unsigned spin, bool& dead,
+                                                 unsigned* err, unsigned* guard) {
+    for (unsigned tries = 0;; ++tries) {
+        ld_planes_sc1<N>(p, voff, f);
+        unsigned m = 0xffffffffu;
+#pragma unroll
+        for (int s = 0; s < 3 * N; ++s) m = min(min(m, min(f[s][0], f[s][1])), min(f[s][2], f[s][3]));
+        if (__all(m != 0u) || dead) return;
+        if (tries > spin) { if ((threadIdx.x & 63) == 0) note_timeout(err, guard); dead = true; return; }
+    }
 }
 
 template <int KS, bool PL>
@@ -884,6 +905,7 @@
     float p_out;
     int V, ldl;
     int xcd_map;
+    char* pl;
 };
 
 constexpr int SHARDS = 4, SHARD_STRIDE = 16, CNT_WORDS = SHARDS * SHARD_STRIDE;
@@ -985,10 +1007,11 @@
     return ((unsigned long long)(u ^ ((u >> 31) ? 0xffffffffu : 0x80000000u)) << 32) | (unsigned long long)(0xffffffffu - (unsigned)idx);
 }
 
-template <bool FREE, int WGS = DEC_WGS>
+template <bool FREE, int WGS = DEC_WGS, bool PL = false>
 __global__ __launch_bounds__(512, 1) void dec_fwd_persistent_kernel(DecPArgs a) {
     extern __shared__ __attribute__((aligned(16))) float dlds[];
     static_assert(WGS == 64 || (WGS == 32 && !FREE), "H = 512 (both forms) or H = 256 (teacher-forced form)");
+    static_assert(!(PL && FREE), "the free-running form keeps the fp32 hand-off");
     constexpr int H = WGS * DEC_U, C = 2 * H, Q = C + 3 * H, KS = H / 256;
     constexpr int E = DEC_E;
     int i, rt;
@@ -1095,6 +1118,10 @@
     gu32* c6 = (gu32*)(a.cnt + ((int64_t)4 * a.RT + rt) * Tt * CNT_WORDS);
     constexpr unsigned PER_SHARD = WGS / SHARDS;
     bool dead = false;
+    const char* plb = PL ? a.pl + (int64_t)rt * pl_block_bytes(H) : nullptr;
+    const int64_t pl_step = (int64_t)a.RT * pl_block_bytes(H);
+    const int pl_ld = __builtin_amdgcn_readfirstlane(wave) * (KS * PL_KSTEP_BYTES), pl_st = (u0 >> 5) * PL_KSTEP_BYTES;
+    const unsigned pl_so = pl_slot_off(fr, eu);
     __syncthreads();
     VAG_PSTAMP(2);
 #ifdef VAG_LAB
@@ -1115,38 +1142,117 @@
         const int src4 = ld_src4(lane);
         VAG_STAMP(0);
         float4 ha[KS], hb[KS];
-        if (t == 0) {
-            const float* hp = a.h0 + (int64_t)arow * H + kbase + 8 * fg;
-#pragma unroll
-            for (int s = 0; s < KS; ++s) { ha[s] = *reinterpret_cast<const float4*>(hp + 32 * s); hb[s] = *reinterpret_cast<const float4*>(hp + 32 * s + 4); }
-        } else {
-            wait_count(c1 + (t - 1) * CNT_WORDS, PER_SHARD, a.err, a.guard, a.spin, dead);
-            VAG_STAMP(1);
-            ld_rows_tagged<KS>(a.h2_all + ((int64_t)(t - 1) * B + lrow) * H + kbase + 8 * (lane & 3), ha, hb, a.spin, dead, a.err, a.guard);
-#pragma unroll
-            for (int s = 0; s < KS; ++s) { ha[s] = perm4(ha[s], src4); hb[s] = perm4(hb[s], src4); }
-        }
-        {
+        if constexpr (PL) {
+            bf16x8 hf[KS][3];
+            if (t == 0) {
+                const float* hp = a.h0 + (int64_t)arow * H + kbase + 8 * fg;
+#pragma unroll
+                for (int s = 0; s < KS; ++s)
+                    split8(*reinterpret_cast<const float4*>(hp + 32 * s), *reinterpret_cast<const float4*>(hp + 32 * s + 4), hf[s]);
+            } else {
+                wait_count(c1 + (t - 1) * CNT_WORDS, PER_SHARD, a.err, a.guard, a.spin, dead);
+                VAG_STAMP(1);
+                u32x4 gf[3 * KS];
+                ld_planes_marked<KS>(plb + (int64_t)(Tt + t - 1) * pl_step + pl_ld, 16u * lane, gf, a.spin, dead, a.err, a.guard);
+#pragma unroll
+                for (int s = 0; s < 3 * KS; ++s) hf[s / 3][s % 3] = __builtin_bit_cast(bf16x8, gf[s]);
+            }
             f32x4 acc[2] = {{0.f, 0.f, 0.f, 0.f}, {0.f, 0.f, 0.f, 0.f}};
 #pragma unroll
             for (int s = 0; s < KS; ++s) {
-                bf16x8 hf[3];
-                split8(ha[s], hb[s], hf);
-                acc[0] = mma6(w1[s][0], hf, acc[0]);
-                acc[1] = mma6(w1[s][1], hf, acc[1]);
+                acc[0] = mma6(w1[s][0], hf[s], acc[0]);
+                acc[1] = mma6(w1[s][1], hf[s], acc[1]);
             }
             red[(wave * 3 + 0) * 64 + lane] = make_float4(acc[0][0], acc[0][1], acc[0][2], acc[0][3]);
             red[(wave * 3 + 1) * 64 + lane] = make_float4(acc[1][0], acc[1][1], acc[1][2], acc[1][3]);
+        } else {
+            if (t == 0) {
+                const float* hp = a.h0 + (int64_t)arow * H + kbase + 8 * fg;
+#pragma unroll
+                for (int s = 0; s < KS; ++s) { ha[s] = *reinterpret_cast<const float4*>(hp + 32 * s); hb[s] = *reinterpret_cast<const float4*>(hp + 32 * s + 4); }
+            } else {
+                wait_count(c1 + (t - 1) * CNT_WORDS, PER_SHARD, a.err, a.guard, a.spin, dead);
+                VAG_STAMP(1);
+                ld_rows_tagged<KS>(a.h2_all + ((int64_t)(t - 1) * B + lrow) * H + kbase + 8 * (lane & 3), ha, hb, a.spin, dead, a.err, a.guard);
+#pragma unroll
+                for (int s = 0; s < KS; ++s) { ha[s] = perm4(ha[s], src4); hb[s] = perm4(hb[s], src4); }
+            }
+            {
+                f32x4 acc[2] = {{0.f, 0.f, 0.f, 0.f}, {0.f, 0.f, 0.f, 0.f}};
+#pragma unroll
+                for (int s = 0; s < KS; ++s) {
+                    bf16x8 hf[3];
+                    split8(ha[s], hb[s], hf);
+                    acc[0] = mma6(w1[s][0], hf, acc[0]);
+                    acc[1] = mma6(w1[s][1], hf, acc[1]);
+                }
+                red[(wave * 3 + 0) * 64 + lane] = make_float4(acc[0][0], acc[0][1], acc[0][2], acc[0][3]);
+                red[(wave * 3 + 1) * 64 + lane] = make_float4(acc[1][0], acc[1][1], acc[1][2], acc[1][3]);
+            }
+        }
+        const int eh = (tx >> 5) & 1, eu2 = eu + 2 * eh;
+        const bool ep2 = PL && tx < 64, eok2 = ep2 && em < B;
+        const float2* red2 = reinterpret_cast<const float2*>(red);
+        float2 xo2[3];
+        if (eok2) {
+            const float* xp = a.xp1 + ((int64_t)t * B + em) * 3 * H + eu2;
+#pragma unroll
+            for (int g = 0; g < 3; ++g) xo2[g] = *reinterpret_cast<const float2*>(xp + g * H);
         }
         float4 xo[3];
-        if (!FREE && eok) {
+        if (!FREE && !PL && eok) {
             const float* xp = a.xp1 + ((int64_t)t * B + em) * 3 * H + eu;
 #pragma unroll
             for (int g = 0; g < 3; ++g) xo[g] = *reinterpret_cast<const float4*>(xp + g * H);
         }
         __syncthreads();
         float4 cr = make_float4(0, 0, 0, 0), cz = cr, cn = cr, hw = cr;
-        if (ep) {
+        if constexpr (PL) {
+            if (ep2) {
+                float2 cs2[3] = {make_float2(0.f, 0.f), make_float2(0.f, 0.f), make_float2(0.f, 0.f)};
+#pragma unroll
+                for (int w = 0; w < 8; ++w) {
+                    const float2 x0 = red2[((w * 3 + 0) * 64 + hq * 16 + fr) * 2 + eh], x1 = red2[((w * 3 + 0) * 64 + (2 + hq) * 16 + fr) * 2 + eh];
+                    const float2 x2 = red2[((w * 3 + 1) * 64 + hq * 16 + fr) * 2 + eh];
+                    cs2[0].x += x0.x; cs2[0].y += x0.y;
+                    cs2[1].x += x1.x; cs2[1].y += x1.y;
+                    cs2[2].x += x2.x; cs2[2].y += x2.y;
+                }
+                if (!eok2) st_planes2_marked(plb + t * pl_step + pl_st, pl_so + 4 * eh, 0.f, 0.f);
+                if (eok2) {
+                    const float2 b0 = *reinterpret_cast<const float2*>(bs_s + 0 * 8 + 4 * hq + 2 * eh);
+                    const float2 b1_ = *reinterpret_cast<const float2*>(bs_s + 1 * 8 + 4 * hq + 2 * eh);
+                    const float2 b2_ = *reinterpret_cast<const float2*>(bs_s + 2 * 8 + 4 * hq + 2 * eh);
+                    const float r_[2] = {cs2[0].x + b0.x + xo2[0].x, cs2[0].y + b0.y + xo2[0].y};
+                    const float z_[2] = {cs2[1].x + b1_.x + xo2[1].x, cs2[1].y + b1_.y + xo2[1].y};
+                    const float gh[2] = {cs2[2].x + b2_.x, cs2[2].y + b2_.y};
+                    const float xn[2] = {xo2[2].x, xo2[2].y};
+                    const float2 hprev = *reinterpret_cast<const float2*>(hs_s + 128 + fr * 8 + 4 * hq + 2 * eh);
+                    const float hpv[2] = {hprev.x, hprev.y};
+                    float rr[2], zz[2], nn[2], ho[2];
+#pragma unroll
+                    for (int q = 0; q < 2; ++q) {
+                        rr[q] = vag_sigmoid(r_[q]);
+                        zz[q] = vag_sigmoid(z_[q]);
+                        nn[q] = vag_tanh(xn[q] + rr[q] * gh[q]);
+                        ho[q] = (1.f - zz[q]) * nn[q] + zz[q] * hpv[q];
+                    }
+                    const float2 h1v = make_float2(tag1(ho[0]), tag1(ho[1]));
+                    *reinterpret_cast<float2*>(hs_s + fr * 8 + 4 * hq + 2 * eh) = h1v;
+                    st_planes2_marked(plb + t * pl_step + pl_st, pl_so + 4 * eh, h1v.x, h1v.y);
+                    if (tx == 0) arrive(c2 + t * CNT_WORDS, i);
+                    const int64_t o = (int64_t)em * H + eu2;
+                    *reinterpret_cast<float2*>(a.h1 + (int64_t)t * BH + o) = h1v;
+                    float* sv = a.g1 + (int64_t)t * 4 * BH + o;
+                    *reinterpret_cast<float2*>(sv) = make_float2(rr[0], rr[1]);
+                    *reinterpret_cast<float2*>(sv + BH) = make_float2(zz[0], zz[1]);
+                    *reinterpret_cast<float2*>(sv + 2 * BH) = make_float2(nn[0], nn[1]);
+                    *reinterpret_cast<float2*>(sv + 3 * BH) = make_float2(gh[0], gh[1]);
+                }
+                if (tx == 0 && !eok2) arrive(c2 + t * CNT_WORDS, i);
+            }
+        }
+        if (!PL && ep) {
 #pragma unroll
             for (int w = 0; w < 8; ++w) {
                 const float4 x0 = red[(w * 3 + 0) * 64 + hq * 16 + fr], x1 = red[(w * 3 + 0) * 64 + (2 + hq) * 16 + fr];
@@ -1303,7 +1409,7 @@
                 for (int g = 0; g < 3; ++g) xo[g] = *reinterpret_cast<const float4*>(xp + g * H);
             }
         }
-        if (ep) {
+        if (!PL && ep) {
             if (eok) {
                 const float4 b0 = *reinterpret_cast<const float4*>(bs_s + 0 * 8 + 4 * hq), b1_ = *reinterpret_cast<const float4*>(bs_s + 1 * 8 + 4 * hq);
                 const float4 b2_ = *reinterpret_cast<const float4*>(bs_s + 2 * 8 + 4 * hq);
@@ -1338,15 +1444,22 @@
         VAG_STAMP(2);
         wait_count(c2 + t * CNT_WORDS, PER_SHARD, a.err, a.guard, a.spin, dead);
         VAG_STAMP(3);
-        ld_rows_tagged<KS>(a.h1 + ((int64_t)t * B + lrow) * H + kbase + 8 * (lane & 3), ha, hb, a.spin, dead, a.err, a.guard);
-#pragma unroll
-        for (int s = 0; s < KS; ++s) { ha[s] = perm4(ha[s], src4); hb[s] = perm4(hb[s], src4); }
         bf16x8 hf2[KS][3];
+        if constexpr (PL) {
+            u32x4 gf[3 * KS];
+            ld_planes_marked<KS>(plb + t * pl_step + pl_ld, 16u * lane, gf, a.spin, dead, a.err, a.guard);
+#pragma unroll
+            for (int s = 0; s < 3 * KS; ++s) hf2[s / 3][s % 3] = __builtin_bit_cast(bf16x8, gf[s]);
+        } else {
+            ld_rows_tagged<KS>(a.h1 + ((int64_t)t * B + lrow) * H + kbase + 8 * (lane & 3), ha, hb, a.spin, dead, a.err, a.guard);
+#pragma unroll
+            for (int s = 0; s < KS; ++s) { ha[s] = perm4(ha[s], src4); hb[s] = perm4(hb[s], src4); }
+        }
         {
             f32x4 acc = {0.f, 0.f, 0.f, 0.f};
 #pragma unroll
             for (int s = 0; s < KS; ++s) {
-                split8(ha[s], hb[s], hf2[s]);
+                if constexpr (!PL) split8(ha[s], hb[s], hf2[s]);
                 acc = mma6(w2[s][0], hf2[s], acc);
             }
             red[(wave * 3 + 0) * 64 + lane] = make_float4(acc[0], acc[1], acc[2], acc[3]);
@@ -1459,7 +1572,45 @@
             cw_s[x] = s0 + s1;
         }
         __syncthreads();
-        if (eok) {
+        if constexpr (PL) {
+            if (ep2 && !eok2) st_planes2_marked(plb + (Tt + t) * pl_step + pl_st, pl_so + 4 * eh, 0.f, 0.f);
+            if (eok2) {
+                const int e8 = 4 * hq + 2 * eh;
+                float gi[3][2], bi[3][2], hh[3][2];
+#pragma unroll
+                for (int g = 0; g < 3; ++g) {
+                    const float2 x = *reinterpret_cast<const float2*>(gi_s + fr * 24 + g * 8 + e8);
+                    const float2 y = *reinterpret_cast<const float2*>(bs_s + 48 + g * 8 + e8);
+                    const float2 z = *reinterpret_cast<const float2*>(hp_s + fr * 24 + g * 8 + e8);
+                    gi[g][0] = x.x; gi[g][1] = x.y;
+                    bi[g][0] = y.x; bi[g][1] = y.y;
+                    hh[g][0] = z.x; hh[g][1] = z.y;
+                }
+                const float2 h1v = *reinterpret_cast<const float2*>(hs_s + fr * 8 + e8);
+                const float h1a[2] = {h1v.x, h1v.y};
+                float rr[2], zz[2], nn[2], ho[2];
+#pragma unroll
+                for (int q = 0; q < 2; ++q) {
+                    rr[q] = vag_sigmoid(gi[0][q] + bi[0][q] + hh[0][q]);
+                    zz[q] = vag_sigmoid(gi[1][q] + bi[1][q] + hh[1][q]);
+                    nn[q] = vag_tanh(gi[2][q] + bi[2][q] + rr[q] * hh[2][q]);
+                    ho[q] = (1.f - zz[q]) * nn[q] + zz[q] * h1a[q];
+                }
+                const float2 h2v = make_float2(tag1(ho[0]), tag1(ho[1]));
+                *reinterpret_cast<float2*>(hs_s + 128 + fr * 8 + e8) = h2v;
+                st_planes2_marked(plb + (Tt + t) * pl_step + pl_st, pl_so + 4 * eh, h2v.x, h2v.y);
+                if (tx == 0) arrive(c1 + t * CNT_WORDS, i);
+                const int64_t o = (int64_t)em * H + eu2;
+                *reinterpret_cast<float2*>(a.h2_all + (int64_t)t * BH + o) = h2v;
+                float* sv = a.g2 + (int64_t)t * 4 * BH + o;
+                *reinterpret_cast<float2*>(sv) = make_float2(rr[0], rr[1]);
+                *reinterpret_cast<float2*>(sv + BH) = make_float2(zz[0], zz[1]);
+                *reinterpret_cast<float2*>(sv + 2 * BH) = make_float2(nn[0], nn[1]);
+                *reinterpret_cast<float2*>(sv + 3 * BH) = make_float2(hh[2][0], hh[2][1]);
+            }
+            if (tx == 0 && !eok2) arrive(c1 + t * CNT_WORDS, i);
+        }
+        if (!PL && eok) {
             float gi[3][4];
 #pragma unroll
             for (int g = 0; g < 3; ++g) {
@@ -1499,7 +1650,7 @@
             *reinterpret_cast<float4*>(sv + 2 * BH) = make_float4(nn[0], nn[1], nn[2], nn[3]);
             *reinterpret_cast<float4*>(sv + 3 * BH) = make_float4(hn[0], hn[1], hn[2], hn[3]);
         }
-        if (tx == 0 && (!VAG_TAGGED || !eok)) arrive(c1 + t * CNT_WORDS, i);
+        if (!PL && tx == 0 && (!VAG_TAGGED || !eok)) arrive(c1 + t * CNT_WORDS, i);
     }
 #ifdef VAG_LAB
     if (!FREE && a.dbg && threadIdx.x == 0 && i == 0 && rt < 8) a.dbg[(Tt + 2) * 8 + rt] = __builtin_amdgcn_s_memrealtime();
@@ -2148,7 +2299,10 @@
 }
 static int dec_fwd_zero(DecPArgs& a, unsigned* sync, hipStream_t s) {
     VAG_TRY(sync_begin(a, sync, vag_dec_persistent_sync_words(a.B, a.Tt), s, a.psc, a.Tt * a.B * a.Ts * ACC_SHARDS));
-    if (VAG_TAGGED && !vag_ctx().persist_prezeroed) {
+    if (a.pl) {
+        if (!vag_ctx().persist_prezeroed && hipMemsetAsync(a.pl, 0, (size_t)vag_dec_fwd_planes_floats(a.B, a.Tt, a.H) * 4, s) != hipSuccess)
+            return (int)hipGetLastError();
+    } else if (VAG_TAGGED && !vag_ctx().persist_prezeroed) {
         const int nh = a.Tt * a.B * a.H;
         hipLaunchKernelGGL(zero2_u32_kernel, dim3((unsigned)cdiv64(2 * (int64_t)nh, 256)), dim3(256), 0, s,
                            reinterpret_cast<unsigned*>(a.h1), nh, reinterpret_cast<unsigned*>(a.h2_all), nh);
@@ -2167,17 +2321,23 @@
                   aligned16(bcat) && aligned16(v) && aligned16(encwp) && aligned16(b_ih2) && aligned16(h1) && aligned16(g1) &&
                   aligned16(qhp) && aligned16(h2_all) && aligned16(g2));
     DecPArgs a = dec_fwd_args(pe, mask, h0, xp1, W1, b1, wcat, bcat, v, encwp, b_ih2, h1, g1, qhp, alpha, h2_all, g2, psc, B, Ts, Tt, H);
+    a.pl = reinterpret_cast<char*>(vag_dec_fwd_planes_region(B, Ts, Tt, H));
+    if (vag_ctx().persist_prezeroed && reinterpret_cast<char*>(vag_ctx().dec_fwd_planes_zeroed) != a.pl) a.pl = nullptr;
     VAG_TRY(dec_fwd_zero(a, sync, s));
     int64_t lds = dec_persistent_lds_bytes(Ts);
     if (lds < 84 * 1024) lds = 84 * 1024;
-    if (!max_lds_once<dec_fwd_persistent_kernel<false, 64>>()) return VAG_EINVAL;
-    if (H == 256 && !max_lds_once<dec_fwd_persistent_kernel<false, 32>>()) return VAG_EINVAL;
+    bool lds_ok = false;
+    void (*kern)(DecPArgs) = nullptr;
+#define VAG_DEC_FWD_FORM(W, P) do { lds_ok = max_lds_once<dec_fwd_persistent_kernel<false, W, P>>(); kern = dec_fwd_persistent_kernel<false, W, P>; } while (0)
+    if (H == 512) { if (a.pl) VAG_DEC_FWD_FORM(64, true); else VAG_DEC_FWD_FORM(64, false); }
+    else { if (a.pl) VAG_DEC_FWD_FORM(32, true); else VAG_DEC_FWD_FORM(32, false); }
+#undef VAG_DEC_FWD_FORM
+    if (!lds_ok) return VAG_EINVAL;
     {
         PTimerScope timed(1, s);
         row_tile_passes(a.RT, dec_tiles_per_pass(H), [&](int rt0, int tiles) {
             a.rt0 = rt0;
-            if (H == 512) hipLaunchKernelGGL((dec_fwd_persistent_kernel<false, 64>), dim3(tiles * 64u), dim3(512), (size_t)lds, s, a);
-            else hipLaunchKernelGGL((dec_fwd_persistent_kernel<false, 32>), dim3(tiles * 32u), dim3(512), (size_t)lds, s, a);
+            hipLaunchKernelGGL(kern, dim3(tiles * (unsigned)dec_wgs(H)), dim3(512), (size_t)lds, s, a);
         });
     }
     VAG_LAUNCH_CHECK();
@@ -2339,6 +2499,16 @@
 int64_t vag_enc_fwd_planes_floats(int64_t B, int64_t Ts, int64_t H) {
     if ((H != 1024 && H != 512 && H != 256) || B <= 0 || Ts <= 0 || !pl_any_device_takes(cdiv64(B, 16), (int)(PL_MAX_CUS / (2 * (H / 16))))) return 0;
     return 2 * Ts * cdiv64(B, 16) * pl_block_bytes(H) / 4;
+}
+extern "C" int64_t vag_dec_fwd_planes_floats(int64_t B, int64_t Tt, int64_t H) {
+    if ((H != 512 && H != 256) || B <= 0 || Tt <= 0 || !pl_any_device_takes(cdiv64(B, 16), PL_MAX_CUS / dec_wgs(H))) return 0;
+    return 2 * Tt * cdiv64(B, 16) * pl_block_bytes(H) / 4;
+}
+float* vag_dec_fwd_planes_region(int64_t B, int64_t Ts, int64_t Tt, int64_t H) {
+    const VagCallCtx& c = vag_ctx();
+    if (!VAG_TAGGED || !(vag_opt().handoff_planes & 8) || !c.handoff_planes || vag_dec_fwd_planes_floats(B, Tt, H) <= 0) return nullptr;
+    if (c.handoff_floats < vag_handoff_planes_floats(B, Ts, Tt, H)) return nullptr;
+    return c.handoff_planes + vag_enc_fwd_planes_floats(B, Ts, H);
 }
 static int64_t dec_bwd_handoff_floats(int64_t B, int64_t Tt, int64_t H) {
     if ((H != 512 && H != 256) || B <= 0 || Tt <= 0 || !pl_any_device_takes(cdiv64(B, 16), PL_MAX_CUS / dec_wgs(H))) return 0;
diff --git a/vag-nmt_amd/csrc/step.hip b/vag-nmt_amd/csrc/step.hip
--- a/vag-nmt_amd/csrc/step.hip
+++ b/vag-nmt_amd/csrc/step.hip
@@ -251,12 +251,14 @@
         {
             unsigned* zp[3];
             int64_t zn[3];
-            vag_step_zero_ranges(k.ws_enc, k.ws_dec, B, Ts, Tt, c.Es, Et, H, zp, zn);
+            float* dpl = c.free_run ? nullptr : vag_dec_fwd_planes_region(B, Ts, Tt, H);
+            ctx.dec_fwd_planes_zeroed = dpl;
+            vag_step_zero_ranges(k.ws_enc, k.ws_dec, B, Ts, Tt, c.Es, Et, H, dpl != nullptr, zp, zn);
             int64_t nb = cdiv64((Tt + 1) * B, 256);
             if (nb < cdiv64(zn[1], 1024)) nb = cdiv64(zn[1], 1024);
             if (nb > 1024) nb = 1024;
             ZeroRanges zr;
-            zr.p[0] = reinterpret_cast<uint4*>(h2_all); zr.n[0] = Tt * B * H / 4;
+            zr.p[0] = reinterpret_cast<uint4*>(dpl ? dpl : h2_all); zr.n[0] = dpl ? vag_dec_fwd_planes_floats(B, Tt, H) / 4 : Tt * B * H / 4;
             zr.p[1] = reinterpret_cast<uint4*>(k.tmid); zr.n[1] = Tt * B * Et / 4;
             zr.p[2] = reinterpret_cast<uint4*>(zp[2]); zr.n[2] = zn[2] / 4;
             zr.p[3] = reinterpret_cast<uint4*>(k.scr_head); zr.n[3] = chunk > 0 ? 0 : Tt * B * Et / 4;
diff --git a/vag-nmt_amd/vagnmt_hip/_lib.py b/vag-nmt_amd/vagnmt_hip/_lib.py
--- a/vag-nmt_amd/vagnmt_hip/_lib.py
+++ b/vag-nmt_amd/vagnmt_hip/_lib.py
@@ -219,6 +219,7 @@
     "vag_set_operator_context": (I32, [P, I32]),
     "vag_set_option": (I32, [C.c_char_p, I64]),
     "vag_handoff_planes_floats": (I64, [I64, I64, I64, I64]),
+    "vag_dec_fwd_planes_floats": (I64, [I64, I64, I64]),
     "vag_set_handoff_planes": (I32, [P, I64]),
     "vag_recurrence_supported": (I32, [I32, I64, I64, I64, I64]),
     "vag_persistent_timeouts": (I32, []),
```

After: 23550 sentence-pairs/s, median of 6. 1.01x the previous value.
